# kowaalczyk/reformer-tts

Measured on AMD Instinct MI355X. Metric: mel-frames/sec training step, LJSpeech-shape batch, higher is better.
Workload: dtype bf16; 1 GPU; config/baseline.yml full Reformer-TTS training step (enc 3 / dec 3 layers, d=512, LSH 8 rounds, buckets 64/128), per-GPU batch 12, text 200->256, mel 1024x80; global_batch=12, parallelism=dp1, reversible_recompute=full

## Files before the change

### include/rtts.h

```cpp
#ifndef RTTS_H
#define RTTS_H

#include <stdint.h>

#ifdef __cplusplus
extern "C" {
#endif

#define RTTS_VERSION 1

int rtts_version(void);
const char* rtts_last_error(void);

int rtts_lsh_hash_sort(const void* qk, int64_t ld_qk, const float* rotations, int rot_rows,
                       int B, int H, int T, int dh, int n_hashes, int bucket_size,
                       int32_t* buckets, int32_t* st, int32_t* undo, void* stream);
int rtts_lsh_hash_sort_launches(int T);

int rtts_lsh_attn_fwd(const void* qk, const void* v, int64_t ld, const int32_t* st, const uint8_t* mask,
                      int B, int H, int T, int dh, int n_hashes, int bucket_size, int causal,
                      void* o, float* lse, float drop_p, uint32_t drop_seed, const uint32_t* seed_dev, void* stream);
int rtts_lsh_attn_fwd_run_length(int B, int H, int T, int n_hashes, int bucket_size);
int rtts_debug_set_walk(int fwd_run, int bwd_run);

int rtts_lsh_combine_fwd(const void* o, const float* lse, int B, int H, int T, int dh, int n_hashes,
                         void* out, int64_t ld_out, float* lse_tot, void* stream);

int rtts_lsh_bwd_qk_slots(void);
int rtts_lsh_attn_bwd_run_length(int B, int H, int T, int n_hashes, int bucket_size);
int rtts_lsh_bwd_delta(const void* out, int64_t ld_out, const void* dout, int64_t ld_dout,
                       int B, int H, int T, int dh, float* delta, void* stream);
int rtts_lsh_attn_bwd(const void* qk, const void* v, int64_t ld, const int32_t* st, const uint8_t* mask,
                      const void* dout, int64_t ld_dout, const float* lse_tot, const float* delta,
                      int B, int H, int T, int dh, int n_hashes, int bucket_size, int causal,
                      void* dqk_part, void* dv_part, uint8_t* row_flags, float drop_p, uint32_t drop_seed, const uint32_t* seed_dev,
                      void* stream);
int rtts_lsh_bwd_reduce(const void* dqk_part, const void* dv_part, int B, int H, int T, int dh, int n_hashes,
                        void* dqk, void* dv, int64_t ld_d, const uint8_t* row_flags, void* stream);

int rtts_grad_clip_scale(const float* grads, int64_t n, float grad_mult, float max_norm, float* partial_ws,
                         float* scale_out, void* stream);
int rtts_adamw_step(float* params, const float* grads, float* exp_avg, float* exp_avg_sq, const uint8_t* decay_mask,
                    int64_t n, const float* scale, const float* hyper, float beta1, float beta2, float eps,
                    float weight_decay, void* bf16_mirror, void* stream);

int rtts_ln_fwd(const float* x, const float* gamma, const float* beta, void* xn, float* mean, float* rstd,
                int M, int d, void* stream);
int rtts_ln_bwd(const void* dxn, const float* x, const float* mean, const float* rstd, const float* gamma,
                float* dx_io, float* dgamma, float* dbeta, float* partial_ws, int M, int d,
                void* dyb_next, float* partial_next, float drop_p, uint32_t seed, const uint32_t* seed_dev, void* stream);
int rtts_ln_bwd_to(const void* dxn, const float* x, const float* mean, const float* rstd, const float* gamma, const float* dx_in,
                   float* dx_out, float* dgamma, float* dbeta, float* partial_ws, int M, int d,
                   void* dyb_next, float* partial_next, float drop_p, uint32_t seed, const uint32_t* seed_dev, void* stream);
int rtts_ln_bwd_join(const void* dxn, const float* x, const float* mean, const float* rstd, const float* gamma, const float* dx_in,
                     const float* addend, float* dx_out, float* dgamma, float* dbeta, float* partial_ws, int M, int d,
                     void* dyb_next, float* partial_next, float drop_p, uint32_t seed, const uint32_t* seed_dev, void* stream);
int rtts_cast_colsum(const float* dy, void* dyb, float* dbias, float* partial_ws, int M, int d, float drop_p, uint32_t seed,
                     const uint32_t* seed_dev, const float* scale_dev, void* stream);
int rtts_colsum_bf16(void* dh, const void* h, int64_t ld, float* dbias, float* partial_ws, int M, int d,
                     int relu_gate, float gate_scale, void* gated_out, void* stream);
#define RTTS_COLSUM_MAX_GROUP 48
typedef struct {
    const float* partial;
    float* out;
    int32_t nrows, n;
    int32_t ld, reserved;
} rtts_colsum_job;
int rtts_colsum_partial_rows(int M);
int rtts_colsum_final_grouped(const rtts_colsum_job* jobs, int n, void* stream);
int rtts_residual_epilogue(const float* x, const void* g, const float* bias, float sign, float* y,
                           int64_t M, int d, float drop_p, uint32_t seed, const uint32_t* seed_dev, void* stream);
int rtts_residual_ln(float* x, const void* g, const float* bias, float sign, const float* gamma, const float* beta,
                     void* xn, float* mean, float* rstd, int M, int d, float drop_p, uint32_t seed, const uint32_t* seed_dev,
                     float* y, void* stream);
int rtts_sum_streams(const float* a, const float* b, int64_t n, float* out, void* out_bf16, void* stream);
int rtts_bias_act(void* h, const float* bias, int64_t M, int d, int relu, void* stream);
int rtts_cast_f32_bf16(const float* src, void* dst, int64_t n, void* stream);

int rtts_xattn_key_chunks(int Tk);
int rtts_xattn_fwd(const void* q, int64_t ld_q, const void* kv, int64_t ld_kv, const uint8_t* kvalid,
                   int B, int H, int Tq, int Tk, int dh, void* o, int64_t ld_o, float* lse,
                   float drop_p, uint32_t seed, const uint32_t* seed_dev, void* stream);
int rtts_xattn_bwd(const void* q, int64_t ld_q, const void* kv, int64_t ld_kv, const uint8_t* kvalid,
                   const void* dout, int64_t ld_dout, const float* lse, const float* delta,
                   int B, int H, int Tq, int Tk, int dh, void* dq, int64_t ld_dq, void* dkv_part,
                   float drop_p, uint32_t seed, const uint32_t* seed_dev, void* dq_chunks, void* stream);
int rtts_sum_slabs(const void* part, int nslabs, int64_t n, void* out, void* stream);
int rtts_xattn_probs_mean(const void* q, int64_t ld_q, const void* kv, int64_t ld_kv, const uint8_t* kvalid,
                          const float* lse, int B, int H, int Tq, int Tk, int dh, float* a, int64_t ld_a, void* stream);

int rtts_conv1d_k5(const void* x, int64_t ldx, const void* wp, int64_t ldw, int transposed, int M, int C_out, int C_in,
                   void* y, int64_t ldy, const float* bias, int out_f32, void* stream);
int rtts_to_halo(const void* src, int64_t ld_src, int64_t src_batch_stride, int C_src, int src_f32, int B, int L, int halo, int C,
                 void* dst, int lead, int64_t rows, void* stream);
int rtts_conv_w_perm(const float* w, int Co, int Ci, int CP, void* wp, void* stream);
int rtts_conv_dw_unperm(const float* dwp, int Co, int Ci, int CP, float* dw, void* stream);
#define RTTS_CONV_PERM_MAX_GROUP 8
typedef struct {
    const float* w;
    void* wp;
    int32_t Co, Ci, CP, reserved;
} rtts_conv_perm_job;
int rtts_conv_w_perm_grouped(const rtts_conv_perm_job* jobs, int n, void* stream);
int rtts_conv_dw_unperm_grouped(const rtts_conv_perm_job* jobs, int n, void* stream);
int rtts_conv1d_k5_moments(const void* x, int64_t ldx, const void* wp, int64_t ldw, int M, int C_out, int C_in, void* y, int64_t ldy,
                           int B, int L, int halo, float* partial, void* stream);
int rtts_bn_stats_from_partials(const float* partial, int nrows, int B, int L, int C, float* mean, float* rstd, float* run_mean,
                                float* run_var, const float* mean_shift, int64_t* num_batches, void* stream);
int rtts_bn_stats(const float* y, int B, int L, int halo, int C, float* mean, float* rstd, float* run_mean, float* run_var,
                  const float* mean_shift, int64_t* num_batches, float* partial_ws, void* stream);
int rtts_bn_act_fwd(const float* y, const float* mean, const float* rstd, const float* gamma, const float* beta, int act,
                    float drop_p, uint32_t seed, const uint32_t* seed_dev, int B, int L, int halo, int C, void* z, int z_halo,
                    int z_lead, int64_t z_rows, void* stream);
int rtts_bn_act_bwd(const float* y, const void* dz, int dz_halo, const float* mean, const float* rstd, const float* gamma,
                    const float* beta, int act, float drop_p, uint32_t seed, const uint32_t* seed_dev, int B, int L, int halo, int C,
                    void* dy, int dy_lead, int64_t dy_rows, float* dgamma, float* dbeta, float* partial_ws, void* stream);
int rtts_bn_moments(const float* y, int B, int L, int halo, int C, float* moments, float* partial_ws, void* stream);
int rtts_bn_from_moments(const float* moments, int64_t count, int C, float* mean, float* rstd, float* run_mean, float* run_var,
                         const float* mean_shift, int64_t* num_batches, void* stream);
int rtts_bn_act_bwd_sums(const float* y, const void* dz, int dz_halo, const float* mean, const float* rstd, const float* gamma,
                         const float* beta, int act, float drop_p, uint32_t seed, const uint32_t* seed_dev, int B, int L, int halo, int C,
// ... 115 lines not shown
```

### reformer-tts_amd/_lib.py

```python
from __future__ import annotations

import ctypes as C
import os

_HERE = os.path.dirname(os.path.abspath(__file__))
LIB_PATH = os.environ.get("RTTS_LIB") or os.path.join(_HERE, "lib", "librtts_hip.so")

_i64, _i32, _vp, _f32, _u32 = C.c_int64, C.c_int, C.c_void_p, C.c_float, C.c_uint32

class GemmTnProblem(C.Structure):
    _fields_ = [("a", _vp), ("lda", _i64), ("b", _vp), ("ldb", _i64), ("c", _vp), ("ldc", _i64),
                ("M", C.c_int32), ("N", C.c_int32), ("K", C.c_int32), ("accumulate", C.c_int32)]


GEMM_TN_MAX_GROUP = 16


class GemmNtProblem(C.Structure):
    _fields_ = [("a", _vp), ("lda", _i64), ("w", _vp), ("ldw", _i64), ("c", _vp), ("ldc", _i64), ("bias", _vp), ("aux", _vp),
                ("ld_aux", _i64), ("aux_out", _vp), ("M", C.c_int32), ("N", C.c_int32), ("K", C.c_int32), ("epilogue", C.c_int32),
                ("T", C.c_int32), ("H", C.c_int32), ("accumulate", C.c_int32), ("reserved", C.c_int32)]


GEMM_NT_MAX_GROUP = 4


class ColsumJob(C.Structure):
    _fields_ = [("partial", _vp), ("out", _vp), ("nrows", C.c_int32), ("n", C.c_int32), ("ld", C.c_int32), ("reserved", C.c_int32)]


COLSUM_MAX_GROUP = 48


class Segment(C.Structure):
    _fields_ = [("dst", _vp), ("src", _vp), ("count", C.c_int64), ("kind", C.c_int32), ("reserved", C.c_int32)]


SEGMENTS_MAX = 12
SEG_COPY_F32, SEG_COPY_BF16, SEG_ADD_F32, SEG_CAST_F32_BF16 = 0, 1, 2, 3


class ConvPermJob(C.Structure):
    _fields_ = [("w", _vp), ("wp", _vp), ("Co", C.c_int32), ("Ci", C.c_int32), ("CP", C.c_int32), ("reserved", C.c_int32)]


CONV_PERM_MAX_GROUP = 8

SIGNATURES = {
    "rtts_lsh_hash_sort": [_vp, _i64, _vp, _i32, _i32, _i32, _i32, _i32, _i32, _i32, _vp, _vp, _vp, _vp],
    "rtts_lsh_attn_fwd": [_vp, _vp, _i64, _vp, _vp, _i32, _i32, _i32, _i32, _i32, _i32, _i32, _vp, _vp, _f32, _u32, _vp, _vp],
    "rtts_lsh_hash_sort_launches": [_i32],
    "rtts_lsh_attn_fwd_run_length": [_i32, _i32, _i32, _i32, _i32],
    "rtts_lsh_combine_fwd": [_vp, _vp, _i32, _i32, _i32, _i32, _i32, _vp, _i64, _vp, _vp],
    "rtts_lsh_bwd_delta": [_vp, _i64, _vp, _i64, _i32, _i32, _i32, _i32, _vp, _vp],
    "rtts_lsh_attn_bwd": [_vp, _vp, _i64, _vp, _vp, _vp, _i64, _vp, _vp, _i32, _i32, _i32, _i32, _i32, _i32, _i32, _vp, _vp, _vp, _f32, _u32, _vp,
                          _vp],
    "rtts_lsh_bwd_qk_slots": [],
    "rtts_lsh_attn_bwd_run_length": [_i32, _i32, _i32, _i32, _i32],
    "rtts_debug_set_walk": [_i32, _i32],
    "rtts_lsh_bwd_reduce": [_vp, _vp, _i32, _i32, _i32, _i32, _i32, _vp, _vp, _i64, _vp, _vp],
    "rtts_grad_clip_scale": [_vp, _i64, _f32, _f32, _vp, _vp, _vp],
    "rtts_ln_fwd": [_vp, _vp, _vp, _vp, _vp, _vp, _i32, _i32, _vp],
    "rtts_ln_bwd": [_vp, _vp, _vp, _vp, _vp, _vp, _vp, _vp, _vp, _i32, _i32, _vp, _vp, _f32, _u32, _vp, _vp],
    "rtts_ln_bwd_to": [_vp, _vp, _vp, _vp, _vp, _vp, _vp, _vp, _vp, _vp, _i32, _i32, _vp, _vp, _f32, _u32, _vp, _vp],
    "rtts_ln_bwd_join": [_vp, _vp, _vp, _vp, _vp, _vp, _vp, _vp, _vp, _vp, _vp, _i32, _i32, _vp, _vp, _f32, _u32, _vp, _vp],
    "rtts_cast_colsum": [_vp, _vp, _vp, _vp, _i32, _i32, _f32, _u32, _vp, _vp, _vp],
    "rtts_colsum_bf16": [_vp, _vp, _i64, _vp, _vp, _i32, _i32, _i32, _f32, _vp, _vp],
    "rtts_sum_streams": [_vp, _vp, _i64, _vp, _vp, _vp],
    "rtts_residual_epilogue": [_vp, _vp, _vp, _f32, _vp, _i64, _i32, _f32, _u32, _vp, _vp],
    "rtts_colsum_partial_rows": [_i32],
    "rtts_colsum_final_grouped": [C.POINTER(ColsumJob), _i32, _vp],
    "rtts_residual_ln": [_vp, _vp, _vp, _f32, _vp, _vp, _vp, _vp, _vp, _i32, _i32, _f32, _u32, _vp, _vp, _vp],
    "rtts_bias_act": [_vp, _vp, _i64, _i32, _i32, _vp],
    "rtts_cast_f32_bf16": [_vp, _vp, _i64, _vp],
    "rtts_xattn_fwd": [_vp, _i64, _vp, _i64, _vp, _i32, _i32, _i32, _i32, _i32, _vp, _i64, _vp, _f32, _u32, _vp, _vp],
    "rtts_xattn_bwd": [_vp, _i64, _vp, _i64, _vp, _vp, _i64, _vp, _vp, _i32, _i32, _i32, _i32, _i32, _vp, _i64, _vp, _f32, _u32, _vp, _vp, _vp],
    "rtts_xattn_key_chunks": [_i32],
    "rtts_xattn_probs_mean": [_vp, _i64, _vp, _i64, _vp, _vp, _i32, _i32, _i32, _i32, _i32, _vp, _i64, _vp],
    "rtts_sum_slabs": [_vp, _i32, _i64, _vp, _vp],
    "rtts_conv1d_k5": [_vp, _i64, _vp, _i64, _i32, _i32, _i32, _i32, _vp, _i64, _vp, _i32, _vp],
    "rtts_to_halo": [_vp, _i64, _i64, _i32, _i32, _i32, _i32, _i32, _i32, _vp, _i32, _i64, _vp],
    "rtts_heads_grad": [_vp, _vp, _i32, _vp, _i64, _vp, _i32, _i32, _i32, _i32, _i32, _vp, _vp, _vp],
    "rtts_segments": [C.POINTER(Segment), _i32, _vp],
    "rtts_conv_w_perm": [_vp, _i32, _i32, _i32, _vp, _vp],
    "rtts_conv_dw_unperm": [_vp, _i32, _i32, _i32, _vp, _vp],
    "rtts_conv_w_perm_grouped": [C.POINTER(ConvPermJob), _i32, _vp],
    "rtts_conv_dw_unperm_grouped": [C.POINTER(ConvPermJob), _i32, _vp],
    "rtts_conv1d_k5_moments": [_vp, _i64, _vp, _i64, _i32, _i32, _i32, _vp, _i64, _i32, _i32, _i32, _vp, _vp],
    "rtts_bn_stats_from_partials": [_vp, _i32, _i32, _i32, _i32, _vp, _vp, _vp, _vp, _vp, _vp, _vp],
    "rtts_bn_stats": [_vp, _i32, _i32, _i32, _i32, _vp, _vp, _vp, _vp, _vp, _vp, _vp, _vp],
    "rtts_bn_act_fwd": [_vp, _vp, _vp, _vp, _vp, _i32, _f32, _u32, _vp, _i32, _i32, _i32, _i32, _vp, _i32, _i32, _i64, _vp],
    "rtts_bn_act_bwd": [_vp, _vp, _i32, _vp, _vp, _vp, _vp, _i32, _f32, _u32, _vp, _i32, _i32, _i32, _i32, _vp, _i32, _i64, _vp, _vp, _vp, _vp],
    "rtts_bn_moments": [_vp, _i32, _i32, _i32, _i32, _vp, _vp, _vp],
    "rtts_bn_from_moments": [_vp, _i64, _i32, _vp, _vp, _vp, _vp, _vp, _vp, _vp],
    "rtts_bn_act_bwd_sums": [_vp, _vp, _i32, _vp, _vp, _vp, _vp, _i32, _f32, _u32, _vp, _i32, _i32, _i32, _i32, _vp, _vp, _vp, _vp, _vp],
    "rtts_bn_act_bwd_apply": [_vp, _vp, _i32, _vp, _vp, _vp, _vp, _i32, _f32, _u32, _vp, _i32, _i32, _i32, _i32, _vp, _i64, _vp, _i32, _i64, _vp],
    "rtts_tts_loss": [_vp, _vp, _i64, _vp, _vp, _vp, _i64, _vp, _i32, _i32, _i32, _f32, _f32, _f32, _f32, _vp, _vp, _i64, _vp, _vp, _vp, _i32, _i32,
                      _vp, _i64, _i32, _i32, _i64, _i64, _vp, _i64, _i64, _vp],
    "rtts_pe_add": [_vp, _vp, _vp, _f32, _u32, _vp, _i32, _i64, _i32, _vp, _vp],
    "rtts_debug_stamp": [_vp, _i32, _vp],
    "rtts_batch_masks": [_vp, _i64, _i32, _i32, _i32, _vp, _i64, _i64, _i32, _i32, _i32, _vp, _vp, _vp, _vp, _vp],
    "rtts_pe_dalpha": [_vp, _vp, _f32, _u32, _vp, _i32, _i64, _i32, _vp, _vp, _vp],
    "rtts_relu_drop": [_vp, _f32, _u32, _vp, _i64, _vp],
    "rtts_embedding_bwd": [_vp, _vp, _i32, _i32, _i32, _i32, _vp, _f32, _u32, _vp, _vp],
    "rtts_embedding_bwd_strided": [_vp, _vp, _i64, _i64, _i32, _i32, _i32, _i32, _i32, _vp, _f32, _u32, _vp, _vp],
    "rtts_embedding_fwd": [_vp, _vp, _i32, _i32, _i32, _f32, _u32, _vp, _vp, _vp],
    "rtts_gemm_tn": [_vp, _i64, _vp, _i64, _i32, _i32, _i32, _vp, _i64, _i32, _vp, _i64, _vp],
    "rtts_gemm_tn_grouped": [C.POINTER(GemmTnProblem), _i32, _vp, _i64, _vp],
    "rtts_gemm_nt": [_vp, _i64, _vp, _i64, _i32, _i32, _i32, _i32, _vp, _i64, _vp, _i32, _vp, _i64, _vp, _vp],
    "rtts_gemm_nt_partial_rows": [_i32, _i32],
    "rtts_gemm_nt_grouped": [C.POINTER(GemmNtProblem), _i32, _i32, _vp],
    "rtts_debug_set_gemm_mode": [_i32],
    "rtts_gemm_nt_gate_words": [_i32, _i32],
    "rtts_gemm_nt_gated": [_vp, _i64, _vp, _i64, _i32, _i32, _i32, _i32, _vp, _i64, _vp, _i32, _vp, _vp, _vp],
    "rtts_peak_copy": [_vp, _vp, _i64, _vp],
    "rtts_comm_probe": [_vp, _vp, _i64, _i32, _i32, _vp],
    "rtts_peak_mfma": [_vp, _i32, _i32, _vp],
    "rtts_sw_depthwise_k3": [_vp, _vp, _vp, _i32, _i32, _i32, _vp, _vp, _vp, _vp],
    "rtts_sw_gate": [_vp, _vp, _i64, _i32, _i32, _i32, _i32, _i32, _i32, _vp, _vp],
    "rtts_sw_coupling_inv": [_vp, _i64, _vp, _i64, _i32, _vp],
    "rtts_sw_depthwise_k3_seg": [_vp, _vp, _vp, _vp, _i32, _i32, _i64, _i32, _vp, _vp, _vp, _vp],
    "rtts_sw_pack_mel": [_vp, _i64, _i64, _i64, _i32, _i32, _vp, _i32, _i64, _vp, _i64, _vp],
    "rtts_sw_coupling_inv1x1": [_vp, _i64, _vp, _i64, _vp, _i32, _i64, _vp, _i64, _vp],
    "rtts_sw_coupling_fwd1x1": [_vp, _i64, _vp, _i64, _vp, _i32, _i32, _i64, _vp, _i64, _vp, _i64, _i32, _vp, _vp],
    "rtts_sw_nll_reduce": [_vp, _i64, _i32, _vp, _vp, _i32, _i32, _i64, _i64, _vp, _vp],
    "rtts_sw_pack_audio": [_vp, _i64, _vp, _vp, _i32, _i32, _i32, _i64, _vp, _vp],
    "rtts_adamw_step": [_vp, _vp, _vp, _vp, _vp, _i64, _vp, _vp, _f32, _f32, _f32, _f32, _vp, _vp],
    "rtts_mel_frames": [_i64, _i32],
    "rtts_mel_spectrogram": [_vp, C.POINTER(_i64), C.POINTER(_i64), _vp, _vp, _i32, _vp, _vp, _i32, _i32, _i32, _i32, _f32, _vp, _i64, _vp],
    "rtts_resample_len": [_i64, _i32, _i32],
    "rtts_resample": [_vp, _i32, _i32, C.POINTER(_i64), C.POINTER(_i64), _vp, _vp, _i32, _vp, _vp, _i32, _i32, _i32, _vp, _vp],
}

_lib = None


class RttsError(RuntimeError):
    pass


_NOTED = set()
PATHS_LEFT = []


def note_general_path(where: str, reason: str) -> None:
    key = (where, reason)
    if key in _NOTED:
        return
    _NOTED.add(key)
    PATHS_LEFT.append(key)
    import logging
    logging.getLogger("reformer_tts_amd").warning("%s: general (eager) path instead of the explicit HIP executor -- %s", where, reason)


def log_once(key: str, message: str) -> None:
    if key in _NOTED:
        return
    _NOTED.add(key)
    import logging
    logging.getLogger("reformer_tts_amd").warning("%s", message)


def load() -> C.CDLL:
    global _lib
    if _lib is None:
        if not os.path.exists(LIB_PATH):
            raise RttsError(
                f"{LIB_PATH} is missing: build it with `python reformer-tts_amd/build.py` "
                "(or __graft_entry__.build()). There is no CPU fallback for the HIP path.")
        import torch
        lib = C.CDLL(LIB_PATH)
        lib.rtts_version.restype = C.c_int
        lib.rtts_last_error.restype = C.c_char_p
        for name, args in SIGNATURES.items():
            fn = getattr(lib, name)
            fn.argtypes = args
            fn.restype = C.c_int
        lib.rtts_gemm_nt_gate_words.restype = C.c_int64
        lib.rtts_mel_frames.restype = C.c_int64
        lib.rtts_resample_len.restype = C.c_int64
        _lib = lib
        fw, bw = os.environ.get("RTTS_LSH_FWD_WALK"), os.environ.get("RTTS_LSH_BWD_WALK")
        if fw is not None or bw is not None:
            _WALK[:] = [-1 if fw is None else int(fw), -1 if bw is None else int(bw)]
            lib.rtts_debug_set_walk(*_WALK)
        gs = os.environ.get("RTTS_GEMM_STORE")
        if gs is not None:
            lib.rtts_debug_set_gemm_mode(10 + int(gs))
    return _lib


_WALK = [-1, -1]


class forced_walk:

    def __init__(self, fwd=None, bwd=None):
        self.want = (fwd, bwd)

    def __enter__(self):
        self.old = list(_WALK)
        new = [o if w is None else int(w) for o, w in zip(self.old, self.want)]
        call("rtts_debug_set_walk", *new)
        _WALK[:] = new
        return self

    def __exit__(self, *exc):
        call("rtts_debug_set_walk", *self.old)
        _WALK[:] = self.old
        return False


def call(name: str, *args) -> None:
    lib = load()
    rc = getattr(lib, name)(*args)
    if rc != 0:
        raise RttsError(lib.rtts_last_error().decode() or f"{name} failed with code {rc}")
```

### reformer-tts_amd/csrc/lsh_attn_bwd.hip

```cpp
#include "rtts_common.h"
#include <float.h>

#define AB_DH 64
#define AB_ROWB 128
#ifndef AB_SPLIT_EPI
#define AB_SPLIT_EPI 1
#endif
#ifndef AB_DQ_UNROLL
#define AB_DQ_UNROLL 16
#endif
#ifndef AB_UNROLL
#define AB_UNROLL 4
#endif

typedef __attribute__((ext_vector_type(8))) short short8v;

#ifdef AB_PHASE_TIMING
__device__ unsigned long long g_ab_phase[32 * 8192];
#define AB_STAMP(i) do { if (threadIdx.x == 0 && blockIdx.x < 8192) g_ab_phase[blockIdx.x * 32 + (i)] = __builtin_readcyclecounter(); } while (0)
extern "C" int rtts_debug_ab_phases(void* dst) { return (int)hipMemcpyFromSymbol(dst, HIP_SYMBOL(g_ab_phase), sizeof(g_ab_phase)); }
#define AB_WSTAMP(i, w) do { if ((threadIdx.x & 63) == 0 && blockIdx.x < 8192) g_ab_phase[blockIdx.x * 32 + (i) + (w)] = __builtin_readcyclecounter(); } while (0)
#else
#define AB_STAMP(i) do { } while (0)
#define AB_WSTAMP(i, w) do { } while (0)
#endif

__device__ __forceinline__ bf16x8 tr_frag(const unsigned char* p0, const unsigned char* p1) {
    const short4v lo = __builtin_amdgcn_ds_read_tr16_b64_v4i16((RTTS_LDS short4v*)p0);
    const short4v hi = __builtin_amdgcn_ds_read_tr16_b64_v4i16((RTTS_LDS short4v*)p1);
    const short8v both = {lo[0], lo[1], lo[2], lo[3], hi[0], hi[1], hi[2], hi[3]};
    return __builtin_bit_cast(bf16x8, both);
}

__device__ __forceinline__ int ab_sw(int row) { return ((row >> 1) & 3) | ((((row >> 3) ^ (row >> 1)) & 1) << 2); }
__device__ __forceinline__ int ab_off(int row, int piece) { return row * 128 + ((piece ^ ab_sw(row)) << 4); }
template <int BS>
__device__ __forceinline__ int ab_ds_off(int key, int gran) {
    const int k0 = key & 1, k1 = (key >> 1) & 1, k2 = (key >> 2) & 1, k3 = (key >> 3) & 1;
    if (BS == 128) return key * 256 + ((gran ^ ((k1 << 4) | (k0 << 3) | (k1 << 2) | (k2 << 1) | k3)) << 3);
    return key * 128 + ((gran ^ ((k1 << 3) | (k0 << 2) | (k2 << 1) | k3)) << 3);
}

__device__ __forceinline__ int ab_stg_w(int r, int piece, int hh) { return r * 128 + ((piece ^ (r & 7)) << 4) + ((hh ^ ((r >> 3) & 1)) << 3); }
__device__ __forceinline__ int ab_stg_r(int i, int srow, int spiece) { return (i * 8 + srow) * 128 + ((spiece ^ srow) << 4); }
__device__ __forceinline__ uint4 ab_stg_fix(int i, const uint4 v) { return (i & 1) ? uint4{v.z, v.w, v.x, v.y} : v; }

#ifndef AB_KT2
#define AB_KT2 1
#endif

typedef __attribute__((ext_vector_type(2))) __bf16 ab_bf2;
__device__ __forceinline__ float ab_frags_sumsq(const bf16x8 (&f)[4]) {
    float part[4];
#pragma unroll
    for (int ks = 0; ks < 4; ++ks) {
        const uint4 u = __builtin_bit_cast(uint4, f[ks]);
        float a = 0.f;
        a = __builtin_amdgcn_fdot2_f32_bf16(__builtin_bit_cast(ab_bf2, u.x), __builtin_bit_cast(ab_bf2, u.x), a, false);
        a = __builtin_amdgcn_fdot2_f32_bf16(__builtin_bit_cast(ab_bf2, u.y), __builtin_bit_cast(ab_bf2, u.y), a, false);
        a = __builtin_amdgcn_fdot2_f32_bf16(__builtin_bit_cast(ab_bf2, u.z), __builtin_bit_cast(ab_bf2, u.z), a, false);
        a = __builtin_amdgcn_fdot2_f32_bf16(__builtin_bit_cast(ab_bf2, u.w), __builtin_bit_cast(ab_bf2, u.w), a, false);
        part[ks] = a;
    }
    return (part[0] + part[1]) + (part[2] + part[3]);
}

struct AbDrop {
    uint32_t seed;
    const uint32_t* seed_dev;
    uint32_t thresh;
    float scale;
};

template <int BS, bool CAUSAL, bool MASKED, bool DROP>
__global__ __launch_bounds__(BS * 4 / AB_KT2, AB_KT2 == 2 ? 1 : 2) void lsh_attn_bwd_kernel(
    const bf16_t* __restrict__ qk, const bf16_t* __restrict__ v, int64_t ld, const int32_t* __restrict__ st,
    const uint8_t* __restrict__ mask, const bf16_t* __restrict__ dout, int64_t ld_do, const float* __restrict__ lse_tot,
    const float* __restrict__ delta, int H, int T, int n_hashes, bf16_t* __restrict__ dqk_part, bf16_t* __restrict__ dv_part,
    size_t slot_stride, AbDrop dr) {
    constexpr int KT2 = AB_KT2;
    constexpr int NK = 2 * BS;
    constexpr int NQT = BS / 32;
    constexpr int NW = NK / (32 * KT2);
    constexpr int NTHR = 64 * NW;
    constexpr int DSROW = BS * 2;
    extern __shared__ __attribute__((aligned(16))) unsigned char smem[];
    int* kpos = reinterpret_cast<int*>(smem) + NK;
    float* qlse = reinterpret_cast<float*>(kpos + 2 * NK);
    float* qdel = qlse + BS;
    int* qpe_s = reinterpret_cast<int*>(qdel + BS);
    unsigned char* Ks = reinterpret_cast<unsigned char*>(qpe_s + BS);
    unsigned char* Os = Ks + NK * 128;
    unsigned char* Ds = Os + BS * 128;
    unsigned char* Stg = Ds + NK * DSROW;

    const int nb = T / BS;
    const int C = n_hashes * nb;
    const uint32_t wi = xcd_remap(blockIdx.x, gridDim.x);
    const int bh = wi / C, c = wi % C;
    const int b = bh / H, h = bh % H;
    const int cprev = (c == 0) ? C - 1 : c - 1;
    const int tid = threadIdx.x, lane = tid & 63, wave = __builtin_amdgcn_readfirstlane(tid >> 6);
    const int r = lane & 31, hh = lane >> 5;

    AB_STAMP(0);
    const int32_t* st_row = st + (size_t)bh * n_hashes * T;
    const bf16_t* qbase = qk + (size_t)b * T * ld + (size_t)h * AB_DH;
    const bf16_t* vbase = v + (size_t)b * T * ld + (size_t)h * AB_DH;
    const bf16_t* dobase = dout + (size_t)b * T * ld_do + (size_t)h * AB_DH;

    constexpr int ITERS = NK * 8 / NTHR;
    int trow[ITERS];
#pragma unroll
    for (int it = 0; it < ITERS; ++it) {
        const int row = (it * NTHR + tid) >> 3;
        const int slot = (row < BS) ? c * BS + row : cprev * BS + (row - BS);
        trow[it] = st_row[slot];
    }
    int myrow[KT2], mypos[KT2];
#pragma unroll
    for (int k2 = 0; k2 < KT2; ++k2) {
        myrow[k2] = (wave * KT2 + k2) * 32 + r;
        mypos[k2] = st_row[(myrow[k2] < BS) ? c * BS + myrow[k2] : cprev * BS + (myrow[k2] - BS)];
    }
#ifdef AB_PHASE_TIMING
    __builtin_amdgcn_s_waitcnt(0x0F70);
    AB_STAMP(10);
#endif
#pragma unroll
    for (int it = 0; it < ITERS; ++it) {
        const int rowb = it * (NTHR / 8) + wave * 8;
        const int lp = (lane & 7) ^ ab_sw(rowb + (lane >> 3));
        __builtin_amdgcn_global_load_lds((const __attribute__((address_space(1))) void*)(qbase + (size_t)trow[it] * ld + lp * 8),
                                         (RTTS_LDS void*)(Ks + rowb * 128), 16, 0, 0);
        if (it < ITERS / 2)
            __builtin_amdgcn_global_load_lds((const __attribute__((address_space(1))) void*)(dobase + (size_t)trow[it] * ld_do + lp * 8),
                                             (RTTS_LDS void*)(Os + rowb * 128), 16, 0, 0);
    }
    int rvalid[ITERS / 2];
    float rlse[ITERS / 2], rdel[ITERS / 2];
#pragma unroll
    for (int it = 0; it < ITERS / 2; ++it) {
        rvalid[it] = MASKED ? (int)mask[(size_t)b * T + trow[it]] : 1;
        rlse[it] = lse_tot[(size_t)bh * T + trow[it]];
        rdel[it] = delta[(size_t)bh * T + trow[it]];
    }
    int myvalid[KT2];
    bf16x8 vf[KT2][4];
#pragma unroll
    for (int k2 = 0; k2 < KT2; ++k2) {
        myvalid[k2] = MASKED ? (int)mask[(size_t)b * T + mypos[k2]] : 1;
#pragma unroll
        for (int ks = 0; ks < 4; ++ks) vf[k2][ks] = *reinterpret_cast<const bf16x8*>(vbase + (size_t)mypos[k2] * ld + ks * 16 + 8 * hh);
    }
#ifdef AB_PHASE_TIMING
    __builtin_amdgcn_s_waitcnt(0x0F70);
    AB_STAMP(11);
#endif
    const int cbase = (tid & 7) < 3 ? (tid & 7) * (NK * 4) : 3 * NK * 4 + ((tid & 7) - 3) * (BS * 4);
#pragma unroll
    for (int it = 0; it < ITERS / 2; ++it) {
        const int row = (it * NTHR + tid) >> 3, piece = tid & 7;
// ... 224 lines not shown
        for (int di = 0; di < KT2; ++di) {
            const int dt = (KT2 == 2) ? di : (wave & 1);
            const int kpc = dt * 4 + 2 * trc + (trp >> 1);
            ko0[di] = ab_off(rl, kpc) + 8 * (trp & 1);
            ko1[di] = ab_off(rl + 4, kpc) + 8 * (trp & 1);
        }
        const int gq = qt * 8 + 4 * trc + trp;
        const int do0 = ab_ds_off<BS>(rl, gq), do1 = ab_ds_off<BS>(rl + 4, gq);
#pragma unroll AB_DQ_UNROLL
        for (int kb = 0; kb < NK; kb += 16) {
            const bf16x8 bfrag = tr_frag(Ds + kb * DSROW + do0, Ds + kb * DSROW + do1);
#pragma unroll
            for (int di = 0; di < KT2; ++di) {
                const bf16x8 afrag = tr_frag(Ks + kb * 128 + ko0[di], Ks + kb * 128 + ko1[di]);
                dq[di] = __builtin_amdgcn_mfma_f32_32x32x16_bf16(afrag, bfrag, dq[di], 0, 0, 0);
            }
        }
#pragma unroll
        for (int di = 0; di < KT2; ++di) {
            const int dt = (KT2 == 2) ? di : (wave & 1);
#pragma unroll
            for (int g = 0; g < 4; ++g) {
                uint2 pk;
                pk.x = pack_bf16x2(dq[di][4 * g], dq[di][4 * g + 1]);
                pk.y = pack_bf16x2(dq[di][4 * g + 2], dq[di][4 * g + 3]);
                *reinterpret_cast<uint2*>(Os + ab_off(qt * 32 + r, dt * 4 + g) + 8 * hh) = pk;
            }
        }
    }
    AB_STAMP(6);
    __syncthreads();
    AB_STAMP(7);

#pragma unroll
    for (int k2 = 0; k2 < KT2; ++k2) {
        unsigned char* stg = Stg + (wave * KT2 + k2) * (32 * AB_ROWB);
        bf16_t* dkdst = dqk_part + (own_tile ? 0 : slot_stride);
        float kraw[2][16];
        float dot = 0.f;
#pragma unroll
        for (int dt = 0; dt < 2; ++dt)
#pragma unroll
            for (int g = 0; g < 4; ++g) {
                const uint2 kk = *reinterpret_cast<const uint2*>(Ks + ab_off(myrow[k2], dt * 4 + g) + 8 * hh);
                kraw[dt][4 * g] = __uint_as_float(kk.x << 16);
                kraw[dt][4 * g + 1] = __uint_as_float(kk.x & 0xffff0000u);
                kraw[dt][4 * g + 2] = __uint_as_float(kk.y << 16);
                kraw[dt][4 * g + 3] = __uint_as_float(kk.y & 0xffff0000u);
#pragma unroll
                for (int j = 0; j < 4; ++j) dot = __builtin_fmaf(kraw[dt][4 * g + j], gacc[k2][dt][4 * g + j], dot);
            }
        const float ncoef = -rtts_xhalf_sum(dot) * (ksc[k2] * 8.f) * (ksc[k2] * 8.f);
#pragma unroll
        for (int dt = 0; dt < 2; ++dt)
#pragma unroll
            for (int g = 0; g < 4; ++g) {
                float dk[4];
#pragma unroll
                for (int j = 0; j < 4; ++j) dk[j] = __builtin_fmaf(kraw[dt][4 * g + j], ncoef, gacc[k2][dt][4 * g + j]);
                if (own_tile) {
                    const uint2 dqv = *reinterpret_cast<const uint2*>(Os + ab_off(myrow[k2], dt * 4 + g) + 8 * hh);
                    dk[0] += __uint_as_float(dqv.x << 16);
                    dk[1] += __uint_as_float(dqv.x & 0xffff0000u);
                    dk[2] += __uint_as_float(dqv.y << 16);
                    dk[3] += __uint_as_float(dqv.y & 0xffff0000u);
                }
                uint2 pk;
                pk.x = pack_bf16x2(dk[0], dk[1]);
                pk.y = pack_bf16x2(dk[2], dk[3]);
                *reinterpret_cast<uint2*>(stg + ab_stg_w(r, dt * 4 + g, hh)) = pk;
            }
        __builtin_amdgcn_wave_barrier();
        uint4 rowv[4];
#pragma unroll
        for (int i = 0; i < 4; ++i) rowv[i] = ab_stg_fix(i, *reinterpret_cast<const uint4*>(stg + ab_stg_r(i, srow, spiece)));
#pragma unroll
        for (int i = 0; i < 4; ++i) rtts_store16_out(dkdst + (obase + rpos[k2][i]) * AB_DH + spiece * 8, rowv[i]);
    }
    AB_STAMP(8);
#ifdef AB_PHASE_TIMING
    __builtin_amdgcn_s_waitcnt(0);
    AB_STAMP(9);
#endif
}



__device__ __forceinline__ void ab_dma16(const void* gptr, RTTS_LDS void* lds_dst_wave_uniform) {
    const uint32_t m0v = __builtin_amdgcn_readfirstlane((uint32_t)(uintptr_t)lds_dst_wave_uniform);
    asm volatile("s_mov_b32 m0, %1\n\ts_nop 0\n\tglobal_load_lds_dwordx4 %0, off" ::"v"(gptr), "s"(m0v) : "m0");
}

template <int BS, bool CAUSAL, bool MASKED, bool DROP>
__global__ __launch_bounds__(BS * 4, 2) void lsh_attn_bwd_walk_kernel(
    const bf16_t* __restrict__ qk, const bf16_t* __restrict__ v, int64_t ld, const int32_t* __restrict__ st,
    const uint8_t* __restrict__ mask, const bf16_t* __restrict__ dout, int64_t ld_do, const float* __restrict__ lse_tot,
    const float* __restrict__ delta, int H, int T, int n_hashes, bf16_t* __restrict__ dqk_part, bf16_t* __restrict__ dv_part,
    size_t slot_stride, int R, uint8_t* __restrict__ row_flags, AbDrop dr) {
    constexpr int NK = 2 * BS;
    constexpr int NQT = BS / 32;
    constexpr int NW = NK / 32;
    constexpr int NTHR = 64 * NW;
    constexpr int DSROW = BS * 2;
    constexpr int KSLOT = BS * 128;
    extern __shared__ __attribute__((aligned(16))) unsigned char smem[];
    int* kposS = reinterpret_cast<int*>(smem);
    float* qlseS = reinterpret_cast<float*>(kposS + 4 * BS);
    float* qdelS = qlseS + 2 * BS;
    int* qpeS = reinterpret_cast<int*>(qdelS + 2 * BS);
    unsigned char* KsR = reinterpret_cast<unsigned char*>(qpeS + 2 * BS);
    unsigned char* OsR = KsR + 3 * KSLOT;
    unsigned char* Ds = OsR + 2 * KSLOT;
    unsigned char* Stg = Ds;

    const int nb = T / BS;
    const int C = n_hashes * nb;
    const int runs = C / R;
    const uint32_t run = xcd_remap(blockIdx.x, gridDim.x);
    const int bh = run / runs, c0 = (run % runs) * R;
    const int b = bh / H, h = bh % H;
    const int32_t* st_row = st + (size_t)bh * n_hashes * T;
    const bf16_t* qbase = qk + (size_t)b * T * ld + (size_t)h * AB_DH;
    const bf16_t* vbase = v + (size_t)b * T * ld + (size_t)h * AB_DH;
    const bf16_t* dobase = dout + (size_t)b * T * ld_do + (size_t)h * AB_DH;

    {
        const int tid = threadIdx.x, lane = tid & 63, wave = __builtin_amdgcn_readfirstlane(tid >> 6);
        const int cp0 = (c0 == 0) ? C - 1 : c0 - 1;
        constexpr int ITERS = NK * 8 / NTHR;
        int trow[ITERS];
#pragma unroll
        for (int it = 0; it < ITERS; ++it) {
            const int row = (it * NTHR + tid) >> 3;
            trow[it] = st_row[(row < BS) ? c0 * BS + row : cp0 * BS + (row - BS)];
        }
        int pnext = 0;
        if (R > 1 && tid < BS) pnext = st_row[(c0 + 1) * BS + tid];
#pragma unroll
        for (int it = 0; it < ITERS; ++it) {
            const int rowb = it * (NTHR / 8) + wave * 8;
            const int lp = (lane & 7) ^ ab_sw(rowb + (lane >> 3));
            unsigned char* kdst = (rowb < BS) ? KsR + KSLOT + rowb * 128 : KsR + (rowb - BS) * 128;
            __builtin_amdgcn_global_load_lds((const __attribute__((address_space(1))) void*)(qbase + (size_t)trow[it] * ld + lp * 8),
                                             (RTTS_LDS void*)kdst, 16, 0, 0);
            if (it < ITERS / 2)
                __builtin_amdgcn_global_load_lds((const __attribute__((address_space(1))) void*)(dobase + (size_t)trow[it] * ld_do + lp * 8),
                                                 (RTTS_LDS void*)(OsR + rowb * 128), 16, 0, 0);
        }
        int rvalid[ITERS / 2];
        float rlse[ITERS / 2], rdel[ITERS / 2];
#pragma unroll
        for (int it = 0; it < ITERS / 2; ++it) {
            rvalid[it] = MASKED ? (int)mask[(size_t)b * T + trow[it]] : 1;
            rlse[it] = lse_tot[(size_t)bh * T + trow[it]];
            rdel[it] = delta[(size_t)bh * T + trow[it]];
        }
#pragma unroll
        for (int it = 0; it < ITERS; ++it) {
            const int row = (it * NTHR + tid) >> 3, piece = tid & 7;
            if (piece == 1) kposS[(row < BS) ? BS + row : row - BS] = trow[it];
            if (it < ITERS / 2) {
                if (piece == 3) qlseS[row] = rlse[it] * 1.4426950408889634f;
                if (piece == 4) qdelS[row] = -rdel[it];
                if (piece == 5) qpeS[row] = rvalid[it] ? (CAUSAL ? trow[it] : 0) : -1;
            }
        }
        if (R > 1 && tid < BS) kposS[2 * BS + tid] = pnext;
    }
#if AB_SPLIT_EPI
    __builtin_amdgcn_s_waitcnt(0x0F70);
    __syncthreads();
#endif

    bf16x8 vf[4], kf[4];
    float ksc = 0.f, sdq = 0.f;
    int myvalid = 1, mypos = 0, kpk = 0;
    f32x16 dvacc[2], gacc[2];
#pragma unroll 1
    for (int j = 0; j < R; ++j) {
        int tid = threadIdx.x;
        asm volatile("" : "+v"(tid));
// ... 318 lines not shown
#endif
                    const float dqf[4] = {__uint_as_float(dqv.x << 16), __uint_as_float(dqv.x & 0xffff0000u), __uint_as_float(dqv.y << 16),
                                          __uint_as_float(dqv.y & 0xffff0000u)};
#pragma unroll
                    for (int jj = 0; jj < 4; ++jj) {
                        gacc[dt][4 * g + jj] += dqf[jj];
                        sd4[jj] = __builtin_fmaf(kraw[dt][4 * g + jj], dqf[jj], sd4[jj]);
                    }
                }
            sdq = rtts_xhalf_sum((sd4[0] + sd4[1]) + (sd4[2] + sd4[3]));
        }
        if (!own_tile || j == R - 1) {
            const int slot = (!own_tile && j == 0) ? 1 : 0;
            const size_t obase = ((size_t)bh * n_hashes + (own_tile ? c / nb : cprev / nb)) * T;
            const int srow = lane >> 3, spiece = lane & 7;
#if AB_SPLIT_EPI
            unsigned char* stg = Ds + ((own_tile ? BS : 0) + wt * 32) * DSROW;
            static_assert(32 * DSROW >= 32 * AB_ROWB, "the staging must fit a wave's rows of the dS'^T image");
#else
            unsigned char* stg = Stg + wave * (32 * AB_ROWB);
#endif
            int rpos[4];
#pragma unroll
            for (int i = 0; i < 4; ++i) rpos[i] = own_tile ? kq[wt * 32 + i * 8 + srow] : kl[wt * 32 + i * 8 + srow];
            {
                bf16_t* dvdst = dv_part + slot * slot_stride;
#pragma unroll
                for (int dt = 0; dt < 2; ++dt)
#pragma unroll
                    for (int g = 0; g < 4; ++g) {
                        uint2 pk;
                        pk.x = pack_bf16x2(dvacc[dt][4 * g], dvacc[dt][4 * g + 1]);
                        pk.y = pack_bf16x2(dvacc[dt][4 * g + 2], dvacc[dt][4 * g + 3]);
                        *reinterpret_cast<uint2*>(stg + ab_stg_w(r, dt * 4 + g, hh)) = pk;
                    }
                __builtin_amdgcn_wave_barrier();
                uint4 rowv[4];
#pragma unroll
                for (int i = 0; i < 4; ++i) rowv[i] = ab_stg_fix(i, *reinterpret_cast<const uint4*>(stg + ab_stg_r(i, srow, spiece)));
#pragma unroll
                for (int i = 0; i < 4; ++i) rtts_store16_out(dvdst + (obase + rpos[i]) * AB_DH + spiece * 8, rowv[i]);
                __builtin_amdgcn_wave_barrier();
            }
            {
                bf16_t* dkdst = dqk_part + slot * slot_stride;
                float dot4[4] = {0.f, 0.f, 0.f, 0.f};
#pragma unroll
                for (int dt = 0; dt < 2; ++dt)
#pragma unroll
                    for (int e = 0; e < 16; ++e) dot4[e & 3] = __builtin_fmaf(kraw[dt][e], gacc[dt][e], dot4[e & 3]);
                const float dot = (dot4[0] + dot4[1]) + (dot4[2] + dot4[3]);
                const float ncoef = -(rtts_xhalf_sum(dot) - sdq) * (ksc * 8.f) * (ksc * 8.f);
#pragma unroll
                for (int dt = 0; dt < 2; ++dt)
#pragma unroll
                    for (int g = 0; g < 4; ++g) {
                        float dk[4];
#pragma unroll
                        for (int jj = 0; jj < 4; ++jj) dk[jj] = __builtin_fmaf(kraw[dt][4 * g + jj], ncoef, gacc[dt][4 * g + jj]);
                        uint2 pk;
                        pk.x = pack_bf16x2(dk[0], dk[1]);
                        pk.y = pack_bf16x2(dk[2], dk[3]);
                        *reinterpret_cast<uint2*>(stg + ab_stg_w(r, dt * 4 + g, hh)) = pk;
                    }
                __builtin_amdgcn_wave_barrier();
                uint4 rowv[4];
#pragma unroll
                for (int i = 0; i < 4; ++i) rowv[i] = ab_stg_fix(i, *reinterpret_cast<const uint4*>(stg + ab_stg_r(i, srow, spiece)));
#pragma unroll
                for (int i = 0; i < 4; ++i) rtts_store16_out(dkdst + (obase + rpos[i]) * AB_DH + spiece * 8, rowv[i]);
            }
            if (slot == 0 && spiece == 0) {
#pragma unroll
                for (int i = 0; i < 4; ++i) row_flags[obase + rpos[i]] = own_tile ? 1 : 0;
            }
        }
        AB_JSTAMP(8);
#ifdef AB_PHASE_TIMING
        __builtin_amdgcn_s_waitcnt(0x0F70);
        AB_JSTAMP(9);
#endif
    }
#undef AB_JSTAMP
}

extern "C" int rtts_lsh_bwd_qk_slots(void) { return RTTS_LSH_BWD_QK_SLOTS; }

extern "C" int rtts_lsh_attn_bwd_run_length(int B, int H, int T, int n_hashes, int bucket_size) {
    if (B <= 0 || H <= 0 || n_hashes <= 0 || bucket_size <= 0 || T <= 0 || T % bucket_size) return -1;
    const int C = n_hashes * (T / bucket_size);
    const long long chunks = (long long)B * H * C;
    int R = 0;
    if (AB_KT2 == 1)
        for (int cand = 8; cand >= 4; cand >>= 1)
            if (C % cand == 0 && chunks / cand >= 768) { R = cand; break; }
    const int w = rtts_walk_override(1);
    if (w >= 0 && AB_KT2 == 1) R = (w >= 1 && C % w == 0) ? w : 0;
    return R;
}

template <int BS>
static int launch_attn_bwd(const bf16_t* qk, const bf16_t* v, int64_t ld, const int32_t* st, const uint8_t* mask,
                           const bf16_t* dout, int64_t ld_do, const float* lse_tot, const float* delta, int B, int H, int T,
                           int n_hashes, int causal, bf16_t* dqk_part, bf16_t* dv_part, uint8_t* row_flags, float drop_p,
                           uint32_t drop_seed, const uint32_t* seed_dev, hipStream_t stream) {
    constexpr int NK = 2 * BS;
    const size_t slot_stride = (size_t)B * H * n_hashes * T * AB_DH;
    const bool drop = drop_p > 0.f;
    const int vi = (drop ? 4 : 0) + (causal ? 2 : 0) + (mask ? 1 : 0);
    const AbDrop dr{drop_seed, seed_dev, rtts_drop_thresh(drop_p), 1.f / (1.f - drop_p)};
    const int C = n_hashes * (T / BS);
    const long long chunks = (long long)B * H * C;
    const int R = rtts_lsh_attn_bwd_run_length(B, H, T, n_hashes, BS);
    if (R >= 1 && AB_KT2 == 1) {
        RTTS_REQUIRE(row_flags, "rtts_lsh_attn_bwd: this shape is worked by the walking kernel (rtts_lsh_attn_bwd_run_length() = %d): "
                                "row_flags (B*H*n_hashes*T bytes) is required", R);
        const size_t ds_bytes = (size_t)NK * (BS * 2), stg_bytes = (size_t)(NK / 32) * 32 * AB_ROWB;
        const size_t wlds = (size_t)BS * 40 + 5 * (size_t)BS * 128 + (ds_bytes > stg_bytes ? ds_bytes : stg_bytes);
        static RttsLdsState wattr[8];
        const dim3 wgrid((unsigned)(chunks / R)), wblock(BS * 4);
#define AB_WGO(C_, M_, D_)                                                                                                 \
    do {                                                                                                                   \
        auto kern = lsh_attn_bwd_walk_kernel<BS, C_, M_, D_>;                                                              \
        RTTS_ENSURE_LDS("rtts_lsh_attn_bwd", kern, wlds, wattr[vi]);                                                       \
        hipLaunchKernelGGL(kern, wgrid, wblock, wlds, stream, qk, v, ld, st, mask, dout, ld_do, lse_tot, delta, H, T, n_hashes, \
                           dqk_part, dv_part, slot_stride, R, row_flags, dr);                                              \
    } while (0)
#define AB_WGO2(C_, M_) do { if (drop) AB_WGO(C_, M_, true); else AB_WGO(C_, M_, false); } while (0)
        if (causal) {
            if (mask) AB_WGO2(true, true); else AB_WGO2(true, false);
        } else {
            if (mask) AB_WGO2(false, true); else AB_WGO2(false, false);
        }
#undef AB_WGO2
#undef AB_WGO
        RTTS_LAUNCH_CHECK("rtts_lsh_attn_bwd");
        return 0;
    }
    const size_t lds = NK * 128 + BS * 128 + NK * (BS * 2) + (NK / 32) * 32 * AB_ROWB + NK * 12 + BS * 12;
    const dim3 grid(B * H * n_hashes * (T / BS)), block(BS * 4 / AB_KT2);
    static RttsLdsState attr[8];
#define AB_GO(C_, M_, D_)                                                                                                  \
    do {                                                                                                                   \
        auto kern = lsh_attn_bwd_kernel<BS, C_, M_, D_>;                                                                   \
        RTTS_ENSURE_LDS("rtts_lsh_attn_bwd", kern, lds, attr[vi]);                                                         \
        hipLaunchKernelGGL(kern, grid, block, lds, stream, qk, v, ld, st, mask, dout, ld_do, lse_tot, delta, H, T, n_hashes, \
                           dqk_part, dv_part, slot_stride, dr);                                                            \
    } while (0)
#define AB_GO2(C_, M_) do { if (drop) AB_GO(C_, M_, true); else AB_GO(C_, M_, false); } while (0)
    if (causal) {
        if (mask) AB_GO2(true, true); else AB_GO2(true, false);
    } else {
        if (mask) AB_GO2(false, true); else AB_GO2(false, false);
    }
#undef AB_GO2
#undef AB_GO
    RTTS_LAUNCH_CHECK("rtts_lsh_attn_bwd");
    return 0;
}

extern "C" int rtts_lsh_attn_bwd(const void* qk, const void* v, int64_t ld, const int32_t* st, const uint8_t* mask,
                                 const void* dout, int64_t ld_dout, const float* lse_tot, const float* delta, int B, int H,
                                 int T, int dh, int n_hashes, int bucket_size, int causal, void* dqk_part, void* dv_part,
                                 uint8_t* row_flags, float drop_p, uint32_t drop_seed, const uint32_t* seed_dev, void* stream) {
    RTTS_ENTER(stream);
    RTTS_REQUIRE(qk && v && st && dout && lse_tot && delta && dqk_part && dv_part, "rtts_lsh_attn_bwd: null pointer");
    RTTS_REQUIRE(dh == AB_DH, "rtts_lsh_attn_bwd: dh=%d unsupported (this build: 64)", dh);
    RTTS_REQUIRE(bucket_size == 64 || bucket_size == 128, "rtts_lsh_attn_bwd: bucket_size=%d unsupported (64 or 128)", bucket_size);
    RTTS_REQUIRE(T > 0 && T % (2 * bucket_size) == 0,
                 "rtts_lsh_attn_bwd: Sequence length (%d) needs to be divisible by target bucket size x 2 - %d", T, 2 * bucket_size);
    RTTS_REQUIRE(B > 0 && H > 0 && n_hashes > 0, "rtts_lsh_attn_bwd: bad B/H/n_hashes");
    RTTS_REQUIRE(ld >= (int64_t)H * dh && ld % 8 == 0 && ld_dout >= (int64_t)H * dh && ld_dout % 8 == 0,
                 "rtts_lsh_attn_bwd: row strides must be >= H*dh and multiples of 8");
    RTTS_REQUIRE((((uintptr_t)qk | (uintptr_t)v | (uintptr_t)dout | (uintptr_t)dqk_part | (uintptr_t)dv_part) & 15) == 0,
                 "rtts_lsh_attn_bwd: buffers must be 16-byte aligned");
    RTTS_REQUIRE(drop_p >= 0.f && drop_p < 1.f, "rtts_lsh_attn_bwd: drop_p must be in [0, 1)");
    RTTS_REQUIRE(drop_p == 0.f || (uint64_t)B * H * n_hashes * T * 2 * bucket_size < (1ull << 32),
                 "rtts_lsh_attn_bwd: dropout on more than 2^32 query-key pairs (the forward refuses the same shape)");
    hipStream_t s = (hipStream_t)stream;
    if (bucket_size == 64)
        return launch_attn_bwd<64>((const bf16_t*)qk, (const bf16_t*)v, ld, st, mask, (const bf16_t*)dout, ld_dout, lse_tot, delta,
                                   B, H, T, n_hashes, causal, (bf16_t*)dqk_part, (bf16_t*)dv_part, row_flags, drop_p, drop_seed, seed_dev, s);
    return launch_attn_bwd<128>((const bf16_t*)qk, (const bf16_t*)v, ld, st, mask, (const bf16_t*)dout, ld_dout, lse_tot, delta, B,
                                H, T, n_hashes, causal, (bf16_t*)dqk_part, (bf16_t*)dv_part, row_flags, drop_p, drop_seed, seed_dev, s);
}
```

### reformer-tts_amd/csrc/lsh_attn_fwd.hip

```cpp
#include "rtts_common.h"
#include <float.h>

#define AF_DH 64
#define AF_ROWB 144
#define AF_LOG2E 1.4426950408889634f
#define AF_NEG (-1.0e30f)
#define AF_BIGPOS 0x40000000
#define AF_SLACK 8.0f

typedef __attribute__((ext_vector_type(8))) short af_short8;
typedef __attribute__((ext_vector_type(2))) __bf16 af_bf2;

#ifdef AF_PHASE_TIMING
__device__ unsigned long long g_af_phase[16 * 8192];
#define AF_STAMP(i) do { if ((threadIdx.x & 63) == 0 && blockIdx.x < 8192 && ((threadIdx.x >> 6) == 0 || (threadIdx.x >> 6) == BS / 32)) \
        g_af_phase[blockIdx.x * 16 + ((threadIdx.x >> 6) ? 8 : 0) + (i)] = __builtin_readcyclecounter(); } while (0)
extern "C" int rtts_debug_af_phases(void* dst) { return (int)hipMemcpyFromSymbol(dst, HIP_SYMBOL(g_af_phase), sizeof(g_af_phase)); }
#ifndef AF_WSTEP
#define AF_WSTEP 1
#endif
#define AF_WSTAMP(i) do { if (j == AF_WSTEP && lane == 0 && blockIdx.x < 8192 && qt == 0) \
        g_af_phase[blockIdx.x * 16 + (kh ? 8 : 0) + (i)] = __builtin_readcyclecounter(); } while (0)
#else
#define AF_STAMP(i) do { } while (0)
#define AF_WSTAMP(i) do { } while (0)
#endif

#ifndef AF_UNROLL
#define AF_UNROLL BS == 64 ? 2 : 1
#endif
__device__ __forceinline__ int af_sw(int row) { return ((row >> 1) & 3) | ((((row >> 3) ^ (row >> 1)) & 1) << 2); }
__device__ __forceinline__ int af_voff(int row, int piece) { return row * 128 + ((piece ^ af_sw(row)) << 4); }

__device__ __forceinline__ float af_sum16(const f32x16& a) {
    const float s0 = (a[0] + a[1]) + (a[2] + a[3]), s1 = (a[4] + a[5]) + (a[6] + a[7]);
    const float s2 = (a[8] + a[9]) + (a[10] + a[11]), s3 = (a[12] + a[13]) + (a[14] + a[15]);
    return (s0 + s1) + (s2 + s3);
}

#ifndef AF_FOLD
#define AF_FOLD 1
#endif
#ifndef AF_TILE_SKIP
#define AF_TILE_SKIP 1
#endif
__device__ __forceinline__ void af_tile_probs(f32x16& acc, const float* __restrict__ ksc_t, const int* __restrict__ kpos_t,
                                              const int* __restrict__ kpe_t, int keyt, int hh, bool chk_self, int qpos, int qpe, float& m,
                                              float& l, f32x16 (&oacc)[2], bool live_all = false) {
    const bool fresh = m < -1.0e4f;
    const float mref = fresh ? 0.f : m;
    const float nref = -mref, selfv = (-5e4f * AF_LOG2E) - mref;
    float gmax[2] = {AF_NEG, AF_NEG};
    if (chk_self) {
#pragma unroll
        for (int g = 0; g < 4; ++g) {
            const int key0 = keyt + 8 * g + 4 * hh;
            const float4 sc = *reinterpret_cast<const float4*>(ksc_t + key0);
            const int4 kp = *reinterpret_cast<const int4*>(kpos_t + key0);
            const int4 ke = *reinterpret_cast<const int4*>(kpe_t + key0);
            const float scv[4] = {sc.x, sc.y, sc.z, sc.w};
            const int kpv[4] = {kp.x, kp.y, kp.z, kp.w};
            const int kev[4] = {ke.x, ke.y, ke.z, ke.w};
#pragma unroll
            for (int j = 0; j < 4; ++j) {
                float x = __builtin_fmaf(acc[4 * g + j], scv[j], nref);
                x = (kev[j] > qpe) ? AF_NEG : x;
                x = (kpv[j] == qpos) ? selfv : x;
                acc[4 * g + j] = x;
                gmax[g & 1] = fmaxf(gmax[g & 1], x);
            }
        }
    } else if (live_all) {
#pragma unroll
        for (int g = 0; g < 4; ++g) {
            const float4 sc = *reinterpret_cast<const float4*>(ksc_t + keyt + 8 * g + 4 * hh);
            const float scv[4] = {sc.x, sc.y, sc.z, sc.w};
#pragma unroll
            for (int j = 0; j < 4; ++j) {
                const float x = __builtin_fmaf(acc[4 * g + j], scv[j], nref);
                acc[4 * g + j] = x;
                gmax[g & 1] = fmaxf(gmax[g & 1], x);
            }
        }
    } else {
#pragma unroll
        for (int g = 0; g < 4; ++g) {
            const int key0 = keyt + 8 * g + 4 * hh;
            const float4 sc = *reinterpret_cast<const float4*>(ksc_t + key0);
            const int4 ke = *reinterpret_cast<const int4*>(kpe_t + key0);
            const float scv[4] = {sc.x, sc.y, sc.z, sc.w};
            const int kev[4] = {ke.x, ke.y, ke.z, ke.w};
#pragma unroll
            for (int j = 0; j < 4; ++j) {
                float x = __builtin_fmaf(acc[4 * g + j], scv[j], nref);
                x = (kev[j] > qpe) ? AF_NEG : x;
                acc[4 * g + j] = x;
                gmax[g & 1] = fmaxf(gmax[g & 1], x);
            }
        }
    }
    const float tmax = rtts_xhalf_max(fmaxf(gmax[0], gmax[1]));
    if (__any(tmax > (fresh ? 0.5f * AF_NEG : AF_SLACK))) {
        const float mnew = fmaxf(m, tmax + mref);
        const float alpha = __builtin_amdgcn_exp2f(m - mnew);
        const float d = mnew - mref;
        m = mnew;
#pragma unroll
        for (int i = 0; i < 16; ++i) {
            oacc[0][i] *= alpha;
            oacc[1][i] *= alpha;
            acc[i] -= d;
        }
        l *= alpha;
    }
#pragma unroll
    for (int i = 0; i < 16; ++i) acc[i] = __builtin_amdgcn_exp2f(acc[i]);
    l += af_sum16(acc);
}

template <int BS, bool CAUSAL, bool MASKED, bool DROP>
__global__ __launch_bounds__(BS * 4, 2) void lsh_attn_fwd_kernel(const bf16_t* __restrict__ qk, const bf16_t* __restrict__ v,
                                                                 int64_t ld, const int32_t* __restrict__ st,
                                                                 const uint8_t* __restrict__ mask, int H, int T, int n_hashes,
                                                                 bf16_t* __restrict__ o, float* __restrict__ lse, uint32_t drop_seed,
                                                                 const uint32_t* __restrict__ seed_dev, uint32_t drop_thresh,
                                                                 float drop_scale) {
    constexpr int NK = 2 * BS;
    constexpr int NKT = NK / 32;
    constexpr int NTHR = BS * 4;
    constexpr int NQT = BS / 32;
    extern __shared__ __attribute__((aligned(16))) unsigned char smem[];
    float* ksc = reinterpret_cast<float*>(smem);
    int* kpos = reinterpret_cast<int*>(ksc + NK);
    int* kpe = kpos + NK;
    unsigned char* Ks = smem + NK * 12;
    unsigned char* Vs = Ks + NK * AF_ROWB;

    const int nb = T / BS;
    const int C = n_hashes * nb;
    const uint32_t wi = xcd_remap(blockIdx.x, gridDim.x);
    const int bh = wi / C, c = wi % C;
    const int b = bh / H, h = bh % H;
    const int cprev = (c == 0) ? C - 1 : c - 1;
    const int tid = threadIdx.x, lane = tid & 63, wave = __builtin_amdgcn_readfirstlane(tid >> 6);

    const int32_t* st_row = st + (size_t)bh * n_hashes * T;
    const bf16_t* qbase = qk + (size_t)b * T * ld + (size_t)h * AF_DH;
    const bf16_t* vbase = v + (size_t)b * T * ld + (size_t)h * AF_DH;

    AF_STAMP(0);
    constexpr int ITERS = NK * 8 / NTHR;
    {
        int trow[ITERS];
#pragma unroll
        for (int it = 0; it < ITERS; ++it) {
            const int row = (it * NTHR + tid) >> 3;
            const int slot = (row < BS) ? c * BS + row : cprev * BS + (row - BS);
            trow[it] = st_row[slot];
        }
        uint4 kreg[ITERS];
        int rvalid[ITERS];
#pragma unroll
        for (int it = 0; it < ITERS; ++it) {
            const int piece = tid & 7;
            kreg[it] = *reinterpret_cast<const uint4*>(qbase + (size_t)trow[it] * ld + piece * 8);
            const int rowb = it * (NTHR / 8) + wave * 8;
            const int lp = (lane & 7) ^ af_sw(rowb + (lane >> 3));
            __builtin_amdgcn_global_load_lds((const __attribute__((address_space(1))) void*)(vbase + (size_t)trow[it] * ld + lp * 8),
                                             (RTTS_LDS void*)(Vs + rowb * 128), 16, 0, 0);
            rvalid[it] = MASKED ? (int)mask[(size_t)b * T + trow[it]] : 1;
        }
        const int cbase = (tid & 7) * (NK * 4);
#pragma unroll
        for (int it = 0; it < ITERS; ++it) {
            const int row = (it * NTHR + tid) >> 3, piece = tid & 7;
            *reinterpret_cast<uint4*>(Ks + row * AF_ROWB + piece * 16) = kreg[it];
            float ss = 0.f;
            ss = __builtin_amdgcn_fdot2_f32_bf16(__builtin_bit_cast(af_bf2, kreg[it].x), __builtin_bit_cast(af_bf2, kreg[it].x), ss, false);
            ss = __builtin_amdgcn_fdot2_f32_bf16(__builtin_bit_cast(af_bf2, kreg[it].y), __builtin_bit_cast(af_bf2, kreg[it].y), ss, false);
            ss = __builtin_amdgcn_fdot2_f32_bf16(__builtin_bit_cast(af_bf2, kreg[it].z), __builtin_bit_cast(af_bf2, kreg[it].z), ss, false);
            ss = __builtin_amdgcn_fdot2_f32_bf16(__builtin_bit_cast(af_bf2, kreg[it].w), __builtin_bit_cast(af_bf2, kreg[it].w), ss, false);
            ss = rtts_sum8(ss);
            int w = __float_as_int((0.125f * AF_LOG2E) * __builtin_amdgcn_rsqf(fmaxf(ss, 1e-24f)));
            w = piece == 1 ? trow[it] : w;
            w = piece == 2 ? (rvalid[it] ? (CAUSAL ? trow[it] : 0) : AF_BIGPOS) : w;
            if (piece < 3) *reinterpret_cast<int*>(reinterpret_cast<unsigned char*>(ksc) + cbase + row * 4) = w;
        }
    }
    AF_STAMP(1);
    __syncthreads();
    AF_STAMP(2);

    const int r = lane & 31, hh = lane >> 5;
    const int qt = wave % NQT, kh = wave / NQT;
    const int qrow = qt * 32 + r;
    bf16x8 qf[4];
#pragma unroll
    for (int ks = 0; ks < 4; ++ks) qf[ks] = *reinterpret_cast<const bf16x8*>(Ks + qrow * AF_ROWB + (ks * 16 + 8 * hh) * 2);
    const int qpos = kpos[qrow];
    const int qpe = (kpe[qrow] == AF_BIGPOS) ? -1 : (CAUSAL ? qpos : 0);
    const int trq = (lane & 15) >> 2, trp = lane & 3, trc = (lane >> 4) & 1;

    int tro[2];
#pragma unroll
    for (int dt = 0; dt < 2; ++dt) tro[dt] = af_voff(4 * hh + trq, dt * 4 + 2 * trc + (trp >> 1)) + 8 * (trp & 1);

    const bool wrap = (cprev / nb) != (c / nb);
    float m = AF_NEG, l = 0.f;
    f32x16 oacc[2] = {{0}, {0}};
// ... 34 lines not shown
                }
            }
        } else {
#pragma unroll
            for (int g = 0; g < 4; ++g) {
                const int key0 = kt * 32 + 8 * g + 4 * hh;
                const float4 sc = *reinterpret_cast<const float4*>(ksc + key0);
                const int4 ke = *reinterpret_cast<const int4*>(kpe + key0);
                const float scv[4] = {sc.x, sc.y, sc.z, sc.w};
                const int kev[4] = {ke.x, ke.y, ke.z, ke.w};
#pragma unroll
                for (int j = 0; j < 4; ++j) {
                    float x = acc[4 * g + j] * scv[j];
#if !defined(AF_ABLATE) || AF_ABLATE != 2
                    x = (kev[j] > qpe) ? AF_NEG : x;
#endif
                    acc[4 * g + j] = x;
                    gmax[g & 1] = fmaxf(gmax[g & 1], x);
                }
            }
        }
        tmax = rtts_xhalf_max(fmaxf(gmax[0], gmax[1]));
#endif
        if (__any(tmax > m + AF_SLACK)) {
            const float mnew = fmaxf(m, tmax);
            const float alpha = __builtin_amdgcn_exp2f(m - mnew);
            m = mnew;
#pragma unroll
            for (int i = 0; i < 16; ++i) {
                oacc[0][i] *= alpha;
                oacc[1][i] *= alpha;
            }
            l *= alpha;
        }
#if defined(AF_ABLATE) && AF_ABLATE == 3
#pragma unroll
        for (int i = 0; i < 16; ++i) l += acc[i];
#else
#pragma unroll
        for (int i = 0; i < 16; ++i) acc[i] = __builtin_amdgcn_exp2f(acc[i] - m);
        l += af_sum16(acc);
#endif
#endif
        if constexpr (DROP) {
            const uint32_t seed = drop_seed + (seed_dev ? seed_dev[0] : 0u);
            const uint32_t pair0 = ((uint32_t)wi * BS + (uint32_t)qrow) * (uint32_t)NK + (uint32_t)(kt * 32 + 4 * hh);
#pragma unroll
            for (int i = 0; i < 16; ++i) acc[i] *= rtts_drop_keep(seed, pair0 + 8 * (i >> 2) + (i & 3), drop_thresh, drop_scale);
        }
#if defined(AF_ABLATE) && AF_ABLATE == 4
        oacc[0][0] += acc[0] + acc[5] + acc[10] + acc[15];
        if (false)
#endif
#pragma unroll
        for (int s2 = 0; s2 < 2; ++s2) {
            const int o8 = 8 * s2;
            const bf16x8 pf = cvt_bf16x8(acc[o8], acc[o8 + 1], acc[o8 + 2], acc[o8 + 3], acc[o8 + 4], acc[o8 + 5], acc[o8 + 6], acc[o8 + 7]);
#pragma unroll
            for (int dt = 0; dt < 2; ++dt) {
                const int blk = (kt * 32 + 16 * s2) * 128;
                const short4v lo = __builtin_amdgcn_ds_read_tr16_b64_v4i16((RTTS_LDS short4v*)(Vs + blk + tro[dt]));
                const short4v hi = __builtin_amdgcn_ds_read_tr16_b64_v4i16((RTTS_LDS short4v*)(Vs + blk + 8 * 128 + tro[dt ^ 1]));
                const af_short8 both = {lo[0], lo[1], lo[2], lo[3], hi[0], hi[1], hi[2], hi[3]};
                oacc[dt] = __builtin_amdgcn_mfma_f32_32x32x16_bf16(__builtin_bit_cast(bf16x8, both), pf, oacc[dt], 0, 0, 0);
            }
        }
    }
    l = rtts_xhalf_sum(l);

    float* part = reinterpret_cast<float*>(Ks) + (size_t)qt * 34 * 64;
    AF_STAMP(3);
    __syncthreads();
    AF_STAMP(4);
    if (kh == 1) {
#pragma unroll
        for (int i = 0; i < 16; ++i) {
            part[i * 64 + lane] = oacc[0][i];
            part[(16 + i) * 64 + lane] = oacc[1][i];
        }
        part[32 * 64 + lane] = m;
        part[33 * 64 + lane] = l;
    }
    __syncthreads();
    if (kh == 1) return;
    {
        const float m2 = part[32 * 64 + lane], l2 = part[33 * 64 + lane];
        const float mm = fmaxf(m, m2);
        float a1 = __builtin_amdgcn_exp2f(m - mm), a2 = __builtin_amdgcn_exp2f(m2 - mm);
        l = l * a1 + l2 * a2;
        m = mm;
        const float inv_l = 1.f / l;
        a1 *= inv_l;
        a2 *= inv_l;
#pragma unroll
        for (int i = 0; i < 16; ++i) {
            oacc[0][i] = oacc[0][i] * a1 + part[i * 64 + lane] * a2;
            oacc[1][i] = oacc[1][i] * a1 + part[(16 + i) * 64 + lane] * a2;
        }
    }

    const int round = c / nb;
    const size_t obase = ((size_t)bh * n_hashes + round) * T;
    unsigned char* stg = Vs + qt * (32 * AF_ROWB);
#pragma unroll
    for (int dt = 0; dt < 2; ++dt) {
#pragma unroll
        for (int g = 0; g < 4; ++g) {
            uint2 pk;
            pk.x = pack_bf16x2(oacc[dt][4 * g], oacc[dt][4 * g + 1]);
            pk.y = pack_bf16x2(oacc[dt][4 * g + 2], oacc[dt][4 * g + 3]);
            *reinterpret_cast<uint2*>(stg + r * AF_ROWB + (dt * 32 + 8 * g + 4 * hh) * 2) = pk;
        }
    }
    if (hh == 0) lse[obase + qpos] = (m + __builtin_amdgcn_logf(l)) * 0.6931471805599453f;
    __builtin_amdgcn_wave_barrier();
    const int srow = lane >> 3, spiece = lane & 7;
    uint4 rowv[4];
    int rpos[4];
#pragma unroll
    for (int i = 0; i < 4; ++i) {
        rowv[i] = *reinterpret_cast<const uint4*>(stg + (i * 8 + srow) * AF_ROWB + spiece * 16);
        rpos[i] = kpos[qt * 32 + i * 8 + srow];
    }
#pragma unroll
    for (int i = 0; i < 4; ++i) rtts_store16_out(o + (obase + rpos[i]) * AF_DH + spiece * 8, rowv[i]);
    AF_STAMP(5);
}


template <int BS, bool DROP>
__device__ __forceinline__ void af_walk_tiles(const unsigned char* __restrict__ Kt, const unsigned char* __restrict__ Vt,
                                              const float* __restrict__ ksc_t, const int* __restrict__ kpos_t,
                                              const int* __restrict__ kpe_t, const int* __restrict__ kmin_t, const int* __restrict__ kmax_t,
                                              const bf16x8 (&qf)[4], int qpos, int qpe, int self_lo,
                                              int self_hi, int r, int hh, const int (&tro)[2], float& m, float& l, f32x16 (&oacc)[2],
                                              uint32_t pair_base, uint32_t seed, uint32_t drop_thresh, float drop_scale) {
    constexpr int NT = BS / 32;
#pragma unroll AF_UNROLL
    for (int t = 0; t < NT; ++t) {
        const bool self_tile = t >= self_lo && t < self_hi;
        bool live_all = false;
#if AF_TILE_SKIP
        if (!self_tile) {
            if (__all(kmin_t[t] > qpe)) continue;
            live_all = __all(kmax_t[t] <= qpe);
        }
#endif
        f32x16 acc = {0};
#pragma unroll
        for (int ks = 0; ks < 4; ++ks) {
            const bf16x8 kf = *reinterpret_cast<const bf16x8*>(Kt + (t * 32 + r) * AF_ROWB + (ks * 16 + 8 * hh) * 2);
            acc = __builtin_amdgcn_mfma_f32_32x32x16_bf16(kf, qf[ks], acc, 0, 0, 0);
        }
#if AF_FOLD && !defined(AF_ABLATE)
        af_tile_probs(acc, ksc_t, kpos_t, kpe_t, t * 32, hh, self_tile, qpos, qpe, m, l, oacc, live_all);
#else
        float tmax = AF_NEG;
        float gmax[2] = {AF_NEG, AF_NEG};
        if (t >= self_lo && t < self_hi) {
#pragma unroll
            for (int g = 0; g < 4; ++g) {
                const int key0 = t * 32 + 8 * g + 4 * hh;
                const float4 sc = *reinterpret_cast<const float4*>(ksc_t + key0);
                const int4 kp = *reinterpret_cast<const int4*>(kpos_t + key0);
                const int4 ke = *reinterpret_cast<const int4*>(kpe_t + key0);
                const float scv[4] = {sc.x, sc.y, sc.z, sc.w};
                const int kpv[4] = {kp.x, kp.y, kp.z, kp.w};
                const int kev[4] = {ke.x, ke.y, ke.z, ke.w};
#pragma unroll
                for (int j = 0; j < 4; ++j) {
                    float x = acc[4 * g + j] * scv[j];
                    x = (kev[j] > qpe) ? AF_NEG : x;
                    x = (kpv[j] == qpos) ? (-5e4f * AF_LOG2E) : x;
                    acc[4 * g + j] = x;
                    gmax[g & 1] = fmaxf(gmax[g & 1], x);
                }
            }
        } else {
#pragma unroll
            for (int g = 0; g < 4; ++g) {
                const int key0 = t * 32 + 8 * g + 4 * hh;
                const float4 sc = *reinterpret_cast<const float4*>(ksc_t + key0);
                const int4 ke = *reinterpret_cast<const int4*>(kpe_t + key0);
                const float scv[4] = {sc.x, sc.y, sc.z, sc.w};
                const int kev[4] = {ke.x, ke.y, ke.z, ke.w};
#pragma unroll
                for (int j = 0; j < 4; ++j) {
                    float x = acc[4 * g + j] * scv[j];
#if !defined(AF_ABLATE) || AF_ABLATE != 2
                    x = (kev[j] > qpe) ? AF_NEG : x;
#endif
                    acc[4 * g + j] = x;
                    gmax[g & 1] = fmaxf(gmax[g & 1], x);
                }
            }
        }
        tmax = rtts_xhalf_max(fmaxf(gmax[0], gmax[1]));
        if (__any(tmax > m + AF_SLACK)) {
            const float mnew = fmaxf(m, tmax);
            const float alpha = __builtin_amdgcn_exp2f(m - mnew);
            m = mnew;
#pragma unroll
            for (int i = 0; i < 16; ++i) {
                oacc[0][i] *= alpha;
                oacc[1][i] *= alpha;
            }
            l *= alpha;
        }
#pragma unroll
        for (int i = 0; i < 16; ++i) {
#if defined(AF_ABLATE) && AF_ABLATE == 5
            acc[i] = acc[i] - m;
#else
            acc[i] = __builtin_amdgcn_exp2f(acc[i] - m);
#endif
        }
#if !defined(AF_ABLATE) || AF_ABLATE != 6
        l += af_sum16(acc);
#endif
#endif
        if constexpr (DROP) {
            const uint32_t pair0 = pair_base + (uint32_t)(t * 32 + 4 * hh);
#pragma unroll
            for (int i = 0; i < 16; ++i) acc[i] *= rtts_drop_keep(seed, pair0 + 8 * (i >> 2) + (i & 3), drop_thresh, drop_scale);
        }
#pragma unroll
        for (int s2 = 0; s2 < 2; ++s2) {
            const int o8 = 8 * s2;
            const bf16x8 pf = cvt_bf16x8(acc[o8], acc[o8 + 1], acc[o8 + 2], acc[o8 + 3], acc[o8 + 4], acc[o8 + 5], acc[o8 + 6], acc[o8 + 7]);
#pragma unroll
            for (int dt = 0; dt < 2; ++dt) {
                const int blk = (t * 32 + 16 * s2) * 128;
                const short4v lo = __builtin_amdgcn_ds_read_tr16_b64_v4i16((RTTS_LDS short4v*)(Vt + blk + tro[dt]));
                const short4v hi = __builtin_amdgcn_ds_read_tr16_b64_v4i16((RTTS_LDS short4v*)(Vt + blk + 8 * 128 + tro[dt ^ 1]));
                const af_short8 both = {lo[0], lo[1], lo[2], lo[3], hi[0], hi[1], hi[2], hi[3]};
                oacc[dt] = __builtin_amdgcn_mfma_f32_32x32x16_bf16(__builtin_bit_cast(bf16x8, both), pf, oacc[dt], 0, 0, 0);
            }
        }
    }
}

__device__ __forceinline__ float af_piece_sumsq(const uint4 q) {
    float ss = 0.f;
    ss = __builtin_amdgcn_fdot2_f32_bf16(__builtin_bit_cast(af_bf2, q.x), __builtin_bit_cast(af_bf2, q.x), ss, false);
    ss = __builtin_amdgcn_fdot2_f32_bf16(__builtin_bit_cast(af_bf2, q.y), __builtin_bit_cast(af_bf2, q.y), ss, false);
    ss = __builtin_amdgcn_fdot2_f32_bf16(__builtin_bit_cast(af_bf2, q.z), __builtin_bit_cast(af_bf2, q.z), ss, false);
    ss = __builtin_amdgcn_fdot2_f32_bf16(__builtin_bit_cast(af_bf2, q.w), __builtin_bit_cast(af_bf2, q.w), ss, false);
    return ss;
}

template <int BS, bool CAUSAL, bool MASKED, bool DROP>
__global__ __launch_bounds__(BS * 4, 2) void lsh_attn_fwd_walk_kernel(const bf16_t* __restrict__ qk, const bf16_t* __restrict__ v,
                                                                      int64_t ld, const int32_t* __restrict__ st,
                                                                      const uint8_t* __restrict__ mask, int H, int T, int n_hashes,
                                                                      bf16_t* __restrict__ o, float* __restrict__ lse,
                                                                      uint32_t drop_seed, const uint32_t* __restrict__ seed_dev,
                                                                      uint32_t drop_thresh, float drop_scale, int L) {
    constexpr int NK = 2 * BS;
    constexpr int NTHR = BS * 4;
    constexpr int NQT = BS / 32;
    const int NPOS = (L + 1) * BS;
    extern __shared__ __attribute__((aligned(16))) unsigned char smem[];
    int* allpos = reinterpret_cast<int*>(smem);
    int* allkpe = allpos + NPOS;
    float* ksc = reinterpret_cast<float*>(allkpe + NPOS);
    int* tkmin = reinterpret_cast<int*>(ksc + NK);
    int* tkmax = tkmin + 128;
    unsigned char* Ks = reinterpret_cast<unsigned char*>(tkmax + 128);
    unsigned char* Vs = Ks + NK * AF_ROWB;

    const int nb = T / BS;
    const int C = n_hashes * nb;
    const int runs = C / L;
    const uint32_t wi = xcd_remap(blockIdx.x, gridDim.x);
    const int bh = wi / runs, c0 = (wi % runs) * L;
    const int b = bh / H, h = bh % H;
    const int tid = threadIdx.x, lane = tid & 63, wave = __builtin_amdgcn_readfirstlane(tid >> 6);
    const int32_t* st_row = st + (size_t)bh * n_hashes * T;
    const bf16_t* qbase = qk + (size_t)b * T * ld + (size_t)h * AF_DH;
    const bf16_t* vbase = v + (size_t)b * T * ld + (size_t)h * AF_DH;

    for (int i = tid; i < NPOS; i += NTHR) {
        int ch = c0 - 1 + i / BS;
        ch = ch < 0 ? ch + C : ch;
        const int pos = st_row[ch * BS + (i % BS)];
        const int valid = MASKED ? (int)mask[(size_t)b * T + pos] : 1;
        allpos[i] = pos;
        allkpe[i] = valid ? (CAUSAL ? pos : 0) : AF_BIGPOS;
    }
    __syncthreads();
    for (int tile = wave; tile < NPOS / 32; tile += NTHR / 64) {
        int lo = allkpe[tile * 32 + (lane & 31)], hi = lo;
#pragma unroll
        for (int o = 16; o > 0; o >>= 1) {
            lo = min(lo, __shfl_xor(lo, o));
            hi = max(hi, __shfl_xor(hi, o));
        }
        if (lane == 0) { tkmin[tile] = lo; tkmax[tile] = hi; }
    }
    {
        constexpr int ITERS = NK * 8 / NTHR;
        uint4 kreg[ITERS];
#pragma unroll
        for (int it = 0; it < ITERS; ++it) {
            const int row = (it * NTHR + tid) >> 3, piece = tid & 7;
            const int pos = allpos[row < BS ? BS + row : row - BS];
            kreg[it] = *reinterpret_cast<const uint4*>(qbase + (size_t)pos * ld + piece * 8);
            const int rowb = it * (NTHR / 8) + wave * 8;
            const int lp = (lane & 7) ^ af_sw(rowb + (lane >> 3));
            __builtin_amdgcn_global_load_lds((const __attribute__((address_space(1))) void*)(vbase + (size_t)pos * ld + lp * 8),
                                             (RTTS_LDS void*)(Vs + rowb * 128), 16, 0, 0);
        }
#pragma unroll
        for (int it = 0; it < ITERS; ++it) {
            const int row = (it * NTHR + tid) >> 3, piece = tid & 7;
            *reinterpret_cast<uint4*>(Ks + row * AF_ROWB + piece * 16) = kreg[it];
            const float ss = rtts_sum8(af_piece_sumsq(kreg[it]));
            if (piece == 0) ksc[row] = (0.125f * AF_LOG2E) * __builtin_amdgcn_rsqf(fmaxf(ss, 1e-24f));
        }
    }
    __syncthreads();

    const int qt = wave % NQT, kh = wave / NQT;
    const uint32_t seed = DROP ? drop_seed + (seed_dev ? seed_dev[0] : 0u) : 0u;
    int lane_o = lane;

#pragma unroll 1
    for (int j = 0; j < L; ++j) {
        asm volatile("" : "+v"(lane_o));
        const int lane = lane_o;
        const int tid = wave * 64 + lane;
        const int r = lane & 31, hh = lane >> 5;
        const int qrow = qt * 32 + r;
        const int trq = (lane & 15) >> 2, trp = lane & 3, trc = (lane >> 4) & 1;
        int tro[2];
#pragma unroll
        for (int dt = 0; dt < 2; ++dt) tro[dt] = af_voff(4 * hh + trq, dt * 4 + 2 * trc + (trp >> 1)) + 8 * (trp & 1);
        AF_WSTAMP(0);
        const int so = j & 1, sp = so ^ 1;
        const int c = c0 + j;
        const int cprev = (c == 0) ? C - 1 : c - 1;
        const int ms = so ^ kh;
        bf16x8 qf[4];
#pragma unroll
        for (int ks = 0; ks < 4; ++ks)
            qf[ks] = *reinterpret_cast<const bf16x8*>(Ks + (so * BS + qrow) * AF_ROWB + (ks * 16 + 8 * hh) * 2);
        const int qpos = allpos[(j + 1) * BS + qrow];
        const int qpe = (allkpe[(j + 1) * BS + qrow] == AF_BIGPOS) ? -1 : (CAUSAL ? qpos : 0);
        const bool wrap = (cprev / nb) != (c / nb);
        const int self_lo = kh ? 0 : qt, self_hi = kh ? (wrap ? NQT : 0) : qt + 1;
        float m = AF_NEG, l = 0.f;
        f32x16 oacc[2] = {{0}, {0}};
        af_walk_tiles<BS, DROP>(Ks + ms * (BS * AF_ROWB), Vs + ms * (BS * 128), ksc + ms * BS, allpos + (j + 1 - kh) * BS,
                                allkpe + (j + 1 - kh) * BS, tkmin + (j + 1 - kh) * NQT, tkmax + (j + 1 - kh) * NQT, qf, qpos, qpe, self_lo,
                                self_hi, r, hh, tro, m, l, oacc,
                                ((uint32_t)(bh * C + c) * BS + (uint32_t)qrow) * (uint32_t)NK + (uint32_t)(kh * BS), seed,
                                drop_thresh, drop_scale);
        l = rtts_xhalf_sum(l);
        AF_WSTAMP(1);

        float* partA = reinterpret_cast<float*>(Ks + sp * (BS * AF_ROWB)) + qt * (18 * 64);
        float* partB = reinterpret_cast<float*>(Vs + sp * (BS * 128)) + qt * (16 * 64);
        __syncthreads();
        AF_WSTAMP(2);
        if (kh == 1) {
#pragma unroll
            for (int i = 0; i < 16; ++i) {
                partA[i * 64 + lane] = oacc[0][i];
                partB[i * 64 + lane] = oacc[1][i];
            }
            partA[16 * 64 + lane] = m;
            partA[17 * 64 + lane] = l;
            if (j + 1 == L) {
                __syncthreads();
                return;
            }
            const int t2 = tid - NTHR / 2;
            const int piece = t2 & 7, row0 = t2 >> 3;
            const int* npos = allpos + (j + 2) * BS + row0;
            const bf16_t* kp = qbase + piece * 8;
            const bf16_t* vp = vbase + piece * 8;
#define AF_FETCH(IT)                                                                                   \
            const size_t off##IT = (size_t)npos[IT * (NTHR / 16)] * ld;                                \
            const uint4 kreg##IT = *reinterpret_cast<const uint4*>(kp + off##IT);                      \
            const uint4 vreg##IT = *reinterpret_cast<const uint4*>(vp + off##IT)
            AF_FETCH(0); AF_FETCH(1); AF_FETCH(2); AF_FETCH(3);
#undef AF_FETCH
            AF_WSTAMP(3);
            __syncthreads();
            AF_WSTAMP(4);
            __syncthreads();
            AF_WSTAMP(5);
#define AF_PLACE(IT)                                                                                   \
            do {                                                                                       \
                const int row = row0 + IT * (NTHR / 16);                                               \
                *reinterpret_cast<uint4*>(Ks + (sp * BS + row) * AF_ROWB + piece * 16) = kreg##IT;     \
                *reinterpret_cast<uint4*>(Vs + sp * (BS * 128) + af_voff(row, piece)) = vreg##IT;      \
                const float ss = rtts_sum8(af_piece_sumsq(kreg##IT));                                  \
                if (piece == 0) ksc[sp * BS + row] = (0.125f * AF_LOG2E) * __builtin_amdgcn_rsqf(fmaxf(ss, 1e-24f)); \
            } while (0)
            AF_PLACE(0); AF_PLACE(1); AF_PLACE(2); AF_PLACE(3);
#undef AF_PLACE
            AF_WSTAMP(6);
        } else {
            AF_WSTAMP(3);
            __syncthreads();
            AF_WSTAMP(4);
            {
                const float m2 = partA[16 * 64 + lane], l2 = partA[17 * 64 + lane];
                const float mm = fmaxf(m, m2);
                float a1 = __builtin_amdgcn_exp2f(m - mm), a2 = __builtin_amdgcn_exp2f(m2 - mm);
                l = l * a1 + l2 * a2;
                m = mm;
                const float inv_l = 1.f / l;
                a1 *= inv_l;
                a2 *= inv_l;
#pragma unroll
                for (int i = 0; i < 16; ++i) {
                    oacc[0][i] = oacc[0][i] * a1 + partA[i * 64 + lane] * a2;
                    oacc[1][i] = oacc[1][i] * a1 + partB[i * 64 + lane] * a2;
                }
            }
            const size_t obase = ((size_t)bh * n_hashes + c / nb) * T;
            unsigned char* stg = Ks + sp * (BS * AF_ROWB) + qt * (32 * AF_ROWB);
#pragma unroll
            for (int dt = 0; dt < 2; ++dt) {
#pragma unroll
                for (int g = 0; g < 4; ++g) {
                    uint2 pk;
                    pk.x = pack_bf16x2(oacc[dt][4 * g], oacc[dt][4 * g + 1]);
                    pk.y = pack_bf16x2(oacc[dt][4 * g + 2], oacc[dt][4 * g + 3]);
                    *reinterpret_cast<uint2*>(stg + r * AF_ROWB + (dt * 32 + 8 * g + 4 * hh) * 2) = pk;
                }
            }
            if (hh == 0) lse[obase + qpos] = (m + __builtin_amdgcn_logf(l)) * 0.6931471805599453f;
            __builtin_amdgcn_wave_barrier();
            const int srow = lane >> 3, spiece = lane & 7;
            uint4 rowv[4];
            int rpos[4];
#pragma unroll
            for (int i = 0; i < 4; ++i) {
                rowv[i] = *reinterpret_cast<const uint4*>(stg + (i * 8 + srow) * AF_ROWB + spiece * 16);
                rpos[i] = allpos[(j + 1) * BS + qt * 32 + i * 8 + srow];
            }
#pragma unroll
            for (int i = 0; i < 4; ++i) rtts_store16_out(o + (obase + rpos[i]) * AF_DH + spiece * 8, rowv[i]);
            AF_WSTAMP(5);
            if (j + 1 == L) return;
            __syncthreads();
            AF_WSTAMP(6);
        }
        __syncthreads();
        AF_WSTAMP(7);
    }
}

static RttsLdsState g_fwd_lds[2][8];
static RttsLdsState g_fwd_walk_lds[2][8];

extern "C" int rtts_lsh_attn_fwd_run_length(int B, int H, int T, int n_hashes, int bucket_size) {
    if (B <= 0 || H <= 0 || n_hashes <= 0 || (bucket_size != 64 && bucket_size != 128) || T <= 0 || T % bucket_size) return -1;
    const int C = n_hashes * (T / bucket_size);
    const long long chunks = (long long)B * H * C;
    const long long resident = 256ll * (bucket_size == 128 ? 2 : 4);
    int R = 0;
    for (int cand = 8; cand >= 2; cand >>= 1)
        if (C % cand == 0 && chunks / cand >= 3 * resident) { R = cand; break; }
    const int w = rtts_walk_override(0);
    if (w >= 0) R = (w >= 1 && w <= 16 && C % w == 0) ? w : 0;
    return R;
}

template <int BS>
static int launch_attn_fwd(const bf16_t* qk, const bf16_t* v, int64_t ld, const int32_t* st, const uint8_t* mask, int B, int H,
                           int T, int n_hashes, int causal, bf16_t* o, float* lse, float drop_p, uint32_t seed,
                           const uint32_t* seed_dev, hipStream_t stream) {
    constexpr int NK = 2 * BS;
    const int L = rtts_lsh_attn_fwd_run_length(B, H, T, n_hashes, BS);
    const int C = n_hashes * (T / BS);
    const size_t lds = L > 0 ? (size_t)(2 * (L + 1) * BS + NK + 256) * 4 + (size_t)NK * (AF_ROWB + 128) : 2 * NK * AF_ROWB + NK * 12;
    const dim3 grid(L > 0 ? B * H * (C / L) : B * H * C), block(BS * 4);
    const bool drop = drop_p > 0.f;
    const int vi = (drop ? 4 : 0) + (causal ? 2 : 0) + (mask ? 1 : 0);
    const uint32_t th = rtts_drop_thresh(drop_p);
    const float sc = 1.f / (1.f - drop_p);
#define AF_GO(C_, M_, D_)                                                                                                  \
    do {                                                                                                                   \
        if (L > 0) {                                                                                                       \
            auto kern = lsh_attn_fwd_walk_kernel<BS, C_, M_, D_>;                                                          \
            RTTS_ENSURE_LDS("rtts_lsh_attn_fwd", kern, lds, g_fwd_walk_lds[BS == 128][vi]);                                \
            hipLaunchKernelGGL(kern, grid, block, lds, stream, qk, v, ld, st, mask, H, T, n_hashes, o, lse, seed, seed_dev, th, sc, L); \
        } else {                                                                                                           \
            auto kern = lsh_attn_fwd_kernel<BS, C_, M_, D_>;                                                               \
            RTTS_ENSURE_LDS("rtts_lsh_attn_fwd", kern, lds, g_fwd_lds[BS == 128][vi]);                                     \
            hipLaunchKernelGGL(kern, grid, block, lds, stream, qk, v, ld, st, mask, H, T, n_hashes, o, lse, seed, seed_dev, th, sc); \
        }                                                                                                                  \
    } while (0)
#define AF_GO2(C_, M_) do { if (drop) AF_GO(C_, M_, true); else AF_GO(C_, M_, false); } while (0)
    if (causal) {
        if (mask) AF_GO2(true, true); else AF_GO2(true, false);
    } else {
        if (mask) AF_GO2(false, true); else AF_GO2(false, false);
    }
#undef AF_GO2
#undef AF_GO
    RTTS_LAUNCH_CHECK("rtts_lsh_attn_fwd");
    return 0;
}

extern "C" int rtts_lsh_attn_fwd(const void* qk, const void* v, int64_t ld, const int32_t* st, const uint8_t* mask, int B,
                                 int H, int T, int dh, int n_hashes, int bucket_size, int causal, void* o, float* lse,
                                 float drop_p, uint32_t drop_seed, const uint32_t* seed_dev, void* stream) {
    RTTS_ENTER(stream);
    RTTS_REQUIRE(qk && v && st && o && lse, "rtts_lsh_attn_fwd: null pointer");
    RTTS_REQUIRE(dh == AF_DH, "rtts_lsh_attn_fwd: dh=%d unsupported (this build: 64)", dh);
    RTTS_REQUIRE(bucket_size == 64 || bucket_size == 128, "rtts_lsh_attn_fwd: bucket_size=%d unsupported (64 or 128)", bucket_size);
    RTTS_REQUIRE(T > 0 && T % (2 * bucket_size) == 0,
                 "rtts_lsh_attn_fwd: Sequence length (%d) needs to be divisible by target bucket size x 2 - %d", T, 2 * bucket_size);
    RTTS_REQUIRE(B > 0 && H > 0 && n_hashes > 0, "rtts_lsh_attn_fwd: bad B/H/n_hashes");
    RTTS_REQUIRE(ld >= (int64_t)H * dh && ld % 8 == 0, "rtts_lsh_attn_fwd: ld must be >= H*dh and a multiple of 8");
    RTTS_REQUIRE((((uintptr_t)qk | (uintptr_t)v | (uintptr_t)o) & 15) == 0, "rtts_lsh_attn_fwd: qk, v, o must be 16-byte aligned");
    RTTS_REQUIRE(drop_p >= 0.f && drop_p < 1.f, "rtts_lsh_attn_fwd: drop_p must be in [0, 1)");
    RTTS_REQUIRE(drop_p == 0.f || (uint64_t)B * H * n_hashes * T * 2 * bucket_size < (1ull << 32),
                 "rtts_lsh_attn_fwd: dropout on more than 2^32 query-key pairs");
    hipStream_t s = (hipStream_t)stream;
    if (bucket_size == 64)
        return launch_attn_fwd<64>((const bf16_t*)qk, (const bf16_t*)v, ld, st, mask, B, H, T, n_hashes, causal, (bf16_t*)o, lse, drop_p,
                                   drop_seed, seed_dev, s);
    return launch_attn_fwd<128>((const bf16_t*)qk, (const bf16_t*)v, ld, st, mask, B, H, T, n_hashes, causal, (bf16_t*)o, lse, drop_p,
                                drop_seed, seed_dev, s);
}
```

### reformer-tts_amd/csrc/lsh_combine.hip

```cpp
#include "rtts_common.h"
#include <float.h>

#define CB_DH 64
#define CB_MAXR 16

__device__ __forceinline__ void unpack8(const uint4 u, float* f) {
    const uint32_t w[4] = {u.x, u.y, u.z, u.w};
#pragma unroll
    for (int k = 0; k < 4; ++k) {
        f[2 * k] = __uint_as_float(w[k] << 16);
        f[2 * k + 1] = __uint_as_float(w[k] & 0xffff0000u);
    }
}

__device__ __forceinline__ uint4 pack8(const float* f) {
    uint4 u;
    u.x = pack_bf16x2(f[0], f[1]);
    u.y = pack_bf16x2(f[2], f[3]);
    u.z = pack_bf16x2(f[4], f[5]);
    u.w = pack_bf16x2(f[6], f[7]);
    return u;
}

__global__ __launch_bounds__(256) void lsh_combine_fwd_kernel(const bf16_t* __restrict__ o, const float* __restrict__ lse, int H,
                                                              int T, int n_hashes, size_t rows, bf16_t* __restrict__ out,
                                                              int64_t ld_out, float* __restrict__ lse_tot) {
    const size_t gid = (size_t)blockIdx.x * blockDim.x + threadIdx.x;
    const size_t row = gid >> 3;
    const int piece = gid & 7;
    if (row >= rows) return;
    const int bh = row / T, t = row % T;
    const int b = bh / H, h = bh % H;
    float lv[CB_MAXR];
    float m = -FLT_MAX;
    for (int r = 0; r < n_hashes; ++r) {
        lv[r] = lse[((size_t)bh * n_hashes + r) * T + t];
        m = fmaxf(m, lv[r]);
    }
    float acc[8] = {0, 0, 0, 0, 0, 0, 0, 0}, wsum = 0.f;
    for (int r = 0; r < n_hashes; ++r) {
        const float w = __expf(lv[r] - m);
        wsum += w;
        float f[8];
        unpack8(*reinterpret_cast<const uint4*>(o + (((size_t)bh * n_hashes + r) * T + t) * CB_DH + piece * 8), f);
#pragma unroll
        for (int k = 0; k < 8; ++k) acc[k] = __builtin_fmaf(w, f[k], acc[k]);
    }
    const float inv = 1.f / wsum;
#pragma unroll
    for (int k = 0; k < 8; ++k) acc[k] *= inv;
    *reinterpret_cast<uint4*>(out + ((size_t)b * T + t) * ld_out + h * CB_DH + piece * 8) = pack8(acc);
    if (piece == 0) lse_tot[row] = m + logf(wsum);
}

__global__ __launch_bounds__(256) void lsh_bwd_delta_kernel(const bf16_t* __restrict__ out, int64_t ld_out,
                                                            const bf16_t* __restrict__ dout, int64_t ld_do, int H, int T,
                                                            size_t rows, float* __restrict__ delta) {
    const size_t gid = (size_t)blockIdx.x * blockDim.x + threadIdx.x;
    const size_t row = gid >> 3;
    const int piece = gid & 7;
    float s = 0.f;
    if (row < rows) {
        const int bh = row / T, t = row % T;
        const int b = bh / H, h = bh % H;
        float a[8], g[8];
        unpack8(*reinterpret_cast<const uint4*>(out + ((size_t)b * T + t) * ld_out + h * CB_DH + piece * 8), a);
        unpack8(*reinterpret_cast<const uint4*>(dout + ((size_t)b * T + t) * ld_do + h * CB_DH + piece * 8), g);
#pragma unroll
        for (int k = 0; k < 8; ++k) s = __builtin_fmaf(a[k], g[k], s);
    }
    s = rtts_sum8(s);
    if (row < rows && piece == 0) delta[row] = s;
}

__global__ __launch_bounds__(256) void lsh_bwd_reduce_kernel(const bf16_t* __restrict__ dqk_part, const bf16_t* __restrict__ dv_part,
                                                             int H, int T, int n_hashes, size_t rows, size_t slot_stride,
                                                             bf16_t* __restrict__ dqk, bf16_t* __restrict__ dv, int64_t ld_d,
                                                             const uint8_t* __restrict__ row_flags) {
    const size_t gid = (size_t)blockIdx.x * blockDim.x + threadIdx.x;
    const size_t row = gid >> 3;
    const int piece = gid & 7;
    if (row >= rows) return;
    const int bh = row / T, t = row % T;
    const int b = bh / H, h = bh % H;
    float aq[8] = {0, 0, 0, 0, 0, 0, 0, 0}, av[8] = {0, 0, 0, 0, 0, 0, 0, 0};
    for (int r = 0; r < n_hashes; ++r) {
        const size_t rr = ((size_t)bh * n_hashes + r) * T + t;
        const size_t off = rr * CB_DH + piece * 8;
        const int nslot = (row_flags == nullptr || row_flags[rr]) ? 2 : 1;
        float f[8];
        for (int s = 0; s < nslot; ++s) {
            unpack8(*reinterpret_cast<const uint4*>(dqk_part + s * slot_stride + off), f);
#pragma unroll
            for (int k = 0; k < 8; ++k) aq[k] += f[k];
            unpack8(*reinterpret_cast<const uint4*>(dv_part + s * slot_stride + off), f);
#pragma unroll
            for (int k = 0; k < 8; ++k) av[k] += f[k];
        }
    }
    const size_t oo = ((size_t)b * T + t) * ld_d + h * CB_DH + piece * 8;
    *reinterpret_cast<uint4*>(dqk + oo) = pack8(aq);
    *reinterpret_cast<uint4*>(dv + oo) = pack8(av);
}

extern "C" int rtts_lsh_combine_fwd(const void* o, const float* lse, int B, int H, int T, int dh, int n_hashes, void* out,
                                    int64_t ld_out, float* lse_tot, void* stream) {
    RTTS_ENTER(stream);
    RTTS_REQUIRE(o && lse && out && lse_tot, "rtts_lsh_combine_fwd: null pointer");
    RTTS_REQUIRE(dh == CB_DH && n_hashes > 0 && n_hashes <= CB_MAXR, "rtts_lsh_combine_fwd: need dh == 64, n_hashes <= 16");
    RTTS_REQUIRE(B > 0 && H > 0 && T > 0 && ld_out >= (int64_t)H * dh && ld_out % 8 == 0, "rtts_lsh_combine_fwd: bad shape/stride");
    RTTS_REQUIRE((((uintptr_t)o | (uintptr_t)out) & 15) == 0, "rtts_lsh_combine_fwd: buffers must be 16-byte aligned");
    const size_t rows = (size_t)B * H * T;
    const unsigned grid = (unsigned)((rows * 8 + 255) / 256);
    hipLaunchKernelGGL(lsh_combine_fwd_kernel, dim3(grid), dim3(256), 0, (hipStream_t)stream, (const bf16_t*)o, lse, H, T, n_hashes,
                       rows, (bf16_t*)out, ld_out, lse_tot);
    RTTS_LAUNCH_CHECK("rtts_lsh_combine_fwd");
    return 0;
}

extern "C" int rtts_lsh_bwd_delta(const void* out, int64_t ld_out, const void* dout, int64_t ld_dout, int B, int H, int T, int dh,
                                  float* delta, void* stream) {
    RTTS_ENTER(stream);
    RTTS_REQUIRE(out && dout && delta, "rtts_lsh_bwd_delta: null pointer");
    RTTS_REQUIRE(dh == CB_DH && B > 0 && H > 0 && T > 0, "rtts_lsh_bwd_delta: need dh == 64");
    RTTS_REQUIRE(ld_out >= (int64_t)H * dh && ld_out % 8 == 0 && ld_dout >= (int64_t)H * dh && ld_dout % 8 == 0,
                 "rtts_lsh_bwd_delta: bad strides");
    RTTS_REQUIRE((((uintptr_t)out | (uintptr_t)dout) & 15) == 0, "rtts_lsh_bwd_delta: buffers must be 16-byte aligned");
    const size_t rows = (size_t)B * H * T;
    const unsigned grid = (unsigned)((rows * 8 + 255) / 256);
    hipLaunchKernelGGL(lsh_bwd_delta_kernel, dim3(grid), dim3(256), 0, (hipStream_t)stream, (const bf16_t*)out, ld_out,
                       (const bf16_t*)dout, ld_dout, H, T, rows, delta);
    RTTS_LAUNCH_CHECK("rtts_lsh_bwd_delta");
    return 0;
}

extern "C" int rtts_lsh_bwd_reduce(const void* dqk_part, const void* dv_part, int B, int H, int T, int dh, int n_hashes, void* dqk,
                                   void* dv, int64_t ld_d, const uint8_t* row_flags, void* stream) {
    RTTS_ENTER(stream);
    RTTS_REQUIRE(dqk_part && dv_part && dqk && dv, "rtts_lsh_bwd_reduce: null pointer");
    RTTS_REQUIRE(dh == CB_DH && B > 0 && H > 0 && T > 0 && n_hashes > 0, "rtts_lsh_bwd_reduce: need dh == 64");
    RTTS_REQUIRE(ld_d >= (int64_t)H * dh && ld_d % 8 == 0, "rtts_lsh_bwd_reduce: bad stride");
    RTTS_REQUIRE((((uintptr_t)dqk_part | (uintptr_t)dv_part | (uintptr_t)dqk | (uintptr_t)dv) & 15) == 0,
                 "rtts_lsh_bwd_reduce: buffers must be 16-byte aligned");
    const size_t rows = (size_t)B * H * T;
    const size_t slot_stride = rows * n_hashes * CB_DH;
    const unsigned grid = (unsigned)((rows * 8 + 255) / 256);
    hipLaunchKernelGGL(lsh_bwd_reduce_kernel, dim3(grid), dim3(256), 0, (hipStream_t)stream, (const bf16_t*)dqk_part,
                       (const bf16_t*)dv_part, H, T, n_hashes, rows, slot_stride, (bf16_t*)dqk, (bf16_t*)dv, ld_d, row_flags);
    RTTS_LAUNCH_CHECK("rtts_lsh_bwd_reduce");
    return 0;
}
```

### reformer-tts_amd/csrc/rtts_api.cpp

```cpp
#include <stdarg.h>
#include <stdio.h>
#include <atomic>
#include "../../include/rtts.h"

static thread_local char g_err[512] = "";

extern "C" void rtts_set_error(const char* fmt, ...) {
    va_list ap;
    va_start(ap, fmt);
    vsnprintf(g_err, sizeof(g_err), fmt, ap);
    va_end(ap);
}

extern "C" const char* rtts_last_error(void) { return g_err; }
extern "C" int rtts_version(void) { return RTTS_VERSION; }

static std::atomic<int> g_walk[2] = {{-1}, {-1}};
int rtts_walk_override(int backward) { return g_walk[backward ? 1 : 0].load(std::memory_order_relaxed); }
extern "C" int rtts_debug_set_walk(int fwd_run, int bwd_run) {
    if (fwd_run < -1 || fwd_run > 16 || bwd_run < -1 || bwd_run > 64) {
        rtts_set_error("rtts_debug_set_walk: run lengths are -1 (library's pick), 0 (one-chunk kernel) or 1..16 / 1..64 (got %d, %d)", fwd_run, bwd_run);
        return -1;
    }
    g_walk[0].store(fwd_run, std::memory_order_relaxed);
    g_walk[1].store(bwd_run, std::memory_order_relaxed);
    return 0;
}
```

### reformer-tts_amd/csrc/rtts_common.h

```cpp
#pragma once
#include <hip/hip_runtime.h>
#include <stdint.h>
#include <stdio.h>
#include <stdarg.h>
#include <atomic>

#include "../../include/rtts.h"

typedef uint16_t bf16_t;
typedef __attribute__((ext_vector_type(8))) __bf16 bf16x8;
typedef __attribute__((ext_vector_type(4))) __bf16 bf16x4;
typedef __attribute__((ext_vector_type(4))) short short4v;
typedef __attribute__((ext_vector_type(16))) float f32x16;
typedef __attribute__((ext_vector_type(4))) float f32x4;

#define RTTS_LDS __attribute__((address_space(3)))

extern "C" void rtts_set_error(const char* fmt, ...);
int rtts_walk_override(int backward);

#define RTTS_REQUIRE(cond, ...)            \
    do {                                   \
        if (!(cond)) {                     \
            rtts_set_error(__VA_ARGS__);   \
            return -1;                     \
        }                                  \
    } while (0)

#define RTTS_LAUNCH_CHECK(name)                                              \
    do {                                                                     \
        hipError_t e_ = hipGetLastError();                                   \
        if (e_ != hipSuccess) {                                              \
            int dev_ = -1;                                                   \
            (void)hipGetDevice(&dev_);                                       \
            rtts_set_error("%s: launch failed: %s (current device %d; the entry points launch on the caller's current device: " \
                           "the stream and every pointer must belong to it)", name, hipGetErrorString(e_), dev_); \
            return -2;                                                       \
        }                                                                    \
    } while (0)

static inline int rtts_bind_device(void* stream) {
    if (!stream) return 0;
    hipDevice_t dev = -1;
    if (hipStreamGetDevice((hipStream_t)stream, &dev) != hipSuccess) {
        (void)hipGetLastError();
        rtts_set_error("the stream handle %p does not belong to any device of this process", stream);
        return -3;
    }
    int cur = -1;
    if (hipGetDevice(&cur) == hipSuccess && cur == (int)dev) return 0;
    if (hipSetDevice((int)dev) != hipSuccess) {
        (void)hipGetLastError();
        rtts_set_error("cannot bind the calling thread to device %d (the device of the stream)", (int)dev);
        return -3;
    }
    return 0;
}
#define RTTS_ENTER(stream)                              \
    do {                                                \
        const int rc_enter_ = rtts_bind_device(stream); \
        if (rc_enter_) return rc_enter_;                \
    } while (0)

struct RttsLdsState { std::atomic<size_t> set[64]; };
static inline hipError_t rtts_ensure_lds(const void* func, size_t lds, RttsLdsState& st) {
    if (lds <= 64 * 1024) return hipSuccess;
    int dev = 0;
    if (hipGetDevice(&dev) != hipSuccess || dev < 0 || dev >= 64) dev = 0;
    if (st.set[dev].load(std::memory_order_acquire) >= lds) return hipSuccess;
    const hipError_t e = hipFuncSetAttribute(func, hipFuncAttributeMaxDynamicSharedMemorySize, (int)lds);
    if (e == hipSuccess) {
        size_t cur = st.set[dev].load(std::memory_order_relaxed);
        while (cur < lds && !st.set[dev].compare_exchange_weak(cur, lds, std::memory_order_release, std::memory_order_relaxed)) {}
    }
    return e;
}
#define RTTS_ENSURE_LDS(name, func, lds, state)                                                                   \
    do {                                                                                                          \
        const hipError_t e_lds_ = rtts_ensure_lds(reinterpret_cast<const void*>(func), (lds), (state));           \
        RTTS_REQUIRE(e_lds_ == hipSuccess, "%s: cannot raise the dynamic LDS limit to %zu bytes: %s", name, (size_t)(lds), \
                     hipGetErrorString(e_lds_));                                                                  \
    } while (0)

#ifndef RTTS_WT_STORES
#define RTTS_WT_STORES 1
#endif
typedef int rtts_v4i __attribute__((ext_vector_type(4)));
__device__ __forceinline__ void rtts_store16_out(void* p, const uint4 v) {
#if RTTS_WT_STORES
    const rtts_v4i w = {(int)v.x, (int)v.y, (int)v.z, (int)v.w};
    asm volatile("global_store_dwordx4 %0, %1, off sc1\n\ts_nop 1" ::"v"(p), "v"(w) : "memory");
#else
    *reinterpret_cast<uint4*>(p) = v;
#endif
}

__device__ __forceinline__ float bf16_to_f32(bf16_t x) { return __uint_as_float(((uint32_t)x) << 16); }

__device__ __forceinline__ bf16_t f32_to_bf16(float x) {
    __bf16 b = (__bf16)x;
    return __builtin_bit_cast(bf16_t, b);
}
// ... 50 lines not shown
```

### reformer-tts_amd/engine.py

```python
from __future__ import annotations

from typing import List, Optional

import os

import torch

from . import _lib, ops
from ._seeds import next_seed, seed_base
from .model.lsh_attention import LSHSelfAttention


STASH_ATTENTION = True
STASH_BLOCK_OUTPUT = True
STASH_PROJECTIONS = True
STASH_STREAMS = True
_NO_G = object()


def _streams_kept() -> bool:
    return STASH_STREAMS and STASH_ATTENTION and STASH_BLOCK_OUTPUT and STASH_PROJECTIONS


RECOMPUTE_MODES = ("full", "attention-stash", "output-stash", "projection-stash", "stash")
# ... 506 lines not shown
    m, n = dy.shape
    k = x.shape[1]
    if n % 128 == 0 and k % 128 == 0 and m % 64 == 0 and dy.stride(1) == 1 and x.stride(1) == 1 and grad_view.stride(1) == 1:
        if DEFER_WGRAD and accumulate:
            _queue().wgrads.append((grad_view, dy, x))
            _queue_final_flush()
            return
        ws = _slab_ws(dy.device)
        _lib.call("rtts_gemm_tn", dy.data_ptr(), dy.stride(0), x.data_ptr(), x.stride(0), m, n, k, grad_view.data_ptr(),
                  grad_view.stride(0), int(accumulate), ws.data_ptr(), ws.numel(), _s())
    elif n % 128 == 0 and m % 64 == 0 and m >= 4096 and k < 128 and dy.stride(1) == 1:
        xp = torch.zeros(m, 128, dtype=x.dtype, device=x.device)
        xp[:, :k].copy_(x)
        tmp = torch.empty(n, 128, dtype=torch.float32, device=x.device)
        ws = _slab_ws(dy.device)
        _lib.call("rtts_gemm_tn", dy.data_ptr(), dy.stride(0), xp.data_ptr(), 128, m, n, 128, tmp.data_ptr(), 128, 0, ws.data_ptr(),
                  ws.numel(), _s())
        if accumulate:
            grad_view.add_(tmp[:, :k])
        else:
            grad_view.copy_(tmp[:, :k])
    else:
        _lib.note_general_path("weight gradient", f"dW {n} x {k} over {m} rows does not tile (N, K % 128, M % 64): library GEMM")
        if accumulate:
            grad_view.add_(torch.mm(dy.t(), x, out_dtype=torch.float32))
        else:
            grad_view.copy_(torch.mm(dy.t(), x, out_dtype=torch.float32))


def _keep_streams(keep, slot, acc, inp, xn, mean, rstd, fresh=False):
    if not keep:
        if fresh:
            out = slot["acc_out"] = torch.empty_like(acc)
            return out
        return None
    out = torch.empty_like(acc)
    slot.update(inp=inp, pre=(xn, mean, rstd), acc_out=out)
    if STASH_BLOCK_OUTPUT:
        slot["g"] = None
    return out


class LSHExec:

    def __init__(self, withnorm):
        self.norm = withnorm.norm
        self.layer: LSHSelfAttention = withnorm.fn.layer
        self._own_slot = {}

    @staticmethod
    def supported(withnorm) -> bool:
        return withnorm.fn.layer.dim % 64 == 0

    def _wqkv(self):
        lyr = self.layer
        a, b = _bf16(lyr.toqk.weight), _bf16(lyr.tov.weight)
        if _adjacent(a, b):
            return torch.as_strided(a, (2 * a.shape[0], a.shape[1]), (a.shape[1], 1))
        return torch.cat([a, b], dim=0)

    def _wqkv_grad(self):
        lyr = self.layer
        ga, gb = _grad(lyr.toqk.weight), _grad(lyr.tov.weight)
        if _adjacent(ga, gb):
            return torch.as_strided(ga, (2 * ga.shape[0], ga.shape[1]), (ga.shape[1], 1)), None
        return None, (ga, gb)

    def _internals(self, inp, b, t, mask, st, stash=None, g=None, pre=None, qkv=None, adrop=None):
        lyr = self.layer
        e = lyr.dim
        if t <= lyr.full_attn_thres:
            raise NotImplementedError("full-attention shortcut (T <= full_attn_thres) is outside the HIP path")
        xn, mean, rstd = pre if pre is not None else ln_fwd(inp, self.norm)
        wqkv = self._wqkv()
        if qkv is None:
            qkv = gemm(xn, wqkv).view(b, t, 2 * e)
        if st is None:
            rot = lyr._rotations(qkv, t // lyr.bucket_size)
            st, _, _ = ops.lsh_hash_sort(qkv[..., :e], rot, lyr.heads, lyr.bucket_size)
        lyr.last_st = st
        if stash is not None:
            out, lse_tot = stash
        else:
            o, lse = ops.lsh_attn_fwd(qkv[..., :e], qkv[..., e:], st, lyr.heads, lyr.bucket_size, lyr.causal, mask, adrop)
            out, lse_tot = ops.lsh_combine_fwd(o, lse, b, lyr.heads)
        if g is None:
            g = gemm(out.view(b * t, e), _bf16(lyr.to_out.weight))
        return xn, mean, rstd, wqkv, qkv, st, out, lse_tot, g

    def forward(self, acc, inp, b, t, mask=None, pre=None, next_norm=None, slot=None, keep_streams=False, fresh_acc=False, **_):
        slot = self._own_slot if slot is None else slot
        pa = getattr(self.layer, "dropout", 0.0) if self.layer.training else 0.0
        adrop = (pa, next_seed()) if pa > 0.0 else None
        xn, mean, rstd, _, qkv, st, out, lse_tot, g = self._internals(inp, b, t, mask, None, pre=pre, adrop=adrop)
        p = self.layer.post_attn_dropout.p if self.layer.training else 0.0
        slot.clear()
        slot.update(st=st, stash=(out, lse_tot) if STASH_ATTENTION else None, g=g if STASH_BLOCK_OUTPUT else None,
                    qkv=qkv if STASH_PROJECTIONS else None, drop=(p, next_seed()) if p > 0.0 else None, adrop=adrop)
        return residual(acc, g, self.layer.to_out.bias, 1.0, next_norm, slot["drop"], out=_keep_streams(keep_streams, slot, acc, inp, xn, mean, rstd, fresh_acc))

    def backward(self, acc, inp, d_acc, d_inp, b, t, mask=None, pre=None, next_norm=None, pre_cast=None, next_cast=None, slot=None,
                 d_src=None, join=None, **_):
        slot = self._own_slot if slot is None else slot
        if "st" not in slot:
            raise RuntimeError("LSHExec.backward: no forward state for this call (backward run twice, or without its forward)")
        lyr = self.layer
        e = lyr.dim
        kept = "inp" in slot
        if kept:
            inp, pre = slot["inp"], slot["pre"]
        adrop = slot.get("adrop")
        xn, mean, rstd, wqkv, qkv, st, out, lse_tot, g = self._internals(inp, b, t, mask, slot["st"], slot["stash"],
                                                                         _NO_G if kept else slot["g"], pre, slot["qkv"], adrop)
        drop = slot["drop"]
        slot.clear()
        post = None if kept else residual(acc, g, lyr.to_out.bias, -1.0, next_norm, drop)
        dyb = _out_grad(d_acc, _grad(lyr.to_out.bias), drop, pre_cast)
        out2 = out.view(b * t, e)
        wgrad(_grad(lyr.to_out.weight), dyb, out2)
        delta = None
        if FUSE_DELTA and e == 64 * lyr.heads and dgrad_delta_ok(b * t, e):
            dout, delta = gemm_dgrad_delta(dyb, _bf16(lyr.to_out.weight), out2, t, lyr.heads)
            dout = dout.view(b, t, e)
        else:
            dout = gemm(dyb, _bf16(lyr.to_out.weight), kn=True).view(b, t, e)
        dqkv = torch.empty_like(qkv)
        ops.lsh_attn_bwd(qkv[..., :e], qkv[..., e:], st, out, dout, lse_tot, lyr.heads, lyr.bucket_size, lyr.causal, mask,
                         dqkv=(dqkv[..., :e], dqkv[..., e:]), drop=adrop, delta=delta)
        dqkv2 = dqkv.view(b * t, 2 * e)
        gview, pair = self._wqkv_grad()
        if gview is not None:
            wgrad(gview, dqkv2, xn)
        else:
            _lib.note_general_path("weight gradient", "toqk / tov gradients are not neighbours in one buffer: library GEMM")
            full = torch.mm(dqkv2.t(), xn, out_dtype=torch.float32)
            pair[0].add_(full[:e])
            pair[1].add_(full[e:])
        dxn = gemm(dqkv2, wqkv, kn=True)
        return post, ln_bwd(dxn, inp, mean, rstd, self.norm, d_inp, next_cast, dx_in=d_src, join=join)


class FFNExec:

    def __init__(self, mod):
        wn = mod.fn if hasattr(mod, "chunks") else mod
        self.norm = wn.norm
        self.l1, self.l2 = wn.fn.net[0], wn.fn.net[3]
        self._own_slot = {}

    @staticmethod
    def supported(mod) -> bool:
        wn = mod.fn if hasattr(mod, "chunks") else mod
        lin1, lin2 = wn.fn.net[0], wn.fn.net[3]
        return wn.fn.net[2].p == 0.0 and all(v % 64 == 0 for v in (lin1.in_features, lin1.out_features, lin2.out_features))

    def _internals(self, inp, g=None, pre=None, h=None):
        xn, mean, rstd = pre if pre is not None else ln_fwd(inp, self.norm)
        if h is None:
            words = gate_words(xn.shape[0], self.l1.weight.shape[0], xn.device)
            h = (gemm(xn, _bf16(self.l1.weight), bias=self.l1.bias, relu=True, words=words), words)
        if g is None:
            g = gemm(h[0], _bf16(self.l2.weight))
        return xn, mean, rstd, h, g

    def forward(self, acc, inp, b, t, pre=None, next_norm=None, slot=None, keep_streams=False, fresh_acc=False, **_):
        slot = self._own_slot if slot is None else slot
        xn, mean, rstd, h, g = self._internals(inp, pre=pre)
        slot.clear()
# ... 396 lines not shown
```

### reformer-tts_amd/model/lsh_attention.py

```python
from __future__ import annotations

from typing import Optional

import torch
from torch import nn
import torch.nn.functional as F

from .. import ops
from .._seeds import next_seed


class _LSHAttnFn(torch.autograd.Function):

    @staticmethod
    def forward(ctx, qkv, st, mask, heads, bucket_size, causal, drop=None):
        d = qkv.shape[-1] // 2
        qk, v = qkv[..., :d], qkv[..., d:]
        o, lse = ops.lsh_attn_fwd(qk, v, st, heads, bucket_size, causal, mask, drop)
        out, lse_tot = ops.lsh_combine_fwd(o, lse, qkv.shape[0], heads)
        ctx.save_for_backward(qkv, st, out, lse_tot, mask)
        ctx.cfg = (heads, bucket_size, causal, drop)
        return out

    @staticmethod
    def backward(ctx, dout):
        qkv, st, out, lse_tot, mask = ctx.saved_tensors
        heads, bucket_size, causal, drop = ctx.cfg
        d = qkv.shape[-1] // 2
        dqkv = torch.empty_like(qkv)
        if dout.dtype != torch.bfloat16 or dout.stride(2) != 1:
            dout = dout.to(torch.bfloat16).contiguous()
        ops.lsh_attn_bwd(qkv[..., :d], qkv[..., d:], st, out, dout, lse_tot, heads, bucket_size, causal, mask,
                         dqkv=(dqkv[..., :d], dqkv[..., d:]), drop=drop)
        return dqkv, None, None, None, None, None, None


def _gemm_tiles(m: int, n: int, k: int) -> bool:
    rows = any(m % r == 0 for r in (96, 128))
    return rows and n % 128 == 0 and k % 128 == 0 and m % 64 == 0


class _ProjectFn(torch.autograd.Function):

    @staticmethod
    def forward(ctx, x, bias, *weights):
        from .. import engine
        wb = (weights[0] if len(weights) == 1 else torch.cat(weights, dim=0)).detach().to(torch.bfloat16)
        y = engine.gemm(x, wb, bias=None if bias is None else bias.detach().float().contiguous())
        ctx.save_for_backward(x, wb)
        ctx.split = [w.shape[0] for w in weights]
        ctx.has_bias = bias is not None
        return y

    @staticmethod
    def backward(ctx, dy):
        from .. import _lib, engine
        x, wb = ctx.saved_tensors
        dy = dy if (dy.dtype == torch.bfloat16 and dy.is_contiguous()) else dy.to(torch.bfloat16).contiguous()
        dx = engine.gemm(dy, wb, kn=True) if ctx.needs_input_grad[0] else None
        dw = torch.empty(wb.shape, dtype=torch.float32, device=x.device)
        engine.wgrad(dw, dy, x, accumulate=False)
        db = None
        if ctx.has_bias:
            m, n = dy.shape
            db = torch.zeros(n, dtype=torch.float32, device=x.device)
            ws = torch.empty(256 * n, dtype=torch.float32, device=x.device)
            _lib.call("rtts_colsum_bf16", dy.data_ptr(), None, dy.stride(0), db.data_ptr(), ws.data_ptr(), m, n, 0, 1.0, None,
                      torch.cuda.current_stream().cuda_stream)
        return (dx, db, *torch.split(dw, ctx.split, dim=0))


def _project(x2, bias, *weights):
    m, k = x2.shape
    n = sum(w.shape[0] for w in weights)
    if x2.is_cuda and _gemm_tiles(m, n, k):
        return _ProjectFn.apply(x2, bias, *weights)
    from .._lib import note_general_path
    note_general_path("LSH attention projections", f"({m} x {k}) -> {n} does not tile (rows % 96 or 128, widths % 128): library GEMM")
    w = (weights[0] if len(weights) == 1 else torch.cat(weights, dim=0)).to(torch.bfloat16)
    return F.linear(x2, w, None if bias is None else bias.to(torch.bfloat16))


class LSHSelfAttention(nn.Module):
    def __init__(self, dim, heads=8, bucket_size=64, n_hashes=8, causal=False, add_local_attn_hash=False,
                 attn_chunks=1, random_rotations_per_head=False, attend_across_buckets=True,
                 allow_duplicate_attention=True, num_mem_kv=0, one_value_head=False, use_full_attn=False,
                 full_attn_thres=None, return_attn=False, post_attn_dropout=0.0, dropout=0.0, seed=0):
        super().__init__()
        if dim % heads != 0:
            raise AssertionError("dimensions must be divisible by number of heads")
        unsupported = dict(add_local_attn_hash=add_local_attn_hash, attend_across_buckets=not attend_across_buckets,
                           allow_duplicate_attention=not allow_duplicate_attention, num_mem_kv=num_mem_kv,
                           one_value_head=one_value_head, use_full_attn=use_full_attn, return_attn=return_attn)
        if not 0.0 <= dropout < 1.0:
            raise ValueError(f"dropout must be in [0, 1), got {dropout}")
        bad = [k for k, v in unsupported.items() if v]
        if bad:
            raise NotImplementedError(f"implementation='hip' supports the default value of {bad} only")
        if dim // heads != 64:
            raise NotImplementedError(f"implementation='hip' is built for dim/heads == 64 (got {dim // heads})")
        self.dim, self.heads, self.bucket_size, self.n_hashes, self.causal = dim, heads, bucket_size, n_hashes, causal
        self.random_rotations_per_head = random_rotations_per_head
# ... 92 lines not shown
```

### reformer-tts_amd/ops.py

```python
from __future__ import annotations

from typing import Optional, Tuple

import torch

from . import _lib


class _Timing:

    def __init__(self):
        self.tags = ()
        self.records = {}

    def enable(self, *tags: str):
        self.tags, self.records = tuple(tags), {}

    def disable(self):
        self.tags = ()

    def start(self, tag: str):
        if not self.tags or not any(tag == t or tag.startswith(t + "/") for t in self.tags):
            return None
        ev = torch.cuda.Event(enable_timing=True)
# ... 12 lines not shown
        recs = [r for k, v in self.records.items() if k == tag or k.startswith(tag + "/") for r in v]
        if not recs:
            return 0.0, 0, 0.0
        torch.cuda.synchronize()
        ms = [a.elapsed_time(b) for a, b, _ in recs]
        return sum(ms) / len(ms), len(ms), sum(f for _, _, f in recs) / len(ms)


TIMING = _Timing()


def _stream() -> int:
    return torch.cuda.current_stream().cuda_stream


def _ptr(t: Optional[torch.Tensor]) -> Optional[int]:
    return None if t is None else t.data_ptr()


def _check_rows(x: torch.Tensor, name: str) -> int:
    if not (x.is_cuda and x.dtype == torch.bfloat16 and x.dim() == 3):
        raise ValueError(f"{name}: expected a CUDA bfloat16 (B,T,W) tensor, got {x.dtype} {tuple(x.shape)} on {x.device}")
    if x.stride(2) != 1 or x.stride(0) != x.shape[1] * x.stride(1):
        raise ValueError(f"{name}: rows must be contiguous with a single row stride, got strides {x.stride()}")
    return x.stride(1)


def lsh_hash_sort(qk: torch.Tensor, rotations: torch.Tensor, heads: int, bucket_size: int,
                  want_buckets: bool = False, want_undo: bool = False):
    ld = _check_rows(qk, "qk")
    b, t, d = qk.shape
    dh = d // heads
    if t % (2 * bucket_size) != 0:
        raise AssertionError(f"Sequence length ({t}) needs to be divisible by target bucket size  x 2 - {bucket_size * 2}")
    if not (rotations.is_cuda and rotations.dtype == torch.float32 and rotations.is_contiguous() and rotations.dim() == 4):
        raise ValueError("rotations: expected a contiguous CUDA float32 (rows, dh, n_hashes, n_buckets/2) tensor")
    rows, rdh, n_hashes, half = rotations.shape
    if rdh != dh or 2 * half != t // bucket_size or rows not in (1, b * heads):
        raise ValueError(f"rotations shape {tuple(rotations.shape)} does not match dh={dh}, n_buckets={t // bucket_size}")
    st = torch.empty(b * heads, n_hashes, t, dtype=torch.int32, device=qk.device)
    buckets = torch.empty_like(st) if want_buckets else None
    undo = torch.empty_like(st) if want_undo else None
    ev = TIMING.start(f"rtts_lsh_hash_sort/nb{t // bucket_size}")
    _lib.call("rtts_lsh_hash_sort", qk.data_ptr(), ld, rotations.data_ptr(), rows, b, heads, t, dh, n_hashes, bucket_size,
              _ptr(buckets), st.data_ptr(), _ptr(undo), _stream())
    TIMING.stop(ev, float(b * heads * t) * (dh * 2 + n_hashes * 4 + n_hashes * 8))
    return st, buckets, undo


def _check_mask(mask: Optional[torch.Tensor], b: int, t: int, device) -> Optional[torch.Tensor]:
    if mask is None:
        return None
    if mask.shape != (b, t):
        raise ValueError(f"input_mask: expected shape {(b, t)}, got {tuple(mask.shape)}")
    return mask.to(device=device, dtype=torch.uint8).contiguous()


def _drop_args(drop, device):
    if not drop or drop[0] <= 0.0:
        return 0.0, 0, None
    from ._seeds import seed_base
    return float(drop[0]), int(drop[1]) & 0xFFFFFFFF, seed_base(device).data_ptr()


def lsh_attn_fwd(qk, v, st, heads: int, bucket_size: int, causal: bool, mask=None, drop=None):
    ld = _check_rows(qk, "qk")
    if _check_rows(v, "v") != ld or v.shape != qk.shape:
        raise ValueError("qk and v must share shape and row stride")
    b, t, d = qk.shape
    dh = d // heads
    n_hashes = st.shape[1]
    if st.shape != (b * heads, n_hashes, t) or st.dtype != torch.int32 or not st.is_contiguous():
        raise ValueError("st: expected contiguous int32 (B*H, n_hashes, T)")
    mask = _check_mask(mask, b, t, qk.device)
    o = torch.empty(b * heads, n_hashes, t, dh, dtype=torch.bfloat16, device=qk.device)
    lse = torch.empty(b * heads, n_hashes, t, dtype=torch.float32, device=qk.device)
    ev = TIMING.start(f"rtts_lsh_attn_fwd/bs{bucket_size}")
    _lib.call("rtts_lsh_attn_fwd", qk.data_ptr(), v.data_ptr(), ld, st.data_ptr(), _ptr(mask), b, heads, t, dh, n_hashes,
              bucket_size, int(causal), o.data_ptr(), lse.data_ptr(), *_drop_args(drop, qk.device), _stream())
    TIMING.stop(ev, 2.0 * 2.0 * bucket_size * (2 * bucket_size) * dh * (n_hashes * t // bucket_size) * b * heads)
    return o, lse


def lsh_combine_fwd(o, lse, batch: int, heads: int, out: Optional[torch.Tensor] = None):
    bh, n_hashes, t, dh = o.shape
    if out is None:
        out = torch.empty(batch, t, heads * dh, dtype=torch.bfloat16, device=o.device)
    ld_out = _check_rows(out, "out")
    lse_tot = torch.empty(bh, t, dtype=torch.float32, device=o.device)
    _lib.call("rtts_lsh_combine_fwd", o.data_ptr(), lse.data_ptr(), batch, heads, t, dh, n_hashes, out.data_ptr(), ld_out,
              lse_tot.data_ptr(), _stream())
    return out, lse_tot


def lsh_attn_bwd(qk, v, st, out, dout, lse_tot, heads: int, bucket_size: int, causal: bool, mask=None,
                 dqkv: Optional[Tuple[torch.Tensor, torch.Tensor]] = None, drop=None, delta: Optional[torch.Tensor] = None):
    ld = _check_rows(qk, "qk")
    if _check_rows(v, "v") != ld:
        raise ValueError("qk and v must share a row stride")
    ld_out, ld_do = _check_rows(out, "out"), _check_rows(dout, "dout")
    b, t, d = qk.shape
    dh = d // heads
    n_hashes = st.shape[1]
    mask = _check_mask(mask, b, t, qk.device)
    dev = qk.device
    if delta is None:
        delta = torch.empty(b * heads, t, dtype=torch.float32, device=dev)
        _lib.call("rtts_lsh_bwd_delta", out.data_ptr(), ld_out, dout.data_ptr(), ld_do, b, heads, t, dh, delta.data_ptr(), _stream())
    elif delta.shape != (b * heads, t) or delta.dtype != torch.float32 or not delta.is_contiguous():
        raise ValueError("delta: expected contiguous fp32 (B*H, T)")
    dqk_part = torch.empty(_lib.load().rtts_lsh_bwd_qk_slots(), b * heads, n_hashes, t, dh, dtype=torch.bfloat16, device=dev)
    dv_part = torch.empty(2, b * heads, n_hashes, t, dh, dtype=torch.bfloat16, device=dev)
    walks = _lib.load().rtts_lsh_attn_bwd_run_length(b, heads, t, n_hashes, bucket_size) > 0
    flags = torch.empty(b * heads, n_hashes, t, dtype=torch.uint8, device=dev) if walks else None
    ev = TIMING.start(f"rtts_lsh_attn_bwd/bs{bucket_size}")
    _lib.call("rtts_lsh_attn_bwd", qk.data_ptr(), v.data_ptr(), ld, st.data_ptr(), _ptr(mask), dout.data_ptr(), ld_do,
              lse_tot.data_ptr(), delta.data_ptr(), b, heads, t, dh, n_hashes, bucket_size, int(causal), dqk_part.data_ptr(),
              dv_part.data_ptr(), _ptr(flags), *_drop_args(drop, dev), _stream())
    TIMING.stop(ev, 5.0 * 2.0 * bucket_size * (2 * bucket_size) * dh * (n_hashes * t // bucket_size) * b * heads)
    if dqkv is None:
        dqk = torch.empty(b, t, d, dtype=torch.bfloat16, device=dev)
        dv = torch.empty(b, t, d, dtype=torch.bfloat16, device=dev)
    else:
        dqk, dv = dqkv
    ld_d = _check_rows(dqk, "dqk")
    if _check_rows(dv, "dv") != ld_d:
        raise ValueError("dqk and dv must share a row stride")
    _lib.call("rtts_lsh_bwd_reduce", dqk_part.data_ptr(), dv_part.data_ptr(), b, heads, t, dh, n_hashes, dqk.data_ptr(),
              dv.data_ptr(), ld_d, _ptr(flags), _stream())
    return dqk, dv


def mel_spectrogram(audio: torch.Tensor, sample_offsets_host, frame_offsets_host, offsets: torch.Tensor, nseg: int,
                    dft_basis: torch.Tensor, mel_basis: torch.Tensor, n_fft: int, hop: int, power: int, clip: float,
                    out: torch.Tensor) -> torch.Tensor:
    for name, t in (("audio", audio), ("dft_basis", dft_basis), ("mel_basis", mel_basis), ("out", out)):
        if not (t.is_cuda and t.dtype == torch.float32):
            raise _lib.RttsError(f"mel_spectrogram runs on the GPU only: {name} must be a CUDA float32 tensor "
                                 f"(got {t.dtype} on {t.device})")
    if not (offsets.is_cuda and offsets.dtype == torch.int64 and offsets.shape == (2, nseg + 1) and offsets.is_contiguous()):
        raise ValueError(f"offsets: expected a contiguous CUDA int64 (2, {nseg + 1}) table")
    n_mels = mel_basis.shape[0]
    if not (audio.dim() == 1 and audio.is_contiguous() and dft_basis.is_contiguous() and mel_basis.is_contiguous()
            and tuple(dft_basis.shape) == (n_fft, n_fft) and tuple(mel_basis.shape) == (n_mels, n_fft // 2 + 1)
            and out.dim() == 2 and out.shape[0] == n_mels and out.stride(1) == 1):
        raise ValueError("mel_spectrogram: audio flat, dft_basis (n_fft, n_fft), mel_basis (n_mels, n_fft/2 + 1), out (n_mels, frames) rows")
    if audio.numel() < sample_offsets_host[nseg] or out.shape[1] < frame_offsets_host[nseg]:
        raise ValueError(f"mel_spectrogram: {audio.numel()} samples / {out.shape[1]} output frames for offsets ending at "
                         f"{sample_offsets_host[nseg]} / {frame_offsets_host[nseg]}")
    frames = frame_offsets_host[nseg]
    ev = TIMING.start(f"rtts_mel_spectrogram/n{n_fft}")
    _lib.call("rtts_mel_spectrogram", audio.data_ptr(), sample_offsets_host, frame_offsets_host, offsets[0].data_ptr(),
              offsets[1].data_ptr(), nseg, dft_basis.data_ptr(), mel_basis.data_ptr(), n_fft, hop, n_mels, power, clip,
              out.data_ptr(), out.stride(0), _stream())
    TIMING.stop(ev, 2.0 * frames * (n_fft * n_fft + n_mels * (n_fft // 2 + 1)))
    return out


def resample(audio: torch.Tensor, in_offsets_host, out_offsets_host, offsets: torch.Tensor, nseg: int, first: torch.Tensor,
             taps_table: torch.Tensor, orig_red: int, new_red: int, out: torch.Tensor, channels: int = 1) -> torch.Tensor:
    if not (audio.is_cuda and audio.dtype in (torch.float32, torch.int16)):
        raise _lib.RttsError(f"resample runs on the GPU only: audio must be a CUDA float32 or int16 tensor (got {audio.dtype} on {audio.device})")
    for name, t, dt in (("first", first, torch.int32), ("taps_table", taps_table, torch.float32), ("out", out, torch.float32)):
        if not (t.is_cuda and t.dtype == dt):
            raise _lib.RttsError(f"resample runs on the GPU only: {name} must be a CUDA {dt} tensor (got {t.dtype} on {t.device})")
    if not (offsets.is_cuda and offsets.dtype == torch.int64 and offsets.shape == (2, nseg + 1) and offsets.is_contiguous()):
        raise ValueError(f"offsets: expected a contiguous CUDA int64 (2, {nseg + 1}) table")
    if not (audio.dim() == 1 and audio.is_contiguous() and out.dim() == 1 and out.is_contiguous() and first.is_contiguous()
            and taps_table.dim() == 2 and taps_table.is_contiguous() and tuple(first.shape) == (new_red,)
            and taps_table.shape[1] == new_red):
        raise ValueError("resample: audio and out flat, first (new_red,), taps_table (taps, new_red)")
    if audio.numel() < in_offsets_host[nseg] * channels or out.numel() < out_offsets_host[nseg]:
        raise ValueError(f"resample: {audio.numel()} input values / {out.numel()} output samples for offsets ending at "
                         f"{in_offsets_host[nseg]} frames of {channels} channel(s) / {out_offsets_host[nseg]}")
    taps = taps_table.shape[0]
    ev = TIMING.start(f"rtts_resample/{orig_red}to{new_red}")
    _lib.call("rtts_resample", audio.data_ptr(), 0 if audio.dtype == torch.float32 else 1, channels, in_offsets_host, out_offsets_host,
              offsets[0].data_ptr(), offsets[1].data_ptr(), nseg, first.data_ptr(), taps_table.data_ptr(), orig_red, new_red, taps,
              out.data_ptr(), _stream())
    TIMING.stop(ev, 2.0 * taps * out_offsets_host[nseg])
    return out
```

Before: 1.901 million mel-frames/s.

## Fuse LSH combine and backward reduce into attention kernels via per-head tickets

Adds a per-(batch,head) atomic ticket counter so the last workgroup finishing a head runs the cross-hash combine (forward) or partial-gradient reduce (backward) inside the attention kernel's launch. This removes two separate kernel launches and lets the reduction start while other heads are still computing attention. In exchange the tail work runs serialized on one workgroup per head, and each backward call adds a memset for the tickets and an agent-scope acquire fence.

```diff
diff --git a/include/rtts.h b/include/rtts.h
--- a/include/rtts.h
+++ b/include/rtts.h
@@ -37,6 +37,18 @@
                       void* stream);
 int rtts_lsh_bwd_reduce(const void* dqk_part, const void* dv_part, int B, int H, int T, int dh, int n_hashes,
                         void* dqk, void* dv, int64_t ld_d, const uint8_t* row_flags, void* stream);
+
+int64_t rtts_lsh_ticket_bytes(int B, int H);
+int rtts_lsh_attn_fwd_combined(const void* qk, const void* v, int64_t ld, const int32_t* st, const uint8_t* mask,
+                               int B, int H, int T, int dh, int n_hashes, int bucket_size, int causal,
+                               void* o, float* lse, float drop_p, uint32_t drop_seed, const uint32_t* seed_dev,
+                               void* out, int64_t ld_out, float* lse_tot, int32_t* tickets, void* stream);
+int rtts_lsh_attn_bwd_reduced(const void* qk, const void* v, int64_t ld, const int32_t* st, const uint8_t* mask,
+                              const void* dout, int64_t ld_dout, const float* lse_tot, const float* delta,
+                              int B, int H, int T, int dh, int n_hashes, int bucket_size, int causal,
+                              void* dqk_part, void* dv_part, uint8_t* row_flags, float drop_p, uint32_t drop_seed,
+                              const uint32_t* seed_dev, void* dqk, void* dv, int64_t ld_d, int32_t* tickets, void* stream);
+int rtts_debug_set_lsh_fused(int on);
 
 int rtts_grad_clip_scale(const float* grads, int64_t n, float grad_mult, float max_norm, float* partial_ws,
                          float* scale_out, void* stream);
diff --git a/reformer-tts_amd/_lib.py b/reformer-tts_amd/_lib.py
--- a/reformer-tts_amd/_lib.py
+++ b/reformer-tts_amd/_lib.py
@@ -59,6 +59,12 @@
     "rtts_lsh_attn_bwd_run_length": [_i32, _i32, _i32, _i32, _i32],
     "rtts_debug_set_walk": [_i32, _i32],
     "rtts_lsh_bwd_reduce": [_vp, _vp, _i32, _i32, _i32, _i32, _i32, _vp, _vp, _i64, _vp, _vp],
+    "rtts_lsh_ticket_bytes": [_i32, _i32],
+    "rtts_lsh_attn_fwd_combined": [_vp, _vp, _i64, _vp, _vp, _i32, _i32, _i32, _i32, _i32, _i32, _i32, _vp, _vp, _f32, _u32, _vp,
+                                   _vp, _i64, _vp, _vp, _vp],
+    "rtts_lsh_attn_bwd_reduced": [_vp, _vp, _i64, _vp, _vp, _vp, _i64, _vp, _vp, _i32, _i32, _i32, _i32, _i32, _i32, _i32, _vp, _vp, _vp,
+                                  _f32, _u32, _vp, _vp, _vp, _i64, _vp, _vp],
+    "rtts_debug_set_lsh_fused": [_i32],
     "rtts_grad_clip_scale": [_vp, _i64, _f32, _f32, _vp, _vp, _vp],
     "rtts_ln_fwd": [_vp, _vp, _vp, _vp, _vp, _vp, _i32, _i32, _vp],
     "rtts_ln_bwd": [_vp, _vp, _vp, _vp, _vp, _vp, _vp, _vp, _vp, _i32, _i32, _vp, _vp, _f32, _u32, _vp, _vp],
@@ -179,6 +185,7 @@
         lib.rtts_gemm_nt_gate_words.restype = C.c_int64
         lib.rtts_mel_frames.restype = C.c_int64
         lib.rtts_resample_len.restype = C.c_int64
+        lib.rtts_lsh_ticket_bytes.restype = C.c_int64
         _lib = lib
         fw, bw = os.environ.get("RTTS_LSH_FWD_WALK"), os.environ.get("RTTS_LSH_BWD_WALK")
         if fw is not None or bw is not None:
diff --git a/reformer-tts_amd/csrc/lsh_attn_bwd.hip b/reformer-tts_amd/csrc/lsh_attn_bwd.hip
--- a/reformer-tts_amd/csrc/lsh_attn_bwd.hip
+++ b/reformer-tts_amd/csrc/lsh_attn_bwd.hip
@@ -1,4 +1,5 @@
 #include "rtts_common.h"
+#include "lsh_rows.h"
 #include <float.h>
 
 #define AB_DH 64
@@ -72,12 +73,22 @@
     float scale;
 };
 
-template <int BS, bool CAUSAL, bool MASKED, bool DROP>
+template <typename TAIL>
+__device__ __forceinline__ void ab_tail(const TAIL& tail, const bf16_t* dqk_part, const bf16_t* dv_part, int H, int T, int n_hashes,
+                                        size_t slot_stride, const uint8_t* row_flags, int bh, int ring_wgs, int nthr,
+                                        unsigned char* smem) {
+    if constexpr (TAIL::fused) {
+        if (lsh_ring_arrive(tail.tickets + bh, ring_wgs, reinterpret_cast<int*>(smem)))
+            lsh_bwd_reduce_ring(tail, dqk_part, dv_part, H, T, n_hashes, slot_stride, row_flags, bh, (int)threadIdx.x, nthr);
+    }
+}
+
+template <int BS, bool CAUSAL, bool MASKED, bool DROP, typename TAIL = LshNoTail>
 __global__ __launch_bounds__(BS * 4 / AB_KT2, AB_KT2 == 2 ? 1 : 2) void lsh_attn_bwd_kernel(
     const bf16_t* __restrict__ qk, const bf16_t* __restrict__ v, int64_t ld, const int32_t* __restrict__ st,
     const uint8_t* __restrict__ mask, const bf16_t* __restrict__ dout, int64_t ld_do, const float* __restrict__ lse_tot,
     const float* __restrict__ delta, int H, int T, int n_hashes, bf16_t* __restrict__ dqk_part, bf16_t* __restrict__ dv_part,
-    size_t slot_stride, AbDrop dr) {
+    size_t slot_stride, AbDrop dr, TAIL tail) {
     constexpr int KT2 = AB_KT2;
     constexpr int NK = 2 * BS;
     constexpr int NQT = BS / 32;
@@ -468,6 +479,7 @@
     __builtin_amdgcn_s_waitcnt(0);
     AB_STAMP(9);
 #endif
+    ab_tail(tail, dqk_part, dv_part, H, T, n_hashes, slot_stride, nullptr, bh, C, NTHR, smem);
 }
 
 
@@ -477,12 +489,12 @@
     asm volatile("s_mov_b32 m0, %1\n\ts_nop 0\n\tglobal_load_lds_dwordx4 %0, off" ::"v"(gptr), "s"(m0v) : "m0");
 }
 
-template <int BS, bool CAUSAL, bool MASKED, bool DROP>
+template <int BS, bool CAUSAL, bool MASKED, bool DROP, typename TAIL = LshNoTail>
 __global__ __launch_bounds__(BS * 4, 2) void lsh_attn_bwd_walk_kernel(
     const bf16_t* __restrict__ qk, const bf16_t* __restrict__ v, int64_t ld, const int32_t* __restrict__ st,
     const uint8_t* __restrict__ mask, const bf16_t* __restrict__ dout, int64_t ld_do, const float* __restrict__ lse_tot,
     const float* __restrict__ delta, int H, int T, int n_hashes, bf16_t* __restrict__ dqk_part, bf16_t* __restrict__ dv_part,
-    size_t slot_stride, int R, uint8_t* __restrict__ row_flags, AbDrop dr) {
+    size_t slot_stride, int R, uint8_t* __restrict__ row_flags, AbDrop dr, TAIL tail) {
     constexpr int NK = 2 * BS;
     constexpr int NQT = BS / 32;
     constexpr int NW = NK / 32;
@@ -967,6 +979,7 @@
 #endif
     }
 #undef AB_JSTAMP
+    ab_tail(tail, dqk_part, dv_part, H, T, n_hashes, slot_stride, row_flags, bh, runs, NTHR, smem);
 }
 
 extern "C" int rtts_lsh_bwd_qk_slots(void) { return RTTS_LSH_BWD_QK_SLOTS; }
@@ -984,11 +997,11 @@
     return R;
 }
 
-template <int BS>
+template <int BS, typename TAIL>
 static int launch_attn_bwd(const bf16_t* qk, const bf16_t* v, int64_t ld, const int32_t* st, const uint8_t* mask,
                            const bf16_t* dout, int64_t ld_do, const float* lse_tot, const float* delta, int B, int H, int T,
                            int n_hashes, int causal, bf16_t* dqk_part, bf16_t* dv_part, uint8_t* row_flags, float drop_p,
-                           uint32_t drop_seed, const uint32_t* seed_dev, hipStream_t stream) {
+                           uint32_t drop_seed, const uint32_t* seed_dev, hipStream_t stream, TAIL tail) {
     constexpr int NK = 2 * BS;
     const size_t slot_stride = (size_t)B * H * n_hashes * T * AB_DH;
     const bool drop = drop_p > 0.f;
@@ -1006,10 +1019,10 @@
         const dim3 wgrid((unsigned)(chunks / R)), wblock(BS * 4);
 #define AB_WGO(C_, M_, D_)                                                                                                 \
     do {                                                                                                                   \
-        auto kern = lsh_attn_bwd_walk_kernel<BS, C_, M_, D_>;                                                              \
+        auto kern = lsh_attn_bwd_walk_kernel<BS, C_, M_, D_, TAIL>;                                                        \
         RTTS_ENSURE_LDS("rtts_lsh_attn_bwd", kern, wlds, wattr[vi]);                                                       \
         hipLaunchKernelGGL(kern, wgrid, wblock, wlds, stream, qk, v, ld, st, mask, dout, ld_do, lse_tot, delta, H, T, n_hashes, \
-                           dqk_part, dv_part, slot_stride, R, row_flags, dr);                                              \
+                           dqk_part, dv_part, slot_stride, R, row_flags, dr, tail);                                        \
     } while (0)
 #define AB_WGO2(C_, M_) do { if (drop) AB_WGO(C_, M_, true); else AB_WGO(C_, M_, false); } while (0)
         if (causal) {
@@ -1027,10 +1040,10 @@
     static RttsLdsState attr[8];
 #define AB_GO(C_, M_, D_)                                                                                                  \
     do {                                                                                                                   \
-        auto kern = lsh_attn_bwd_kernel<BS, C_, M_, D_>;                                                                   \
+        auto kern = lsh_attn_bwd_kernel<BS, C_, M_, D_, TAIL>;                                                             \
         RTTS_ENSURE_LDS("rtts_lsh_attn_bwd", kern, lds, attr[vi]);                                                         \
         hipLaunchKernelGGL(kern, grid, block, lds, stream, qk, v, ld, st, mask, dout, ld_do, lse_tot, delta, H, T, n_hashes, \
-                           dqk_part, dv_part, slot_stride, dr);                                                            \
+                           dqk_part, dv_part, slot_stride, dr, tail);                                                      \
     } while (0)
 #define AB_GO2(C_, M_) do { if (drop) AB_GO(C_, M_, true); else AB_GO(C_, M_, false); } while (0)
     if (causal) {
@@ -1044,28 +1057,72 @@
     return 0;
 }
 
+static int check_attn_bwd(const char* who, const void* qk, const void* v, int64_t ld, const int32_t* st, const void* dout,
+                          int64_t ld_dout, const float* lse_tot, const float* delta, int B, int H, int T, int dh, int n_hashes,
+                          int bucket_size, const void* dqk_part, const void* dv_part, float drop_p) {
+    RTTS_REQUIRE(qk && v && st && dout && lse_tot && delta && dqk_part && dv_part, "%s: null pointer", who);
+    RTTS_REQUIRE(dh == AB_DH, "%s: dh=%d unsupported (this build: 64)", who, dh);
+    RTTS_REQUIRE(bucket_size == 64 || bucket_size == 128, "%s: bucket_size=%d unsupported (64 or 128)", who, bucket_size);
+    RTTS_REQUIRE(T > 0 && T % (2 * bucket_size) == 0,
+                 "%s: Sequence length (%d) needs to be divisible by target bucket size x 2 - %d", who, T, 2 * bucket_size);
+    RTTS_REQUIRE(B > 0 && H > 0 && n_hashes > 0, "%s: bad B/H/n_hashes", who);
+    RTTS_REQUIRE(ld >= (int64_t)H * dh && ld % 8 == 0 && ld_dout >= (int64_t)H * dh && ld_dout % 8 == 0,
+                 "%s: row strides must be >= H*dh and multiples of 8", who);
+    RTTS_REQUIRE((((uintptr_t)qk | (uintptr_t)v | (uintptr_t)dout | (uintptr_t)dqk_part | (uintptr_t)dv_part) & 15) == 0,
+                 "%s: buffers must be 16-byte aligned", who);
+    RTTS_REQUIRE(drop_p >= 0.f && drop_p < 1.f, "%s: drop_p must be in [0, 1)", who);
+    RTTS_REQUIRE(drop_p == 0.f || (uint64_t)B * H * n_hashes * T * 2 * bucket_size < (1ull << 32),
+                 "%s: dropout on more than 2^32 query-key pairs (the forward refuses the same shape)", who);
+    return 0;
+}
+
 extern "C" int rtts_lsh_attn_bwd(const void* qk, const void* v, int64_t ld, const int32_t* st, const uint8_t* mask,
                                  const void* dout, int64_t ld_dout, const float* lse_tot, const float* delta, int B, int H,
                                  int T, int dh, int n_hashes, int bucket_size, int causal, void* dqk_part, void* dv_part,
                                  uint8_t* row_flags, float drop_p, uint32_t drop_seed, const uint32_t* seed_dev, void* stream) {
     RTTS_ENTER(stream);
-    RTTS_REQUIRE(qk && v && st && dout && lse_tot && delta && dqk_part && dv_part, "rtts_lsh_attn_bwd: null pointer");
-    RTTS_REQUIRE(dh == AB_DH, "rtts_lsh_attn_bwd: dh=%d unsupported (this build: 64)", dh);
-    RTTS_REQUIRE(bucket_size == 64 || bucket_size == 128, "rtts_lsh_attn_bwd: bucket_size=%d unsupported (64 or 128)", bucket_size);
-    RTTS_REQUIRE(T > 0 && T % (2 * bucket_size) == 0,
-                 "rtts_lsh_attn_bwd: Sequence length (%d) needs to be divisible by target bucket size x 2 - %d", T, 2 * bucket_size);
-    RTTS_REQUIRE(B > 0 && H > 0 && n_hashes > 0, "rtts_lsh_attn_bwd: bad B/H/n_hashes");
-    RTTS_REQUIRE(ld >= (int64_t)H * dh && ld % 8 == 0 && ld_dout >= (int64_t)H * dh && ld_dout % 8 == 0,
-                 "rtts_lsh_attn_bwd: row strides must be >= H*dh and multiples of 8");
-    RTTS_REQUIRE((((uintptr_t)qk | (uintptr_t)v | (uintptr_t)dout | (uintptr_t)dqk_part | (uintptr_t)dv_part) & 15) == 0,
-                 "rtts_lsh_attn_bwd: buffers must be 16-byte aligned");
-    RTTS_REQUIRE(drop_p >= 0.f && drop_p < 1.f, "rtts_lsh_attn_bwd: drop_p must be in [0, 1)");
-    RTTS_REQUIRE(drop_p == 0.f || (uint64_t)B * H * n_hashes * T * 2 * bucket_size < (1ull << 32),
-                 "rtts_lsh_attn_bwd: dropout on more than 2^32 query-key pairs (the forward refuses the same shape)");
+    if (check_attn_bwd("rtts_lsh_attn_bwd", qk, v, ld, st, dout, ld_dout, lse_tot, delta, B, H, T, dh, n_hashes, bucket_size, dqk_part,
+                       dv_part, drop_p))
+        return -1;
     hipStream_t s = (hipStream_t)stream;
     if (bucket_size == 64)
         return launch_attn_bwd<64>((const bf16_t*)qk, (const bf16_t*)v, ld, st, mask, (const bf16_t*)dout, ld_dout, lse_tot, delta,
-                                   B, H, T, n_hashes, causal, (bf16_t*)dqk_part, (bf16_t*)dv_part, row_flags, drop_p, drop_seed, seed_dev, s);
+                                   B, H, T, n_hashes, causal, (bf16_t*)dqk_part, (bf16_t*)dv_part, row_flags, drop_p, drop_seed, seed_dev, s,
+                                   LshNoTail{});
     return launch_attn_bwd<128>((const bf16_t*)qk, (const bf16_t*)v, ld, st, mask, (const bf16_t*)dout, ld_dout, lse_tot, delta, B,
-                                H, T, n_hashes, causal, (bf16_t*)dqk_part, (bf16_t*)dv_part, row_flags, drop_p, drop_seed, seed_dev, s);
+                                H, T, n_hashes, causal, (bf16_t*)dqk_part, (bf16_t*)dv_part, row_flags, drop_p, drop_seed, seed_dev, s,
+                                LshNoTail{});
 }
+
+extern "C" int rtts_lsh_attn_bwd_reduced(const void* qk, const void* v, int64_t ld, const int32_t* st, const uint8_t* mask,
+                                         const void* dout, int64_t ld_dout, const float* lse_tot, const float* delta, int B, int H,
+                                         int T, int dh, int n_hashes, int bucket_size, int causal, void* dqk_part, void* dv_part,
+                                         uint8_t* row_flags, float drop_p, uint32_t drop_seed, const uint32_t* seed_dev, void* dqk,
+                                         void* dv, int64_t ld_d, int32_t* tickets, void* stream) {
+    RTTS_ENTER(stream);
+    const char* who = "rtts_lsh_attn_bwd_reduced";
+    if (check_attn_bwd(who, qk, v, ld, st, dout, ld_dout, lse_tot, delta, B, H, T, dh, n_hashes, bucket_size, dqk_part, dv_part, drop_p))
+        return -1;
+    RTTS_REQUIRE(dqk && dv, "%s: null pointer (dqk, dv)", who);
+    RTTS_REQUIRE(ld_d >= (int64_t)H * dh && ld_d % 8 == 0, "%s: ld_d must be >= H*dh and a multiple of 8", who);
+    RTTS_REQUIRE((((uintptr_t)dqk | (uintptr_t)dv) & 15) == 0, "%s: dqk, dv must be 16-byte aligned", who);
+    RTTS_REQUIRE(tickets, "%s: null ticket buffer (rtts_lsh_ticket_bytes(B, H) = %zu bytes, caller-owned)", who, lsh_ticket_bytes(B, H));
+    RTTS_REQUIRE(((uintptr_t)tickets & 15) == 0, "%s: the ticket buffer must be 16-byte aligned", who);
+    if (!rtts_lsh_fused_tails()) {
+        const int rc = rtts_lsh_attn_bwd(qk, v, ld, st, mask, dout, ld_dout, lse_tot, delta, B, H, T, dh, n_hashes, bucket_size, causal,
+                                         dqk_part, dv_part, row_flags, drop_p, drop_seed, seed_dev, stream);
+        const bool walks = rtts_lsh_attn_bwd_run_length(B, H, T, n_hashes, bucket_size) > 0;
+        return rc ? rc : rtts_lsh_bwd_reduce(dqk_part, dv_part, B, H, T, dh, n_hashes, dqk, dv, ld_d, walks ? row_flags : nullptr, stream);
+    }
+    hipStream_t s = (hipStream_t)stream;
+    const hipError_t e = hipMemsetAsync(tickets, 0, lsh_ticket_bytes(B, H), s);
+    RTTS_REQUIRE(e == hipSuccess, "%s: cannot zero the ticket buffer: %s", who, hipGetErrorString(e));
+    const LshReduceTail tail{(bf16_t*)dqk, (bf16_t*)dv, ld_d, (int*)tickets};
+    if (bucket_size == 64)
+        return launch_attn_bwd<64>((const bf16_t*)qk, (const bf16_t*)v, ld, st, mask, (const bf16_t*)dout, ld_dout, lse_tot, delta,
+                                   B, H, T, n_hashes, causal, (bf16_t*)dqk_part, (bf16_t*)dv_part, row_flags, drop_p, drop_seed, seed_dev, s,
+                                   tail);
+    return launch_attn_bwd<128>((const bf16_t*)qk, (const bf16_t*)v, ld, st, mask, (const bf16_t*)dout, ld_dout, lse_tot, delta, B,
+                                H, T, n_hashes, causal, (bf16_t*)dqk_part, (bf16_t*)dv_part, row_flags, drop_p, drop_seed, seed_dev, s,
+                                tail);
+}
diff --git a/reformer-tts_amd/csrc/lsh_attn_fwd.hip b/reformer-tts_amd/csrc/lsh_attn_fwd.hip
--- a/reformer-tts_amd/csrc/lsh_attn_fwd.hip
+++ b/reformer-tts_amd/csrc/lsh_attn_fwd.hip
@@ -1,4 +1,5 @@
 #include "rtts_common.h"
+#include "lsh_rows.h"
 #include <float.h>
 
 #define AF_DH 64
@@ -118,13 +119,22 @@
     l += af_sum16(acc);
 }
 
-template <int BS, bool CAUSAL, bool MASKED, bool DROP>
+template <typename TAIL>
+__device__ __forceinline__ void af_tail(const TAIL& tail, bf16_t* o, float* lse, int H, int T, int n_hashes, int bh, int ring_wgs,
+                                        int tid, int nthr, unsigned char* smem) {
+    if constexpr (TAIL::fused) {
+        if (lsh_ring_arrive(tail.tickets + bh, ring_wgs, reinterpret_cast<int*>(smem)))
+            lsh_combine_ring(tail, o, lse, H, T, n_hashes, bh, tid, nthr);
+    }
+}
+
+template <int BS, bool CAUSAL, bool MASKED, bool DROP, typename TAIL = LshNoTail>
 __global__ __launch_bounds__(BS * 4, 2) void lsh_attn_fwd_kernel(const bf16_t* __restrict__ qk, const bf16_t* __restrict__ v,
                                                                  int64_t ld, const int32_t* __restrict__ st,
                                                                  const uint8_t* __restrict__ mask, int H, int T, int n_hashes,
                                                                  bf16_t* __restrict__ o, float* __restrict__ lse, uint32_t drop_seed,
                                                                  const uint32_t* __restrict__ seed_dev, uint32_t drop_thresh,
-                                                                 float drop_scale) {
+                                                                 float drop_scale, TAIL tail) {
     constexpr int NK = 2 * BS;
     constexpr int NKT = NK / 32;
     constexpr int NTHR = BS * 4;
@@ -325,7 +335,10 @@
         part[33 * 64 + lane] = l;
     }
     __syncthreads();
-    if (kh == 1) return;
+    if (kh == 1) {
+        af_tail(tail, o, lse, H, T, n_hashes, bh, C, tid, NTHR, smem);
+        return;
+    }
     {
         const float m2 = part[32 * 64 + lane], l2 = part[33 * 64 + lane];
         const float mm = fmaxf(m, m2);
@@ -368,6 +381,7 @@
 #pragma unroll
     for (int i = 0; i < 4; ++i) rtts_store16_out(o + (obase + rpos[i]) * AF_DH + spiece * 8, rowv[i]);
     AF_STAMP(5);
+    af_tail(tail, o, lse, H, T, n_hashes, bh, C, tid, NTHR, smem);
 }
 
 
@@ -492,13 +506,13 @@
     return ss;
 }
 
-template <int BS, bool CAUSAL, bool MASKED, bool DROP>
+template <int BS, bool CAUSAL, bool MASKED, bool DROP, typename TAIL = LshNoTail>
 __global__ __launch_bounds__(BS * 4, 2) void lsh_attn_fwd_walk_kernel(const bf16_t* __restrict__ qk, const bf16_t* __restrict__ v,
                                                                       int64_t ld, const int32_t* __restrict__ st,
                                                                       const uint8_t* __restrict__ mask, int H, int T, int n_hashes,
                                                                       bf16_t* __restrict__ o, float* __restrict__ lse,
                                                                       uint32_t drop_seed, const uint32_t* __restrict__ seed_dev,
-                                                                      uint32_t drop_thresh, float drop_scale, int L) {
+                                                                      uint32_t drop_thresh, float drop_scale, int L, TAIL tail) {
     constexpr int NK = 2 * BS;
     constexpr int NTHR = BS * 4;
     constexpr int NQT = BS / 32;
@@ -616,6 +630,7 @@
             partA[17 * 64 + lane] = l;
             if (j + 1 == L) {
                 __syncthreads();
+                af_tail(tail, o, lse, H, T, n_hashes, bh, runs, tid, NTHR, smem);
                 return;
             }
             const int t2 = tid - NTHR / 2;
@@ -689,7 +704,10 @@
 #pragma unroll
             for (int i = 0; i < 4; ++i) rtts_store16_out(o + (obase + rpos[i]) * AF_DH + spiece * 8, rowv[i]);
             AF_WSTAMP(5);
-            if (j + 1 == L) return;
+            if (j + 1 == L) {
+                af_tail(tail, o, lse, H, T, n_hashes, bh, runs, tid, NTHR, smem);
+                return;
+            }
             __syncthreads();
             AF_WSTAMP(6);
         }
@@ -698,8 +716,8 @@
     }
 }
 
-static RttsLdsState g_fwd_lds[2][8];
-static RttsLdsState g_fwd_walk_lds[2][8];
+static RttsLdsState g_fwd_lds[2][2][8];
+static RttsLdsState g_fwd_walk_lds[2][2][8];
 
 extern "C" int rtts_lsh_attn_fwd_run_length(int B, int H, int T, int n_hashes, int bucket_size) {
     if (B <= 0 || H <= 0 || n_hashes <= 0 || (bucket_size != 64 && bucket_size != 128) || T <= 0 || T % bucket_size) return -1;
@@ -714,10 +732,10 @@
     return R;
 }
 
-template <int BS>
+template <int BS, typename TAIL>
 static int launch_attn_fwd(const bf16_t* qk, const bf16_t* v, int64_t ld, const int32_t* st, const uint8_t* mask, int B, int H,
                            int T, int n_hashes, int causal, bf16_t* o, float* lse, float drop_p, uint32_t seed,
-                           const uint32_t* seed_dev, hipStream_t stream) {
+                           const uint32_t* seed_dev, hipStream_t stream, TAIL tail) {
     constexpr int NK = 2 * BS;
     const int L = rtts_lsh_attn_fwd_run_length(B, H, T, n_hashes, BS);
     const int C = n_hashes * (T / BS);
@@ -730,13 +748,13 @@
 #define AF_GO(C_, M_, D_)                                                                                                  \
     do {                                                                                                                   \
         if (L > 0) {                                                                                                       \
-            auto kern = lsh_attn_fwd_walk_kernel<BS, C_, M_, D_>;                                                          \
-            RTTS_ENSURE_LDS("rtts_lsh_attn_fwd", kern, lds, g_fwd_walk_lds[BS == 128][vi]);                                \
-            hipLaunchKernelGGL(kern, grid, block, lds, stream, qk, v, ld, st, mask, H, T, n_hashes, o, lse, seed, seed_dev, th, sc, L); \
+            auto kern = lsh_attn_fwd_walk_kernel<BS, C_, M_, D_, TAIL>;                                                    \
+            RTTS_ENSURE_LDS("rtts_lsh_attn_fwd", kern, lds, g_fwd_walk_lds[TAIL::fused][BS == 128][vi]);                   \
+            hipLaunchKernelGGL(kern, grid, block, lds, stream, qk, v, ld, st, mask, H, T, n_hashes, o, lse, seed, seed_dev, th, sc, L, tail); \
         } else {                                                                                                           \
-            auto kern = lsh_attn_fwd_kernel<BS, C_, M_, D_>;                                                               \
-            RTTS_ENSURE_LDS("rtts_lsh_attn_fwd", kern, lds, g_fwd_lds[BS == 128][vi]);                                     \
-            hipLaunchKernelGGL(kern, grid, block, lds, stream, qk, v, ld, st, mask, H, T, n_hashes, o, lse, seed, seed_dev, th, sc); \
+            auto kern = lsh_attn_fwd_kernel<BS, C_, M_, D_, TAIL>;                                                         \
+            RTTS_ENSURE_LDS("rtts_lsh_attn_fwd", kern, lds, g_fwd_lds[TAIL::fused][BS == 128][vi]);                        \
+            hipLaunchKernelGGL(kern, grid, block, lds, stream, qk, v, ld, st, mask, H, T, n_hashes, o, lse, seed, seed_dev, th, sc, tail); \
         }                                                                                                                  \
     } while (0)
 #define AF_GO2(C_, M_) do { if (drop) AF_GO(C_, M_, true); else AF_GO(C_, M_, false); } while (0)
@@ -751,25 +769,60 @@
     return 0;
 }
 
+static int check_attn_fwd(const char* who, const void* qk, const void* v, int64_t ld, const int32_t* st, int B, int H, int T, int dh,
+                          int n_hashes, int bucket_size, const void* o, const float* lse, float drop_p) {
+    RTTS_REQUIRE(qk && v && st && o && lse, "%s: null pointer", who);
+    RTTS_REQUIRE(dh == AF_DH, "%s: dh=%d unsupported (this build: 64)", who, dh);
+    RTTS_REQUIRE(bucket_size == 64 || bucket_size == 128, "%s: bucket_size=%d unsupported (64 or 128)", who, bucket_size);
+    RTTS_REQUIRE(T > 0 && T % (2 * bucket_size) == 0,
+                 "%s: Sequence length (%d) needs to be divisible by target bucket size x 2 - %d", who, T, 2 * bucket_size);
+    RTTS_REQUIRE(B > 0 && H > 0 && n_hashes > 0, "%s: bad B/H/n_hashes", who);
+    RTTS_REQUIRE(ld >= (int64_t)H * dh && ld % 8 == 0, "%s: ld must be >= H*dh and a multiple of 8", who);
+    RTTS_REQUIRE((((uintptr_t)qk | (uintptr_t)v | (uintptr_t)o) & 15) == 0, "%s: qk, v, o must be 16-byte aligned", who);
+    RTTS_REQUIRE(drop_p >= 0.f && drop_p < 1.f, "%s: drop_p must be in [0, 1)", who);
+    RTTS_REQUIRE(drop_p == 0.f || (uint64_t)B * H * n_hashes * T * 2 * bucket_size < (1ull << 32),
+                 "%s: dropout on more than 2^32 query-key pairs", who);
+    return 0;
+}
+
 extern "C" int rtts_lsh_attn_fwd(const void* qk, const void* v, int64_t ld, const int32_t* st, const uint8_t* mask, int B,
                                  int H, int T, int dh, int n_hashes, int bucket_size, int causal, void* o, float* lse,
                                  float drop_p, uint32_t drop_seed, const uint32_t* seed_dev, void* stream) {
     RTTS_ENTER(stream);
-    RTTS_REQUIRE(qk && v && st && o && lse, "rtts_lsh_attn_fwd: null pointer");
-    RTTS_REQUIRE(dh == AF_DH, "rtts_lsh_attn_fwd: dh=%d unsupported (this build: 64)", dh);
-    RTTS_REQUIRE(bucket_size == 64 || bucket_size == 128, "rtts_lsh_attn_fwd: bucket_size=%d unsupported (64 or 128)", bucket_size);
-    RTTS_REQUIRE(T > 0 && T % (2 * bucket_size) == 0,
-                 "rtts_lsh_attn_fwd: Sequence length (%d) needs to be divisible by target bucket size x 2 - %d", T, 2 * bucket_size);
-    RTTS_REQUIRE(B > 0 && H > 0 && n_hashes > 0, "rtts_lsh_attn_fwd: bad B/H/n_hashes");
-    RTTS_REQUIRE(ld >= (int64_t)H * dh && ld % 8 == 0, "rtts_lsh_attn_fwd: ld must be >= H*dh and a multiple of 8");
-    RTTS_REQUIRE((((uintptr_t)qk | (uintptr_t)v | (uintptr_t)o) & 15) == 0, "rtts_lsh_attn_fwd: qk, v, o must be 16-byte aligned");
-    RTTS_REQUIRE(drop_p >= 0.f && drop_p < 1.f, "rtts_lsh_attn_fwd: drop_p must be in [0, 1)");
-    RTTS_REQUIRE(drop_p == 0.f || (uint64_t)B * H * n_hashes * T * 2 * bucket_size < (1ull << 32),
-                 "rtts_lsh_attn_fwd: dropout on more than 2^32 query-key pairs");
+    if (check_attn_fwd("rtts_lsh_attn_fwd", qk, v, ld, st, B, H, T, dh, n_hashes, bucket_size, o, lse, drop_p)) return -1;
     hipStream_t s = (hipStream_t)stream;
     if (bucket_size == 64)
         return launch_attn_fwd<64>((const bf16_t*)qk, (const bf16_t*)v, ld, st, mask, B, H, T, n_hashes, causal, (bf16_t*)o, lse, drop_p,
-                                   drop_seed, seed_dev, s);
+                                   drop_seed, seed_dev, s, LshNoTail{});
     return launch_attn_fwd<128>((const bf16_t*)qk, (const bf16_t*)v, ld, st, mask, B, H, T, n_hashes, causal, (bf16_t*)o, lse, drop_p,
-                                drop_seed, seed_dev, s);
-}
+                                drop_seed, seed_dev, s, LshNoTail{});
+}
+
+extern "C" int rtts_lsh_attn_fwd_combined(const void* qk, const void* v, int64_t ld, const int32_t* st, const uint8_t* mask, int B,
+                                          int H, int T, int dh, int n_hashes, int bucket_size, int causal, void* o, float* lse,
+                                          float drop_p, uint32_t drop_seed, const uint32_t* seed_dev, void* out, int64_t ld_out,
+                                          float* lse_tot, int32_t* tickets, void* stream) {
+    RTTS_ENTER(stream);
+    const char* who = "rtts_lsh_attn_fwd_combined";
+    if (check_attn_fwd(who, qk, v, ld, st, B, H, T, dh, n_hashes, bucket_size, o, lse, drop_p)) return -1;
+    RTTS_REQUIRE(out && lse_tot, "%s: null pointer (out, lse_tot)", who);
+    RTTS_REQUIRE(n_hashes <= CB_MAXR, "%s: n_hashes=%d unsupported (the round combine takes <= %d)", who, n_hashes, CB_MAXR);
+    RTTS_REQUIRE(ld_out >= (int64_t)H * dh && ld_out % 8 == 0, "%s: ld_out must be >= H*dh and a multiple of 8", who);
+    RTTS_REQUIRE(((uintptr_t)out & 15) == 0, "%s: out must be 16-byte aligned", who);
+    RTTS_REQUIRE(tickets, "%s: null ticket buffer (rtts_lsh_ticket_bytes(B, H) = %zu bytes, caller-owned)", who, lsh_ticket_bytes(B, H));
+    RTTS_REQUIRE(((uintptr_t)tickets & 15) == 0, "%s: the ticket buffer must be 16-byte aligned", who);
+    if (!rtts_lsh_fused_tails()) {
+        const int rc = rtts_lsh_attn_fwd(qk, v, ld, st, mask, B, H, T, dh, n_hashes, bucket_size, causal, o, lse, drop_p, drop_seed,
+                                         seed_dev, stream);
+        return rc ? rc : rtts_lsh_combine_fwd(o, lse, B, H, T, dh, n_hashes, out, ld_out, lse_tot, stream);
+    }
+    hipStream_t s = (hipStream_t)stream;
+    const hipError_t e = hipMemsetAsync(tickets, 0, lsh_ticket_bytes(B, H), s);
+    RTTS_REQUIRE(e == hipSuccess, "%s: cannot zero the ticket buffer: %s", who, hipGetErrorString(e));
+    const LshCombineTail tail{(bf16_t*)out, ld_out, lse_tot, (int*)tickets};
+    if (bucket_size == 64)
+        return launch_attn_fwd<64>((const bf16_t*)qk, (const bf16_t*)v, ld, st, mask, B, H, T, n_hashes, causal, (bf16_t*)o, lse, drop_p,
+                                   drop_seed, seed_dev, s, tail);
+    return launch_attn_fwd<128>((const bf16_t*)qk, (const bf16_t*)v, ld, st, mask, B, H, T, n_hashes, causal, (bf16_t*)o, lse, drop_p,
+                                drop_seed, seed_dev, s, tail);
+}
diff --git a/reformer-tts_amd/csrc/lsh_combine.hip b/reformer-tts_amd/csrc/lsh_combine.hip
--- a/reformer-tts_amd/csrc/lsh_combine.hip
+++ b/reformer-tts_amd/csrc/lsh_combine.hip
@@ -1,26 +1,4 @@
-#include "rtts_common.h"
-#include <float.h>
-
-#define CB_DH 64
-#define CB_MAXR 16
-
-__device__ __forceinline__ void unpack8(const uint4 u, float* f) {
-    const uint32_t w[4] = {u.x, u.y, u.z, u.w};
-#pragma unroll
-    for (int k = 0; k < 4; ++k) {
-        f[2 * k] = __uint_as_float(w[k] << 16);
-        f[2 * k + 1] = __uint_as_float(w[k] & 0xffff0000u);
-    }
-}
-
-__device__ __forceinline__ uint4 pack8(const float* f) {
-    uint4 u;
-    u.x = pack_bf16x2(f[0], f[1]);
-    u.y = pack_bf16x2(f[2], f[3]);
-    u.z = pack_bf16x2(f[4], f[5]);
-    u.w = pack_bf16x2(f[6], f[7]);
-    return u;
-}
+#include "lsh_rows.h"
 
 __global__ __launch_bounds__(256) void lsh_combine_fwd_kernel(const bf16_t* __restrict__ o, const float* __restrict__ lse, int H,
                                                               int T, int n_hashes, size_t rows, bf16_t* __restrict__ out,
@@ -29,28 +7,7 @@
     const size_t row = gid >> 3;
     const int piece = gid & 7;
     if (row >= rows) return;
-    const int bh = row / T, t = row % T;
-    const int b = bh / H, h = bh % H;
-    float lv[CB_MAXR];
-    float m = -FLT_MAX;
-    for (int r = 0; r < n_hashes; ++r) {
-        lv[r] = lse[((size_t)bh * n_hashes + r) * T + t];
-        m = fmaxf(m, lv[r]);
-    }
-    float acc[8] = {0, 0, 0, 0, 0, 0, 0, 0}, wsum = 0.f;
-    for (int r = 0; r < n_hashes; ++r) {
-        const float w = __expf(lv[r] - m);
-        wsum += w;
-        float f[8];
-        unpack8(*reinterpret_cast<const uint4*>(o + (((size_t)bh * n_hashes + r) * T + t) * CB_DH + piece * 8), f);
-#pragma unroll
-        for (int k = 0; k < 8; ++k) acc[k] = __builtin_fmaf(w, f[k], acc[k]);
-    }
-    const float inv = 1.f / wsum;
-#pragma unroll
-    for (int k = 0; k < 8; ++k) acc[k] *= inv;
-    *reinterpret_cast<uint4*>(out + ((size_t)b * T + t) * ld_out + h * CB_DH + piece * 8) = pack8(acc);
-    if (piece == 0) lse_tot[row] = m + logf(wsum);
+    lsh_combine_row(o, lse, H, T, n_hashes, row, piece, out, ld_out, lse_tot);
 }
 
 __global__ __launch_bounds__(256) void lsh_bwd_delta_kernel(const bf16_t* __restrict__ out, int64_t ld_out,
@@ -81,26 +38,7 @@
     const size_t row = gid >> 3;
     const int piece = gid & 7;
     if (row >= rows) return;
-    const int bh = row / T, t = row % T;
-    const int b = bh / H, h = bh % H;
-    float aq[8] = {0, 0, 0, 0, 0, 0, 0, 0}, av[8] = {0, 0, 0, 0, 0, 0, 0, 0};
-    for (int r = 0; r < n_hashes; ++r) {
-        const size_t rr = ((size_t)bh * n_hashes + r) * T + t;
-        const size_t off = rr * CB_DH + piece * 8;
-        const int nslot = (row_flags == nullptr || row_flags[rr]) ? 2 : 1;
-        float f[8];
-        for (int s = 0; s < nslot; ++s) {
-            unpack8(*reinterpret_cast<const uint4*>(dqk_part + s * slot_stride + off), f);
-#pragma unroll
-            for (int k = 0; k < 8; ++k) aq[k] += f[k];
-            unpack8(*reinterpret_cast<const uint4*>(dv_part + s * slot_stride + off), f);
-#pragma unroll
-            for (int k = 0; k < 8; ++k) av[k] += f[k];
-        }
-    }
-    const size_t oo = ((size_t)b * T + t) * ld_d + h * CB_DH + piece * 8;
-    *reinterpret_cast<uint4*>(dqk + oo) = pack8(aq);
-    *reinterpret_cast<uint4*>(dv + oo) = pack8(av);
+    lsh_bwd_reduce_row(dqk_part, dv_part, H, T, n_hashes, row, piece, slot_stride, dqk, dv, ld_d, row_flags);
 }
 
 extern "C" int rtts_lsh_combine_fwd(const void* o, const float* lse, int B, int H, int T, int dh, int n_hashes, void* out,
diff --git a/reformer-tts_amd/csrc/lsh_rows.h b/reformer-tts_amd/csrc/lsh_rows.h
--- /dev/null
+++ b/reformer-tts_amd/csrc/lsh_rows.h
@@ -0,0 +1,126 @@
+#pragma once
+#include "rtts_common.h"
+#include <float.h>
+
+#define CB_DH 64
+#define CB_MAXR 16
+
+__device__ __forceinline__ void unpack8(const uint4 u, float* f) {
+    const uint32_t w[4] = {u.x, u.y, u.z, u.w};
+#pragma unroll
+    for (int k = 0; k < 4; ++k) {
+        f[2 * k] = __uint_as_float(w[k] << 16);
+        f[2 * k + 1] = __uint_as_float(w[k] & 0xffff0000u);
+    }
+}
+
+__device__ __forceinline__ uint4 pack8(const float* f) {
+    uint4 u;
+    u.x = pack_bf16x2(f[0], f[1]);
+    u.y = pack_bf16x2(f[2], f[3]);
+    u.z = pack_bf16x2(f[4], f[5]);
+    u.w = pack_bf16x2(f[6], f[7]);
+    return u;
+}
+
+__device__ __forceinline__ void lsh_combine_row(const bf16_t* o, const float* lse, int H, int T, int n_hashes, size_t row, int piece,
+                                                bf16_t* out, int64_t ld_out, float* lse_tot) {
+    const int bh = row / T, t = row % T;
+    const int b = bh / H, h = bh % H;
+    float lv[CB_MAXR];
+    float m = -FLT_MAX;
+    for (int r = 0; r < n_hashes; ++r) {
+        lv[r] = lse[((size_t)bh * n_hashes + r) * T + t];
+        m = fmaxf(m, lv[r]);
+    }
+    float acc[8] = {0, 0, 0, 0, 0, 0, 0, 0}, wsum = 0.f;
+    for (int r = 0; r < n_hashes; ++r) {
+        const float w = __expf(lv[r] - m);
+        wsum += w;
+        float f[8];
+        unpack8(*reinterpret_cast<const uint4*>(o + (((size_t)bh * n_hashes + r) * T + t) * CB_DH + piece * 8), f);
+#pragma unroll
+        for (int k = 0; k < 8; ++k) acc[k] = __builtin_fmaf(w, f[k], acc[k]);
+    }
+    const float inv = 1.f / wsum;
+#pragma unroll
+    for (int k = 0; k < 8; ++k) acc[k] *= inv;
+    *reinterpret_cast<uint4*>(out + ((size_t)b * T + t) * ld_out + h * CB_DH + piece * 8) = pack8(acc);
+    if (piece == 0) lse_tot[row] = m + logf(wsum);
+}
+
+__device__ __forceinline__ void lsh_bwd_reduce_row(const bf16_t* dqk_part, const bf16_t* dv_part, int H, int T, int n_hashes,
+                                                   size_t row, int piece, size_t slot_stride, bf16_t* dqk, bf16_t* dv, int64_t ld_d,
+                                                   const uint8_t* row_flags) {
+    const int bh = row / T, t = row % T;
+    const int b = bh / H, h = bh % H;
+    float aq[8] = {0, 0, 0, 0, 0, 0, 0, 0}, av[8] = {0, 0, 0, 0, 0, 0, 0, 0};
+    for (int r = 0; r < n_hashes; ++r) {
+        const size_t rr = ((size_t)bh * n_hashes + r) * T + t;
+        const size_t off = rr * CB_DH + piece * 8;
+        const int nslot = (row_flags == nullptr || row_flags[rr]) ? 2 : 1;
+        float f[8];
+        for (int s = 0; s < nslot; ++s) {
+            unpack8(*reinterpret_cast<const uint4*>(dqk_part + s * slot_stride + off), f);
+#pragma unroll
+            for (int k = 0; k < 8; ++k) aq[k] += f[k];
+            unpack8(*reinterpret_cast<const uint4*>(dv_part + s * slot_stride + off), f);
+#pragma unroll
+            for (int k = 0; k < 8; ++k) av[k] += f[k];
+        }
+    }
+    const size_t oo = ((size_t)b * T + t) * ld_d + h * CB_DH + piece * 8;
+    *reinterpret_cast<uint4*>(dqk + oo) = pack8(aq);
+    *reinterpret_cast<uint4*>(dv + oo) = pack8(av);
+}
+
+__device__ __forceinline__ bool lsh_ring_arrive(int* ticket, int ring_wgs, int* lds_word) {
+    asm volatile("s_waitcnt vmcnt(0)" ::: "memory");
+    __syncthreads();
+    if (threadIdx.x == 0) {
+        __builtin_amdgcn_fence(__ATOMIC_RELEASE, "agent");
+        asm volatile("s_waitcnt vmcnt(0)" ::: "memory");
+        const int drawn = __hip_atomic_fetch_add(ticket, 1, __ATOMIC_RELAXED, __HIP_MEMORY_SCOPE_AGENT);
+        const int last = drawn == ring_wgs - 1;
+        if (last) {
+            __builtin_amdgcn_fence(__ATOMIC_ACQUIRE, "agent");
+            asm volatile("s_waitcnt vmcnt(0)" ::: "memory");
+        }
+        *lds_word = last;
+    }
+    __syncthreads();
+    return *lds_word != 0;
+}
+
+static inline size_t lsh_ticket_bytes(int B, int H) { return (((size_t)B * H * 4) + 15) & ~(size_t)15; }
+
+struct LshNoTail {
+    static constexpr bool fused = false;
+};
+struct LshCombineTail {
+    static constexpr bool fused = true;
+    bf16_t* out;
+    int64_t ld_out;
+    float* lse_tot;
+    int* tickets;
+};
+struct LshReduceTail {
+    static constexpr bool fused = true;
+    bf16_t* dqk;
+    bf16_t* dv;
+    int64_t ld_d;
+    int* tickets;
+};
+
+__device__ __forceinline__ void lsh_combine_ring(const LshCombineTail& tl, const bf16_t* o, const float* lse, int H, int T,
+                                                 int n_hashes, int bh, int tid, int nthr) {
+    for (int g = tid; g < T * 8; g += nthr)
+        lsh_combine_row(o, lse, H, T, n_hashes, (size_t)bh * T + (g >> 3), g & 7, tl.out, tl.ld_out, tl.lse_tot);
+}
+__device__ __forceinline__ void lsh_bwd_reduce_ring(const LshReduceTail& tl, const bf16_t* dqk_part, const bf16_t* dv_part, int H,
+                                                    int T, int n_hashes, size_t slot_stride, const uint8_t* row_flags, int bh,
+                                                    int tid, int nthr) {
+    for (int g = tid; g < T * 8; g += nthr)
+        lsh_bwd_reduce_row(dqk_part, dv_part, H, T, n_hashes, (size_t)bh * T + (g >> 3), g & 7, slot_stride, tl.dqk, tl.dv, tl.ld_d,
+                           row_flags);
+}
diff --git a/reformer-tts_amd/csrc/rtts_api.cpp b/reformer-tts_amd/csrc/rtts_api.cpp
--- a/reformer-tts_amd/csrc/rtts_api.cpp
+++ b/reformer-tts_amd/csrc/rtts_api.cpp
@@ -26,3 +26,15 @@
     g_walk[1].store(bwd_run, std::memory_order_relaxed);
     return 0;
 }
+
+static std::atomic<int> g_lsh_fused{1};
+int rtts_lsh_fused_tails(void) { return g_lsh_fused.load(std::memory_order_relaxed); }
+extern "C" int rtts_debug_set_lsh_fused(int on) {
+    if (on != 0 && on != 1) {
+        rtts_set_error("rtts_debug_set_lsh_fused: 0 (two launches) or 1 (the pass inside the producer's launch), got %d", on);
+        return -1;
+    }
+    g_lsh_fused.store(on, std::memory_order_relaxed);
+    return 0;
+}
+extern "C" int64_t rtts_lsh_ticket_bytes(int B, int H) { return B > 0 && H > 0 ? (int64_t)((((size_t)B * H * 4) + 15) & ~(size_t)15) : -1; }
diff --git a/reformer-tts_amd/csrc/rtts_common.h b/reformer-tts_amd/csrc/rtts_common.h
--- a/reformer-tts_amd/csrc/rtts_common.h
+++ b/reformer-tts_amd/csrc/rtts_common.h
@@ -18,6 +18,7 @@
 
 extern "C" void rtts_set_error(const char* fmt, ...);
 int rtts_walk_override(int backward);
+int rtts_lsh_fused_tails(void);
 
 #define RTTS_REQUIRE(cond, ...)            \
     do {                                   \
diff --git a/reformer-tts_amd/engine.py b/reformer-tts_amd/engine.py
--- a/reformer-tts_amd/engine.py
+++ b/reformer-tts_amd/engine.py
@@ -612,8 +612,8 @@
         if stash is not None:
             out, lse_tot = stash
         else:
-            o, lse = ops.lsh_attn_fwd(qkv[..., :e], qkv[..., e:], st, lyr.heads, lyr.bucket_size, lyr.causal, mask, adrop)
-            out, lse_tot = ops.lsh_combine_fwd(o, lse, b, lyr.heads)
+            _, _, out, lse_tot = ops.lsh_attn_fwd_combined(qkv[..., :e], qkv[..., e:], st, lyr.heads, lyr.bucket_size, lyr.causal,
+                                                           mask, adrop)
         if g is None:
             g = gemm(out.view(b * t, e), _bf16(lyr.to_out.weight))
         return xn, mean, rstd, wqkv, qkv, st, out, lse_tot, g
diff --git a/reformer-tts_amd/model/lsh_attention.py b/reformer-tts_amd/model/lsh_attention.py
--- a/reformer-tts_amd/model/lsh_attention.py
+++ b/reformer-tts_amd/model/lsh_attention.py
@@ -16,8 +16,7 @@
     def forward(ctx, qkv, st, mask, heads, bucket_size, causal, drop=None):
         d = qkv.shape[-1] // 2
         qk, v = qkv[..., :d], qkv[..., d:]
-        o, lse = ops.lsh_attn_fwd(qk, v, st, heads, bucket_size, causal, mask, drop)
-        out, lse_tot = ops.lsh_combine_fwd(o, lse, qkv.shape[0], heads)
+        _, _, out, lse_tot = ops.lsh_attn_fwd_combined(qk, v, st, heads, bucket_size, causal, mask, drop)
         ctx.save_for_backward(qkv, st, out, lse_tot, mask)
         ctx.cfg = (heads, bucket_size, causal, drop)
         return out
diff --git a/reformer-tts_amd/ops.py b/reformer-tts_amd/ops.py
--- a/reformer-tts_amd/ops.py
+++ b/reformer-tts_amd/ops.py
@@ -118,6 +118,37 @@
     return o, lse
 
 
+def lsh_tickets(batch: int, heads: int, device) -> torch.Tensor:
+    return torch.empty(_lib.load().rtts_lsh_ticket_bytes(batch, heads) // 4, dtype=torch.int32, device=device)
+
+
+def lsh_attn_fwd_combined(qk, v, st, heads: int, bucket_size: int, causal: bool, mask=None, drop=None,
+                          out: Optional[torch.Tensor] = None, tickets: Optional[torch.Tensor] = None):
+    ld = _check_rows(qk, "qk")
+    if _check_rows(v, "v") != ld or v.shape != qk.shape:
+        raise ValueError("qk and v must share shape and row stride")
+    b, t, d = qk.shape
+    dh = d // heads
+    n_hashes = st.shape[1]
+    if st.shape != (b * heads, n_hashes, t) or st.dtype != torch.int32 or not st.is_contiguous():
+        raise ValueError("st: expected contiguous int32 (B*H, n_hashes, T)")
+    mask = _check_mask(mask, b, t, qk.device)
+    o = torch.empty(b * heads, n_hashes, t, dh, dtype=torch.bfloat16, device=qk.device)
+    lse = torch.empty(b * heads, n_hashes, t, dtype=torch.float32, device=qk.device)
+    if out is None:
+        out = torch.empty(b, t, heads * dh, dtype=torch.bfloat16, device=qk.device)
+    ld_out = _check_rows(out, "out")
+    lse_tot = torch.empty(b * heads, t, dtype=torch.float32, device=qk.device)
+    if tickets is None:
+        tickets = lsh_tickets(b, heads, qk.device)
+    ev = TIMING.start(f"rtts_lsh_attn_fwd/bs{bucket_size}")
+    _lib.call("rtts_lsh_attn_fwd_combined", qk.data_ptr(), v.data_ptr(), ld, st.data_ptr(), _ptr(mask), b, heads, t, dh, n_hashes,
+              bucket_size, int(causal), o.data_ptr(), lse.data_ptr(), *_drop_args(drop, qk.device), out.data_ptr(), ld_out,
+              lse_tot.data_ptr(), tickets.data_ptr(), _stream())
+    TIMING.stop(ev, 2.0 * 2.0 * bucket_size * (2 * bucket_size) * dh * (n_hashes * t // bucket_size) * b * heads)
+    return o, lse, out, lse_tot
+
+
 def lsh_combine_fwd(o, lse, batch: int, heads: int, out: Optional[torch.Tensor] = None):
     bh, n_hashes, t, dh = o.shape
     if out is None:
@@ -149,11 +180,6 @@
     dv_part = torch.empty(2, b * heads, n_hashes, t, dh, dtype=torch.bfloat16, device=dev)
     walks = _lib.load().rtts_lsh_attn_bwd_run_length(b, heads, t, n_hashes, bucket_size) > 0
     flags = torch.empty(b * heads, n_hashes, t, dtype=torch.uint8, device=dev) if walks else None
-    ev = TIMING.start(f"rtts_lsh_attn_bwd/bs{bucket_size}")
-    _lib.call("rtts_lsh_attn_bwd", qk.data_ptr(), v.data_ptr(), ld, st.data_ptr(), _ptr(mask), dout.data_ptr(), ld_do,
-              lse_tot.data_ptr(), delta.data_ptr(), b, heads, t, dh, n_hashes, bucket_size, int(causal), dqk_part.data_ptr(),
-              dv_part.data_ptr(), _ptr(flags), *_drop_args(drop, dev), _stream())
-    TIMING.stop(ev, 5.0 * 2.0 * bucket_size * (2 * bucket_size) * dh * (n_hashes * t // bucket_size) * b * heads)
     if dqkv is None:
         dqk = torch.empty(b, t, d, dtype=torch.bfloat16, device=dev)
         dv = torch.empty(b, t, d, dtype=torch.bfloat16, device=dev)
@@ -162,8 +188,13 @@
     ld_d = _check_rows(dqk, "dqk")
     if _check_rows(dv, "dv") != ld_d:
         raise ValueError("dqk and dv must share a row stride")
-    _lib.call("rtts_lsh_bwd_reduce", dqk_part.data_ptr(), dv_part.data_ptr(), b, heads, t, dh, n_hashes, dqk.data_ptr(),
-              dv.data_ptr(), ld_d, _ptr(flags), _stream())
+    tickets = lsh_tickets(b, heads, dev)
+    ev = TIMING.start(f"rtts_lsh_attn_bwd/bs{bucket_size}")
+    _lib.call("rtts_lsh_attn_bwd_reduced", qk.data_ptr(), v.data_ptr(), ld, st.data_ptr(), _ptr(mask), dout.data_ptr(), ld_do,
+              lse_tot.data_ptr(), delta.data_ptr(), b, heads, t, dh, n_hashes, bucket_size, int(causal), dqk_part.data_ptr(),
+              dv_part.data_ptr(), _ptr(flags), *_drop_args(drop, dev), dqk.data_ptr(), dv.data_ptr(), ld_d, tickets.data_ptr(),
+              _stream())
+    TIMING.stop(ev, 5.0 * 2.0 * bucket_size * (2 * bucket_size) * dh * (n_hashes * t // bucket_size) * b * heads)
     return dqk, dv
 
 
```

Result: slower. 1.482 million mel-frames/s (-22.0%).
